# 0xPolygonZero/proof-protocol-decoder

Hardware: AMD Instinct MI355X
Metric: txn-proofs/sec (whole node), 256-txn synthetic block (higher is better)
Workload: dtype u64 (Goldilocks field)

## Files before the change

### include/bpg.h

```cpp
#ifndef BPG_H
#define BPG_H
#include <stddef.h>
#include <stdint.h>

#ifdef __cplusplus
extern "C" {
#endif

typedef enum {
  BP_OK = 0,
  BP_ERR_ABORTED = -1,
  BP_ERR_INVALID_INPUT = -2,
  BP_ERR_RANGE = -3,
  BP_ERR_DEVICE = -4,
  BP_ERR_VERIFY = -5,
  BP_ERR_UNSUPPORTED = -6
} bp_status;

const char* bp_last_error(void);
const char* bp_version(void);
int bp_device_count(void);
int bp_use_blocking_sync(int device);
int bp_host_wait_mode(int device);

// ... 61 lines not shown
  uint32_t first_index, count;
  uint32_t kind;
  uint32_t degree;
} bp_air_family;
typedef struct bp_air_desc {
  uint32_t air_id;
  char name[24];
  uint32_t fixed_n_cols;
  uint32_t n_const_max;
  uint32_t degree;
  uint32_t n_cols, n_aux;
  uint32_t n_air_constraints, n_ctl_constraints;
  uint32_t n_units;
  uint32_t n_families;
  bp_air_family families[24];
} bp_air_desc;
uint32_t bp_air_count(void);
int bp_air_describe(uint32_t air_id, uint32_t n_cols, uint32_t n_const, uint32_t deg_pow, bp_air_desc* out);

int bp_air_register(const uint64_t* program, size_t n_words, uint32_t* air_id_out);
int bp_air_unregister(uint32_t air_id);
int bp_air_program_digest(uint32_t air_id, uint8_t out[32]);

uint64_t bp_quotient_scratch_words(uint32_t air_id, const struct bp_stark_cfg* shape);
int bp_quotient_eval(uint32_t air_id, const struct bp_stark_cfg* shape, const uint64_t* d_trace_lde,
                     const uint64_t* d_aux_lde, const uint64_t* d_const_lde, const uint64_t ctl[4],
                     const uint64_t alphas[2], uint64_t* d_scratch, uint64_t* d_qvals_out, void* stream);

int bp_air_port_products(uint32_t air_id, const struct bp_stark_cfg* shape, const uint64_t* d_trace, uint64_t stride,
                         const uint64_t* d_consts, const uint64_t pub[4], const uint64_t ctl[4], uint64_t* d_aux_out, void* stream);

int bp_range_multiplicities(const uint64_t* d_values, uint64_t stride, uint32_t n_cols, uint64_t n_rows, const uint64_t* d_filter,
                            uint32_t log_range, uint64_t* d_mult, uint64_t* first_bad, void* stream);
void bp_tune_range_lds_log(int log_range);

int bp_debug_air_aux(uint32_t air_id, const struct bp_stark_cfg* shape, const uint64_t* d_trace, const uint64_t ctl[4],
                     uint64_t* d_aux_out, void* stream);

typedef struct bp_air_violation {
  uint32_t row, constraint, family, kind;
  uint64_t value;
} bp_air_violation;
int bp_air_check_trace(uint32_t air_id, const struct bp_stark_cfg* shape, const uint64_t* d_trace, uint64_t stride,
                       const uint64_t* d_consts, const uint64_t pub[4], uint32_t max_rows, uint64_t* n_violated_rows,
                       uint32_t* rows_out, bp_air_violation* viol_out, uint32_t max_viol, uint32_t* n_viol, void* stream);
int bp_air_check_trace_host(uint32_t air_id, const struct bp_stark_cfg* shape, const uint64_t* trace, uint64_t stride,
                            const uint64_t* consts, const uint64_t pub[4], uint32_t max_rows, uint64_t* n_violated_rows,
                            uint32_t* rows_out, bp_air_violation* viol_out, uint32_t max_viol, uint32_t* n_viol);

int bp_keccak_trace(const uint64_t* d_inputs, uint64_t seed, uint32_t log_n, uint64_t* d_trace_out, void* stream);
int bp_logic_trace(const uint64_t* d_inputs, uint64_t seed, uint32_t log_n, uint64_t* d_trace_out, void* stream);
int bp_memory_trace(const uint64_t* d_inputs, uint64_t seed, uint32_t log_n, uint64_t* d_trace_out, void* stream);
int bp_arithmetic_trace(const uint64_t* d_inputs, uint64_t seed, uint32_t log_n, uint64_t* d_trace_out, void* stream);
int bp_byte_packing_trace(const uint64_t* d_inputs, uint64_t seed, uint32_t log_n, uint64_t* d_trace_out, void* stream);
int bp_keccak_sponge_trace(const uint64_t* d_inputs, uint64_t seed, uint32_t log_n, uint64_t* d_trace_out, void* stream);
int bp_arithmetic_mul_trace(const uint64_t* d_inputs, uint64_t seed, uint32_t log_n, uint64_t* d_trace_out, void* stream);
int bp_arithmetic_div_trace(const uint64_t* d_inputs, uint32_t log_n, uint64_t* d_trace_out, void* stream);
int bp_arithmetic_div_layout(uint32_t* out, size_t n_words);
int bp_arithmetic_mod_trace(const uint64_t* d_inputs, uint32_t log_n, uint64_t* d_trace_out, void* stream);
int bp_arithmetic_mod_layout(uint32_t* out, size_t n_words);
int bp_arithmetic_shift_trace(const uint64_t* d_inputs, uint32_t log_n, uint64_t* d_trace_out, void* stream);
int bp_arithmetic_shift_layout(uint32_t* out, size_t n_words);
int bp_arithmetic_sdiv_trace(const uint64_t* d_inputs, uint32_t log_n, uint64_t* d_trace_out, void* stream);
int bp_arithmetic_sdiv_layout(uint32_t* out, size_t n_words);
int bp_arithmetic_exp_trace(const uint64_t* d_ops, uint32_t n_ops, const uint32_t* d_starts, uint32_t log_n, uint64_t* d_trace_out,
                            void* stream);
int bp_arithmetic_exp_layout(uint32_t* out, size_t n_words);

typedef struct bp_plonk_layout {
  uint32_t pi_len, n_paths, path_depth, path_pi0;
  uint32_t leaf_len;
} bp_plonk_layout;
int bp_plonk_constants(uint64_t seed, uint32_t log_n, const bp_plonk_layout* layout, uint64_t* d_consts_out, void* stream);
int bp_plonk_trace(const uint64_t* d_consts, uint64_t seed, const uint64_t* pi, const bp_plonk_layout* layout, const uint64_t* paths,
                   uint32_t log_n, uint64_t* d_trace_out, void* stream);

int bp_fri_fold(const uint64_t* d_values, uint32_t log_nl, uint32_t rate_bits, uint32_t arity_bits, uint64_t shift,
                const uint64_t beta[2], uint64_t* d_out, void* stream);

int bp_openings(const uint64_t* d_coeffs, uint64_t stride, uint32_t log_n, uint32_t n_cols, const uint64_t z0[2],
                const uint64_t z1[2], uint64_t* d_pw_scratch, uint64_t* d_out, void* stream);

int bp_pow_grind(const uint64_t state[12], uint32_t pos, uint32_t bits, uint64_t* nonce_out, void* stream);

typedef struct bp_stark_cfg {
  uint32_t log_n, n_cols, n_const, deg_pow, rate_bits, cap_height, num_queries, pow_bits, arity_bits,
      final_poly_bits;
} bp_stark_cfg;
int bp_stark_prove_synthetic(const bp_stark_cfg* cfg, uint64_t seed, uint64_t const_seed, int device,
                             uint8_t** out, size_t* out_len);
int bp_stark_prove_air(uint32_t air_id, const bp_stark_cfg* cfg, uint64_t seed, uint64_t const_seed, int device,
                       uint8_t** out, size_t* out_len);
int bp_stark_prove_trace(uint32_t air_id, const bp_stark_cfg* cfg, const uint64_t* d_trace, uint64_t stride,
                         const uint64_t* d_consts, const uint64_t* pub, int device, uint8_t** out, size_t* out_len);
int bp_stark_verify_air(uint32_t air_id, const bp_stark_cfg* cfg, const uint64_t* const_cap, const uint8_t* proof,
                        size_t len);
void bp_stark_public_inputs(uint64_t seed, uint64_t out[4]);
void bp_stark_public_input_list(uint64_t seed, uint64_t out[4]);
int bp_stark_verify_air_pub(uint32_t air_id, const bp_stark_cfg* cfg, const uint64_t* const_cap, const uint64_t* pub,
                            const uint8_t* proof, size_t len);
typedef struct bp_set_table {
  uint32_t air_id;
  bp_stark_cfg cfg;
  const uint64_t* d_trace;
  uint64_t stride;
  const uint64_t* d_consts;
  const uint64_t* pub;
} bp_set_table;
typedef struct bp_set_port {
  uint32_t table, port;
} bp_set_port;
typedef struct bp_set_link {
  uint32_t n_looking;
  bp_set_port looking[8];
  bp_set_port looked;
} bp_set_link;
#define BP_SET_SKIP_LINK_CHECK 1u
int bp_stark_prove_table_set(const bp_set_table* tables, uint32_t n_tables, const bp_set_link* links, uint32_t n_links,
                             uint32_t flags, int device, uint8_t** out, size_t* out_len);
int bp_stark_verify_table_set(const bp_set_table* statement, uint32_t n_tables, const uint64_t* const* const_caps,
                              const bp_set_link* links, uint32_t n_links, const uint8_t* proof, size_t len);
typedef struct bp_set_table_report {
  uint64_t n_violated_rows;
  uint32_t n_viol, reserved;
  bp_air_violation viol[8];
} bp_set_table_report;
typedef struct bp_set_link_report {
  uint32_t holds;
  uint32_t is_log;
  uint64_t n_looking, n_looked;
  uint64_t n_unbalanced;
  int32_t  first_looking_end;
  int32_t  bad_filter_end;
  int64_t  first_looking_row, first_looked_row, bad_filter_row;
  uint64_t bad_filter_value;
} bp_set_link_report;
typedef struct bp_set_report { bp_set_table_report table[8]; bp_set_link_report link[16]; } bp_set_report;
int bp_check_table_set(const bp_set_table* tables, uint32_t n_tables, const bp_set_link* links, uint32_t n_links,
                       int device, bp_set_report* out);
void bp_release_cached_memory(void);
void bp_free_buffer(uint8_t* buf);

#define BP_NUM_TABLES 7

typedef struct bp_config {
  uint32_t table_log_lo[BP_NUM_TABLES], table_log_hi[BP_NUM_TABLES];
  uint32_t stark_rate_bits, stark_cap_height, stark_num_queries, stark_pow_bits, arity_bits, final_poly_bits;
  uint32_t rec_log_n, rec_n_cols, rec_n_const, rec_rate_bits, rec_num_queries, rec_pow_bits;
  uint32_t shrink_depth;
  uint32_t rec_air_id;
  int32_t device;
  uint32_t n_workers;
  uint64_t arena_bytes;
} bp_config;

typedef struct bp_state bp_state;
typedef struct bp_verifier_state bp_verifier_state;

void bp_config_default(bp_config* cfg);
int bp_state_build(const bp_config* cfg, bp_state** out);
void bp_state_free(bp_state* s);
uint64_t bp_state_device_bytes(const bp_state* s);
const char* bp_state_warnings(const bp_state* s);
int bp_state_config(const bp_state* s, bp_config* out);

int bp_generate_txn_proof(const bp_state* s, const uint8_t* ir, size_t ir_len, const volatile int32_t* abort_flag,
// ... 152 lines not shown
```

### proof_protocol_decoder_amd/_abi.py

```python
import ctypes as C
from ctypes import POINTER as P

vp, cp, i, sz, dbl = C.c_void_p, C.c_char_p, C.c_int, C.c_size_t, C.c_double
u8, u32, u64, i32, i64 = C.c_uint8, C.c_uint32, C.c_uint64, C.c_int32, C.c_int64
u8p, u32p, u64p, i32p, szp = P(u8), P(u32), P(u64), P(i32), P(sz)
u8pp = P(u8p)

BP_OK, BP_ERR_ABORTED, BP_ERR_INVALID_INPUT, BP_ERR_RANGE, BP_ERR_DEVICE, BP_ERR_VERIFY, BP_ERR_UNSUPPORTED = 0, -1, -2, -3, -4, -5, -6
STATUS_NAMES = {v: k for k, v in list(globals().items()) if k == "BP_OK" or k.startswith("BP_ERR_")}
BP_SET_SKIP_LINK_CHECK = 1
BP_NUM_TABLES, BP_IR_WORDS, BP_PV_WORDS = 7, 25, 13

KNOBS = ("quad_threshold", "assume_loaded", "merkle_fused", "merkle_wide", "poseidon_mx", "poseidon_mx_sets",
         "poseidon_grouped", "ntt_mx", "ntt_split", "k5_spread", "host_wait", "host_poseidon", "rec_batch",
         "witness_threads", "side_lanes")


def _u32s(*names):
    return [(n, u32) for n in names]


class AirFamily(C.Structure):
    _fields_ = _u32s("first_index", "count", "kind", "degree")

# ... 104 lines not shown
_cfg, _conf, _wit, _opt, _gi = P(StarkCfg), P(BpConfig), P(TxnWitness), P(ShardOptions), P(GiOptions)
_trace = (i, [vp, u64, u32, vp, vp])
_check = [u32, _cfg, vp, u64, vp, u64p, u32, u64p, u32p, P(AirViolation), u32, u32p]
_knob, _ir_flag, _buf = (None, [i]), (i, [u64p, i]), [u8pp, szp]
PROTOTYPES = {
    "bp_last_error": (cp, []),
    "bp_version": (cp, []),
    "bp_device_count": (i, []),
    "bp_use_blocking_sync": (i, [i]),
    "bp_host_wait_mode": (i, [i]),
    "bp_ntt_batch": (i, [vp, u32, u32, u64, i, vp]),
    "bp_intt_batch": (i, [vp, u64, vp, u64, u32, u32, vp]),
    "bp_lde_batch": (i, [vp, u64, vp, u64, vp, u64, u32, u32, u32, i, vp]),
    "bp_debug_copy_u64": (i, [vp, vp, u64, vp]),
    "bp_debug_field_ops": (i, [vp, vp, vp, u64, vp]),
    "bp_debug_lazy_forms": (i, [vp, vp, vp, u64, vp]),
    "bp_debug_plonk_hash_fold": (i, [u64p, vp, vp]),
    "bp_debug_plonk_hash_fold_host": (i, [u64p, u64p]),
    "bp_debug_mul_pow2": (i, [vp, vp, u64, vp]),
    "bp_tune_quad_threshold": (None, [u64]),
    "bp_tune_merkle_fused": _knob,
    "bp_tune_merkle_wide": _knob,
    "bp_tune_poseidon_mx": _knob,
    "bp_tune_poseidon_mx_sets": _knob,
    "bp_tune_poseidon_grouped": _knob,
    "bp_tune_assume_loaded": _knob,
    "bp_tune_rec_batch": _knob,
    "bp_tune_side_lanes": _knob,
    "bp_tune_rec_riders": _knob,
    "bp_tune_txn_group": _knob,
    "bp_tune_rec_group": _knob,
    "bp_debug_rec_batch_histogram": (i, [u64p, u32, i]),
    "bp_tune_witness_threads": _knob,
    "bp_tune_host_wait": _knob,
    "bp_tune_host_poseidon": _knob,
    "bp_debug_poseidon_host": (i, [vp, sz]),
    "bp_tune_k5_spread": _knob,
    "bp_debug_poseidon_group_ops": (u32, [u32]),
    "bp_debug_poseidon_group_tables": (i, [u32, u32, u8p, i32p, i32p, i32p]),
    "bp_tune_ntt_split": _knob,
    "bp_tune_ntt_mx": _knob,
    "bp_tune_reset": (None, []),
    "bp_debug_tune_state": (i, [cp, sz]),
    "bp_debug_ntt_mx_tables": (i, [i, i, u8p, i32p, u64p, u64p]),
    "bp_debug_poseidon_mx_cin": (i, [u32p]),
    "bp_poseidon_perm_batch": (i, [vp, u64, vp]),
    "bp_merkle_digest_words": (u64, [u32, u32]),
    "bp_merkle_commit": (i, [vp, u64, u32, u32, u32, u32, vp, vp]),
    "bp_air_count": (u32, []),
    "bp_air_describe": (i, [u32, u32, u32, u32, P(AirDesc)]),
    "bp_air_register": (i, [vp, sz, u32p]),
    "bp_air_unregister": (i, [u32]),
    "bp_air_program_digest": (i, [u32, cp]),
    "bp_quotient_scratch_words": (u64, [u32, _cfg]),
    "bp_quotient_eval": (i, [u32, _cfg, vp, vp, vp, u64p, u64p, vp, vp, vp]),
    "bp_air_port_products": (i, [u32, _cfg, vp, u64, vp, u64p, u64p, vp, vp]),
    "bp_range_multiplicities": (i, [vp, u64, u32, u64, vp, u32, vp, u64p, vp]),
    "bp_tune_range_lds_log": _knob,
    "bp_debug_air_aux": (i, [u32, _cfg, vp, u64p, vp, vp]),
    "bp_air_check_trace": (i, _check + [vp]),
    "bp_air_check_trace_host": (i, _check),
    "bp_keccak_trace": _trace,
    "bp_logic_trace": _trace,
    "bp_memory_trace": _trace,
    "bp_arithmetic_trace": _trace,
    "bp_byte_packing_trace": _trace,
    "bp_keccak_sponge_trace": _trace,
    "bp_arithmetic_mul_trace": _trace,
    "bp_arithmetic_div_trace": (i, [vp, u32, vp, vp]),
    "bp_arithmetic_div_layout": (i, [u32p, sz]),
    "bp_arithmetic_mod_trace": (i, [vp, u32, vp, vp]),
    "bp_arithmetic_mod_layout": (i, [u32p, sz]),
    "bp_arithmetic_shift_trace": (i, [vp, u32, vp, vp]),
    "bp_arithmetic_shift_layout": (i, [u32p, sz]),
    "bp_arithmetic_sdiv_trace": (i, [vp, u32, vp, vp]),
    "bp_arithmetic_sdiv_layout": (i, [u32p, sz]),
    "bp_arithmetic_exp_trace": (i, [vp, u32, vp, u32, vp, vp]),
    "bp_arithmetic_exp_layout": (i, [u32p, sz]),
    "bp_plonk_constants": (i, [u64, u32, P(PlonkLayout), vp, vp]),
    "bp_plonk_trace": (i, [vp, u64, u64p, P(PlonkLayout), u64p, u32, vp, vp]),
    "bp_fri_fold": (i, [vp, u32, u32, u32, u64, u64p, vp, vp]),
    "bp_openings": (i, [vp, u64, u32, u32, u64p, u64p, vp, vp, vp]),
    "bp_pow_grind": (i, [u64p, u32, u32, u64p, vp]),
    "bp_stark_prove_synthetic": (i, [_cfg, u64, u64, i] + _buf),
    "bp_stark_prove_air": (i, [u32, _cfg, u64, u64, i] + _buf),
    "bp_stark_prove_trace": (i, [u32, _cfg, vp, u64, vp, u64p, i] + _buf),
    "bp_stark_verify_air": (i, [u32, _cfg, u64p, cp, sz]),
    "bp_stark_public_inputs": (None, [u64, u64p]),
    "bp_stark_public_input_list": (None, [u64, u64p]),
    "bp_stark_verify_air_pub": (i, [u32, _cfg, u64p, u64p, cp, sz]),
    "bp_stark_prove_table_set": (i, [P(SetTable), u32, P(SetLink), u32, u32, i] + _buf),
    "bp_stark_verify_table_set": (i, [P(SetTable), u32, P(u64p), P(SetLink), u32, cp, sz]),
    "bp_check_table_set": (i, [P(SetTable), u32, P(SetLink), u32, i, P(SetReport)]),
    "bp_release_cached_memory": (None, []),
    "bp_free_buffer": (None, [u8p]),
    "bp_config_default": (None, [_conf]),
    "bp_state_build": (i, [_conf, P(vp)]),
    "bp_state_free": (None, [vp]),
    "bp_state_device_bytes": (u64, [vp]),
    "bp_state_warnings": (cp, [vp]),
    "bp_state_config": (i, [vp, _conf]),
    "bp_generate_txn_proof": (i, [vp, cp, sz, i32p] + _buf),
    "bp_generate_txn_proof_keccak": (i, [vp, cp, sz, u64p, sz, vp] + _buf),
    "bp_generate_txn_proof_witness": (i, [vp, cp, sz, _wit, vp] + _buf),
    "bp_generate_txn_table_proofs": (i, [vp, cp, sz, _wit, vp] + _buf),
    "bp_generate_txn_table_proofs_group": (i, [vp, cp, sz, u32, vp, vp] + _buf),
    "bp_verify_txn_table_proofs": (i, [_conf, cp, sz]),
    "bp_verify_txn_table_proofs_for": (i, [_conf, cp, sz, cp, sz]),
    "bp_check_txn_witness": (i, [vp, cp, sz, _wit, P(WitnessReport)]),
    "bp_check_txn_witness_keccak": (i, [vp, cp, sz, u64p, sz, P(WitnessReport)]),
    "bp_debug_txn_plan": (i, [_conf, vp, sz, _wit, P(TxnPlan)]),
    "bp_generate_txn_proof_u8": (i, [vp, cp, sz, vp] + _buf),
    "bp_generate_agg_proof": (i, [vp, cp, sz, i, cp, sz, i] + _buf),
    "bp_generate_block_proof": (i, [vp, cp, sz, cp, sz] + _buf + [u64p]),
    "bp_verifier_state_from_prover": (i, [vp, P(vp)]),
    "bp_verifier_state_build": (i, [_conf, P(vp)]),
    "bp_verifier_state_from_caps": (i, [_conf, u64p, P(vp)]),
    "bp_verifier_state_free": (None, [vp]),
    "bp_verify_block_proof": (i, [vp, cp, sz]),
    "bp_verify_proof": (i, [vp, cp, sz]),
    "bp_ir_encode": (i, [u64, u64, u64, u64, u64p, u64, u32p, u32p, u64p]),
    "bp_ir_encode_dummy": (i, [u64, u64, u64, u64p, u64, u32p, u32p, u64p]),
    "bp_ir_set_keccak_air": _ir_flag,
    "bp_ir_set_logic_air": _ir_flag,
    "bp_ir_set_memory_air": _ir_flag,
    "bp_ir_set_arithmetic_air": _ir_flag,
    "bp_ir_set_arithmetic_mul_air": _ir_flag,
    "bp_ir_set_byte_packing_air": _ir_flag,
    "bp_ir_set_keccak_sponge_air": _ir_flag,
    "bp_proof_public_values": (i, [cp, sz, u64p, P(i)]),
    "bp_compact_decode": (i, [cp, sz, u8p, cp, u32p, u32p, u32p, u32p]),
    "bp_compact_decode_full": (i, [cp, sz] + _buf),
    "bp_compact_instructions": (i, [cp, sz] + _buf),
    "bp_keccak256": (None, [cp, sz, cp]),
    "bp_keccak256_permutation_inputs": (i, [cp, sz, cp, u64p, sz, szp]),
    "bp_keccak256_sponge_rows": (i, [cp, sz, cp, u64p, sz, szp]),
    "bp_decode_block_trace": (i, [cp, sz] + _buf),
    "bp_gi_count": (i, [cp, sz, u32p]),
    "bp_gi_chain_start": (i, [cp, sz, P(GiChain)]),
    "bp_gi_entry_ir": (i, [cp, sz, u32, _gi, P(GiChain), u64p]),
    "bp_generate_txn_proof_gi": (i, [vp, cp, sz, u32, _gi, P(GiChain), vp] + _buf),
    "bp_aggregation_plan": (u32, [u32, u32, u32p]),
    "bp_run_shard": (i, [u32, _opt, ShardLeafFn, ShardAggFn, vp, vp] + _buf + _buf),
    "bp_prove_shard": (i, [vp, cp, sz, u32, _opt, vp] + _buf + _buf),
    "bp_aggregate_proofs": (i, [vp, P(cp), szp, u32, _opt] + _buf),
    "bp_prove_shard_gi": (i, [vp, cp, sz, u32, u32, _gi, _opt, vp] + _buf + _buf),
    "bp_state_root_after": (i, [u64p, u64, u64, u64p]),
    "bp_profile_enable": (None, [i]),
    "bp_profile_reset": (None, []),
    "bp_profile_read": (i, [i, u64p, P(dbl), P(dbl)]),
}
```

### proof_protocol_decoder_amd/csrc/proofgen.cpp

```cpp
#include <algorithm>
#include <array>
#include <atomic>
#include <condition_variable>
#include <cstdlib>
#include <memory>
#include <mutex>
#include <string>
#include <system_error>
#include <thread>
#include <deque>
#include <functional>
#include <set>
#include "caller_table.hpp"
#include "mpt.hpp"
#include "prover.hpp"
#include "rec_pool.hpp"
#include "tune.hpp"
#include "txn_tables.hpp"
#include "worker_table.hpp"

using namespace bpg;
using namespace bpg::txn;
extern "C" int bp_use_blocking_sync(int device);
extern "C" int bp_host_wait_mode(int device);
// ... 553 lines not shown
  return BP_OK;
}
BPG_ABI_CATCH("bp_state_build")

const char* bp_state_warnings(const bp_state* s) { return s ? s->warnings.c_str() : ""; }
int bp_state_config(const bp_state* s, bp_config* out) {
  if (!s || !out) return fail(BP_ERR_INVALID_INPUT, "bp_state_config: null argument");
  *out = s->cfg;
  return BP_OK;
}

void bp_state_free(bp_state* s) {
  if (!s) return;
  (void)hipSetDevice(s->cfg.device);
  for (auto& w : s->workers) w->destroy();
  for (void* p : s->slabs) (void)hipFree(p);
  s->builder.destroy();
  delete s;
}

uint64_t bp_state_device_bytes(const bp_state* s) {
  if (!s) return 0;
  return s->builder.arena.capacity() + (uint64_t)s->workers.size() * s->cfg.arena_bytes;
}

int bp_state_root_after(const uint64_t root_before[4], uint64_t seed, uint64_t txn_number, uint64_t out[4]) {
  if (!root_before || !out) return fail(BP_ERR_INVALID_INPUT, "bp_state_root_after: null argument");
  for (int i = 0; i < 4; i++) if (root_before[i] >= gl::P) return fail(BP_ERR_INVALID_INPUT, "non-canonical state root");
  root_after(root_before, seed, txn_number, out);
  return BP_OK;
}

int bp_proof_public_values(const uint8_t* proof, size_t len, uint64_t pv_out[BP_PV_WORDS], int* kind_out) try {
  if (!proof || len % 8 || len < (BOX_HDR + BP_PV_WORDS) * 8) return fail(BP_ERR_INVALID_INPUT, "proof: truncated");
  const uint64_t* w = reinterpret_cast<const uint64_t*>(proof);
  if (w[0] != PROOF_BOX_MAGIC || w[1] > 2 || w[2] < BP_PV_WORDS || w[2] > air::plonk::MAX_PI || len / 8 < BOX_HDR + w[2])
    return fail(BP_ERR_INVALID_INPUT, "proof: bad header");
  if (pv_out) std::memcpy(pv_out, w + BOX_HDR + w[2] - BP_PV_WORDS, BP_PV_WORDS * 8);
  if (kind_out) *kind_out = (int)w[1];
  return BP_OK;
}
BPG_ABI_CATCH("bp_proof_public_values")

struct TableProofs {
  StarkCfg tcfg[BP_NUM_TABLES];
  std::vector<uint64_t> pv;
  Ctl ctl;
  std::vector<uint64_t> proof[BP_NUM_TABLES];
  uint64_t first_leaf[BP_NUM_TABLES][4];
};
static int build_traces(Worker& w, const Worker& stage, const uint64_t* I, const TxnWitness* wit, const StarkCfg tcfg[BP_NUM_TABLES],
                        uint64_t* const d_trace[BP_NUM_TABLES]) {
  int r;
  uint64_t* const pinned = stage.pinned;
  const size_t pinned_words = stage.pinned_words;
  bool given[BP_NUM_TABLES];
  size_t n_given[BP_NUM_TABLES];
  for (int t = 0; t < BP_NUM_TABLES; t++) {
    given[t] = given_table(wit, tcfg, t);
    n_given[t] = given[t] ? wit->n[t] : 0;
  }
  TracePlan plan;
  if ((r = plan_traces(tcfg, given, n_given, &plan))) return r;
  const bool lookup_kf = plan.lookup[L_SPONGE_KECCAK], lookup_bm = plan.lookup[L_PACKING_MEMORY], lookup_sl = plan.lookup[L_SPONGE_LOGIC];
  static const int GEN_ORDER[BP_NUM_TABLES] = {T_KECCAK_SPONGE, T_ARITHMETIC, T_BYTE_PACKING, T_CPU, T_KECCAK, T_LOGIC, T_MEMORY};
  const uint64_t* d_sponge = d_trace[T_KECCAK_SPONGE];
  const uint32_t sponge_log_n = tcfg[T_KECCAK_SPONGE].log_n;
  const uint64_t sponge_N = (uint64_t)1 << sponge_log_n;
  for (int gi = 0; gi < BP_NUM_TABLES; gi++) {
    const int t = GEN_ORDER[gi];
    const uint64_t N = (uint64_t)1 << tcfg[t].log_n, seed = I[10] ^ splitmix64(t + 1);
    const size_t wds = TABLES[t].item_words, cap = witness_capacity(t, N);
    const size_t mark = w.arena.mark();
    uint64_t* d_in = nullptr;
    if (t == T_LOGIC && lookup_sl) {
      const size_t n_ops = n_given[t], covered = (size_t)air::ctl::SPONGE_LOGIC_OPS * plan.logic_covered;
      d_in = w.arena.alloc_words((size_t)N * wds + n_ops * wds);
      if (!d_in) return fail(BP_ERR_DEVICE, "device arena exhausted for the logic table's operations");
      uint64_t* d_given = nullptr;
      if (n_ops) {
        if (n_ops * wds > pinned_words) return fail(BP_ERR_UNSUPPORTED, "too many logic operations for the input staging buffer");
        std::memcpy(pinned, wit->in[t], n_ops * wds * 8);
        d_given = d_in + (size_t)N * wds;
        BPG_HIP(hipMemcpyAsync(d_given, pinned, n_ops * wds * 8, hipMemcpyHostToDevice, w.stream));
      }
      if ((r = launch_logic_inputs_from_sponge(d_sponge, sponge_log_n, plan.logic_covered, given[t] ? d_given : nullptr, (uint32_t)n_ops,
                                               d_in, (uint32_t)N, seed, w.stream))) return r;
      if (given[t] && !d_given) {
        BPG_HIP(hipMemsetAsync(d_in + covered * wds, 0, ((size_t)N - covered) * wds * 8, w.stream));
      }
    } else if (given[t]) {
      const size_t words = cap * wds;
      d_in = w.arena.alloc_words(words);
      if (!d_in) return fail(BP_ERR_DEVICE, "device arena exhausted for the witness data of table %s", TABLES[t].name);
      if (words > pinned_words) return fail(BP_ERR_UNSUPPORTED, "table %s too tall for the input staging buffer", TABLES[t].name);
      fill_table_inputs(t, N, wit->in[t], wit->n[t], pinned);
      BPG_HIP(hipMemcpyAsync(d_in, pinned, words * 8, hipMemcpyHostToDevice, w.stream));
    } else if (t == T_KECCAK && lookup_kf) {
      d_in = w.arena.alloc_words(cap * wds);
      if (!d_in) return fail(BP_ERR_DEVICE, "device arena exhausted for the Keccak-f table's inputs");
      if ((r = launch_keccak_inputs_from_sponge(d_sponge, sponge_log_n, d_in, (uint32_t)cap, seed, w.stream))) return r;
    } else if (t == T_MEMORY && lookup_bm) {
      d_in = w.arena.alloc_words((size_t)N * wds);
      if (!d_in) return fail(BP_ERR_DEVICE, "device arena exhausted for the memory table's log");
      if ((r = launch_memory_inputs_from_byte_packing(d_trace[T_BYTE_PACKING], tcfg[T_BYTE_PACKING].log_n, d_in, (uint32_t)N, w.stream))) return r;
    }
    r = tcfg[t].air_id == air::SYNTHETIC
            ? launch_synth_trace(d_trace[t], nullptr, tcfg[t].log_n, tcfg[t].n_cols, 0, 1, seed, w.stream)
            : launch_air_trace(tcfg[t].air_id, d_trace[t], d_in, tcfg[t].log_n, d_in ? 0 : seed, w.stream, plan.sponge_row_limit);
    if (r) return r;
    if (t == T_KECCAK && lookup_kf) {
      r = launch_lookup_filter(air::KECCAK_F, d_trace[t], tcfg[t].log_n, d_sponge + (size_t)air::keccak_sponge::COL_FULL * sponge_N,
                               d_sponge + (size_t)air::keccak_sponge::COL_FINAL * sponge_N, (uint32_t)sponge_N, w.stream);
    } else if (t == T_MEMORY && lookup_bm) {
      r = launch_lookup_filter(air::MEMORY, d_trace[t], tcfg[t].log_n, d_trace[T_BYTE_PACKING], nullptr, (uint32_t)1 << tcfg[T_BYTE_PACKING].log_n, w.stream);
    } else if (t == T_LOGIC && lookup_sl) {
      r = launch_lookup_filter(air::LOGIC, d_trace[t], tcfg[t].log_n, d_sponge + (size_t)air::keccak_sponge::COL_FULL * sponge_N,
                               d_sponge + (size_t)air::keccak_sponge::COL_FINAL * sponge_N, plan.logic_covered, w.stream);
    }
    if (r) return r;
    if (d_in) {
      if ((r = w.wait())) return r;
      w.arena.release(mark);
    }
  }
  return BP_OK;
}

static int emit_tables(const TableProofs& tp, uint8_t** out, size_t* out_len) {
  const StarkCfg* tcfg = tp.tcfg;
  const std::vector<uint64_t>& pv = tp.pv;
  std::vector<uint64_t> o = {TABLES_MAGIC, BP_NUM_TABLES};
  o.insert(o.end(), pv.begin(), pv.end());
  o.insert(o.end(), tp.ctl.v, tp.ctl.v + 4);
  for (int t = 0; t < BP_NUM_TABLES; t++) {
    const uint64_t hdr[4] = {tcfg[t].air_id, tcfg[t].log_n, tcfg[t].n_cols, tp.proof[t].size()};
    o.insert(o.end(), hdr, hdr + 4);
    o.insert(o.end(), tp.proof[t].begin(), tp.proof[t].end());
  }
  uint64_t* buf = static_cast<uint64_t*>(std::malloc(o.size() * 8));
  if (!buf) return fail(BP_ERR_DEVICE, "host allocation failed");
  std::memcpy(buf, o.data(), o.size() * 8);
  *out = reinterpret_cast<uint8_t*>(buf);
  *out_len = o.size() * 8;
  return BP_OK;
}

static int group_recursion(const bp_state* s, Worker& w, size_t arena_mark, TableProofs* const* tps, uint32_t g, uint8_t** outs,
                           size_t* out_lens, RecPool* pool, const uint32_t* nodes) {
  const bp_config& cfg = s->cfg;
  constexpr uint32_t T = BP_NUM_TABLES;
  const uint32_t n_chains = T * g;
  int r;
  struct Child {
    uint64_t digest[4], leaf_cap[8];
  };
  std::vector<Child> child(n_chains);
  std::vector<std::vector<PathWitness>> slot_path(n_chains);
  for (uint32_t i = 0; i < g; i++) {
    TableProofs& tp = *tps[i];
    for (uint32_t t = 0; t < T; t++) {
      Child& c = child[T * i + t];
      proof_digest(tp.tcfg[t], tp.proof[t].data(), c.digest);
      slot_path[T * i + t].resize(1);
      first_query_trace_path(tp.tcfg[t], tp.proof[t].data(), c.leaf_cap, c.leaf_cap + 4, &slot_path[T * i + t][0], tp.first_leaf[t]);
      std::vector<uint64_t>().swap(tp.proof[t]);
    }
  }
  if ((r = w.wait())) return r;
  w.arena.release(arena_mark);
  {
    const uint32_t cap = lockstep_cap(s->rec_cfg, w.pinned_words, g);
    std::vector<const Circuit*> circ(n_chains);
    std::vector<std::vector<uint64_t>> pis(n_chains), chain_proof;
    for (uint32_t depth = 0; depth < cfg.shrink_depth; depth++) {
      if (w.aborted()) return fail(BP_ERR_ABORTED, "aborted in the recursion chains (level %u)", depth);
      for (uint32_t i = 0; i < g; i++)
        for (uint32_t t = 0; t < T; t++) {
          const Child& c = child[T * i + t];
          circ[T * i + t] = depth == 0 ? &s->table_circuits[s->table_offset[t] + (tps[i]->tcfg[t].log_n - cfg.table_log_lo[t])] : &s->shrink_circuits[t];
// ... 650 lines not shown
```

### proof_protocol_decoder_amd/csrc/prover.cpp

```cpp
#include <cstdio>
#include <cstdlib>
#include "prover.hpp"
#include "tune.hpp"
#include <algorithm>
#include <chrono>
#if defined(__x86_64__)
#include <immintrin.h>
#endif
#include <memory>
#include <mutex>
#include <unordered_map>
#include <thread>

namespace bpg {

static const uint64_t RC_HOST[360] = {
#include "poseidon_rc.inc"
};
static inline uint64_t sbox_host(uint64_t x) {
  uint64_t x2 = gl::mulc(x, x), x4 = gl::mulc(x2, x2), x3 = gl::mulc(x2, x);
  return gl::mulc(x3, x4);
}
static const uint32_t MDS_C[12] = {17, 15, 41, 16, 2, 28, 13, 13, 39, 18, 34, 20};
static inline void mds_finish_host(const uint64_t al[12], const uint64_t ah[12], uint64_t s[12]) {
// ... 205 lines not shown
  L.n_zeta = c.n_const + c.n_cols + L.n_aux + L.n_quot;
  L.n_next = c.n_cols + L.n_aux;
  L.depth0 = c.log_n + c.rate_bits - c.cap_height;
  size_t o = PROOF_HDR_WORDS;
  L.trace_cap = o; o += L.cap_words;
  L.aux_cap = o; o += L.cap_words;
  L.quot_cap = o; o += L.cap_words;
  L.open_zeta = o; o += 2 * (size_t)L.n_zeta;
  L.open_next = o; o += 2 * (size_t)L.n_next;
  L.open_first = o; o += 2 * (size_t)L.n_aux;
  L.fri_caps = o; o += L.cap_words * L.n_layers;
  L.final_poly = o; o += 2 * (size_t)L.final_len;
  L.pow = o; o += 1;
  L.queries = o;
  size_t q = 1 + (size_t)L.n_zeta + (size_t)(c.n_const ? 4 : 3) * L.depth0 * 4;
  uint32_t lm = c.log_n + c.rate_bits;
  for (uint32_t l = 0; l < L.n_layers; l++) {
    q += (2u << c.arity_bits) + (size_t)(lm - c.arity_bits - c.cap_height) * 4;
    lm -= c.arity_bits;
  }
  L.query_words = q;
  L.total = o + q * c.num_queries;
  return L;
}
void proof_digest(const StarkCfg& c, const uint64_t* proof, uint64_t out[4]) {
  ProofLayout L = proof_layout(c);
  std::vector<uint64_t> buf;
  buf.insert(buf.end(), proof + L.trace_cap, proof + L.trace_cap + 3 * L.cap_words);
  buf.insert(buf.end(), proof + L.final_poly, proof + L.final_poly + 2 * (size_t)L.final_len);
  buf.push_back(proof[L.pow]);
  hash_no_pad_host(buf.data(), buf.size(), out);
}

#define TRY(expr)        \
  do {                   \
    int _rc = (expr);    \
    if (_rc) return _rc; \
  } while (0)

int DeviceArena::init(size_t bytes) {
  destroy();
  BPG_HIP(hipMalloc(reinterpret_cast<void**>(&base_), bytes));
  cap_ = bytes;
  off_ = high_ = 0;
  owned_ = true;
  return BP_OK;
}
void DeviceArena::adopt(void* base, size_t bytes) {
  destroy();
  base_ = static_cast<char*>(base);
  cap_ = bytes;
  off_ = high_ = 0;
  owned_ = false;
}
void DeviceArena::destroy() {
  if (base_ && owned_) (void)hipFree(base_);
  base_ = nullptr;
  cap_ = off_ = 0;
  owned_ = true;
}
uint64_t* DeviceArena::alloc_words(size_t words) {
  size_t bytes = (words * 8 + 255) & ~(size_t)255;
  if (off_ + bytes > cap_) return nullptr;
  char* p = base_ + off_;
  off_ += bytes;
  high_ = std::max(high_, off_);
  return reinterpret_cast<uint64_t*>(p);
}
int Worker::init(int dev, size_t arena_bytes, void* slice) {
  device = dev;
  (void)bp_use_blocking_sync(dev);
  BPG_HIP(hipSetDevice(dev));
  BPG_HIP(hipStreamCreateWithFlags(&stream, hipStreamNonBlocking));
  if (slice) {
    arena.adopt(slice, arena_bytes);
  } else if (int rc = arena.init(arena_bytes)) {
    return rc;
  }
  pinned_words = (size_t)1 << 22;
  BPG_HIP(hipHostMalloc(reinterpret_cast<void**>(&pinned), pinned_words * 8, hipHostMallocDefault));
  BPG_HIP(hipHostGetDevicePointer(reinterpret_cast<void**>(&pinned_dev), pinned, 0));
  BPG_HIP(hipHostMalloc(reinterpret_cast<void**>(&hash_rows), MAX_LOCKSTEP * HASH_ROWS_WORDS * 8, hipHostMallocDefault));
  BPG_HIP(hipHostGetDevicePointer(reinterpret_cast<void**>(&hash_rows_dev), hash_rows, 0));
  BPG_HIP(hipMalloc(reinterpret_cast<void**>(&d_pow_result), 8 * MAX_LOCKSTEP));
  {
    void* dev = nullptr;
    BPG_HIP(hipHostMalloc(&args_mem, ARG_RING_BYTES, hipHostMallocDefault));
    BPG_HIP(hipHostGetDevicePointer(&dev, args_mem, 0));
    args.adopt(args_mem, dev, ARG_RING_BYTES);
    arg_ring_register(stream, &args);
  }
  BPG_HIP(hipEventCreateWithFlags(&sync_event, hipEventBlockingSync | hipEventDisableTiming));
  return init_ntt_kernels();
}
void Worker::destroy() {
  if (stream) (void)hipStreamSynchronize(stream);
  if (stream) arg_ring_unregister(stream);
  args.forget();
  if (args_mem) (void)hipHostFree(args_mem);
  args_mem = nullptr;
  arena.destroy();
  if (pinned) (void)hipHostFree(pinned);
  if (hash_rows) (void)hipHostFree(hash_rows);
  hash_rows = hash_rows_dev = nullptr;
  if (d_pow_result) (void)hipFree(d_pow_result);
  if (sync_event) (void)hipEventDestroy(sync_event);
  if (stream) (void)hipStreamDestroy(stream);
  sync_event = nullptr;
  pinned = nullptr;
  d_pow_result = nullptr;
  stream = nullptr;
}
extern "C" int bp_host_wait_mode(int device);
int Worker::wait_recorded() {
  using clock = std::chrono::steady_clock;
  const int knob = tune().host_wait.load(std::memory_order_relaxed);
  if (knob != 1 && !device_loaded()) {
    const clock::time_point t0 = clock::now();
    for (;;) {
      const hipError_t e = hipEventQuery(sync_event);
      if (e == hipSuccess) return BP_OK;
      if (e != hipErrorNotReady) return fail(BP_ERR_DEVICE, "hipEventQuery failed: %s", hipGetErrorString(e));
      if (clock::now() - t0 > std::chrono::microseconds(1500)) break;
    }
  }
  if (knob == 1 || (knob == 0 && bp_host_wait_mode(device) == 1)) {
    BPG_HIP(hipEventSynchronize(sync_event));
    return BP_OK;
  }
  const clock::time_point t0 = clock::now();
  for (;;) {
    const hipError_t e = hipEventQuery(sync_event);
    if (e == hipSuccess) return BP_OK;
    if (e != hipErrorNotReady) return fail(BP_ERR_DEVICE, "hipEventQuery failed: %s", hipGetErrorString(e));
    const int64_t waited_us = std::chrono::duration_cast<std::chrono::microseconds>(clock::now() - t0).count();
    if (waited_us < 8) continue;
    std::this_thread::sleep_for(std::chrono::microseconds(std::min<int64_t>(200, std::max<int64_t>(5, waited_us / 8))));
  }
}
int Worker::wait() {
  BPG_HIP(hipEventRecord(sync_event, stream));
  TRY(wait_recorded());
  args.rewind();
  return BP_OK;
}

namespace {
constexpr int MAX_DEVICES = 16;
struct SharedRing {
  std::mutex mu;
  ArgRing ring;
  void* mem = nullptr;
};
struct ArgRings {
  std::mutex mu;
  std::unordered_map<hipStream_t, ArgRing*> of;
  std::atomic<uint64_t> generation{1};
  SharedRing shared[MAX_DEVICES];
};
ArgRings& arg_rings() {
  static ArgRings* r = new ArgRings();
  return *r;
}
struct FoundRings {
  uint64_t generation = 0;
  int n = 0;
  hipStream_t st[4];
  ArgRing* ring[4];
};
ArgRing* ring_of(hipStream_t st) {
  thread_local FoundRings found;
  ArgRings& r = arg_rings();
  const uint64_t gen = r.generation.load(std::memory_order_acquire);
  if (found.generation != gen) { found.generation = gen; found.n = 0; }
  for (int k = 0; k < found.n; k++)
    if (found.st[k] == st) return found.ring[k];
  ArgRing* ring = nullptr;
  bool current = true;
  {
    std::lock_guard<std::mutex> lk(r.mu);
    current = r.generation.load(std::memory_order_relaxed) == gen;
    auto it = r.of.find(st);
    if (it != r.of.end()) ring = it->second;
  }
  if (ring && current) {
    const int k = found.n < 4 ? found.n++ : 0;
    found.st[k] = st;
    found.ring[k] = ring;
  }
  return ring;
}
int arg_ring_status(ArgRing::Status s, size_t bytes, size_t cap) {
  switch (s) {
    case ArgRing::OK: return BP_OK;
    case ArgRing::TOO_LARGE: return fail(BP_ERR_UNSUPPORTED, "argument blocks of %zu bytes do not fit the argument ring (%zu bytes)", bytes, cap);
    case ArgRing::WAIT_FAILED: return fail(BP_ERR_DEVICE, "waiting for the stream of a full argument ring failed");
    default: return fail(BP_ERR_DEVICE, "the stream's argument ring has no memory");
  }
}
}
void arg_ring_register(hipStream_t st, ArgRing* ring) {
  ArgRings& r = arg_rings();
  std::lock_guard<std::mutex> lk(r.mu);
  r.of[st] = ring;
  r.generation.fetch_add(1, std::memory_order_release);
}
void arg_ring_unregister(hipStream_t st) {
  ArgRings& r = arg_rings();
  std::lock_guard<std::mutex> lk(r.mu);
  r.of.erase(st);
  r.generation.fetch_add(1, std::memory_order_release);
}
int arg_ring_put(hipStream_t st, const void* blocks, size_t bytes, const void** dev) {
  if (ArgRing* own = ring_of(st))
    return arg_ring_status(own->put(blocks, bytes, dev, [&] { return hipStreamSynchronize(st) == hipSuccess ? 0 : 1; }), bytes, own->capacity());
  int device = 0;
  BPG_HIP(hipGetDevice(&device));
  if (device < 0 || device >= MAX_DEVICES) return fail(BP_ERR_UNSUPPORTED, "device %d: argument rings are kept for devices 0..%d", device, MAX_DEVICES - 1);
  SharedRing& sh = arg_rings().shared[device];
  std::lock_guard<std::mutex> lk(sh.mu);
  if (!sh.mem) {
    void *m = nullptr, *d = nullptr;
    BPG_HIP(hipHostMalloc(&m, ARG_RING_BYTES, hipHostMallocDefault));
    const hipError_t e = hipHostGetDevicePointer(&d, m, 0);
    if (e != hipSuccess) {
      (void)hipHostFree(m);
      return fail(BP_ERR_DEVICE, "hipHostGetDevicePointer failed for the argument ring: %s", hipGetErrorString(e));
    }
    sh.mem = m;
    sh.ring.adopt(m, d, ARG_RING_BYTES);
  }
  return arg_ring_status(sh.ring.put(blocks, bytes, dev, [] { return hipDeviceSynchronize() == hipSuccess ? 0 : 1; }), bytes, sh.ring.capacity());
}
int Worker::d2h(uint64_t* host_dst, const uint64_t* dev_src, size_t words) {
  for (size_t off = 0; off < words; off += pinned_words) {
    size_t k = std::min(pinned_words, words - off);
    BPG_HIP(hipMemcpyAsync(pinned, dev_src + off, k * 8, hipMemcpyDeviceToHost, stream));
    TRY(wait());
    std::memcpy(host_dst + off, pinned, k * 8);
  }
  return BP_OK;
}

#define ARENA_ALLOC(var, words)                                                                         \
  uint64_t* var = w.arena.alloc_words(words);                                                           \
  if (!var)                                                                                             \
    return fail(BP_ERR_DEVICE, "device arena exhausted (%zu MiB) allocating %zu words for " #var,     \
                w.arena.capacity() >> 20, (size_t)(words))

extern "C" int bp_lde_batch(const uint64_t*, uint64_t, uint64_t*, uint64_t, uint64_t*, uint64_t, uint32_t, uint32_t,
                            uint32_t, int, void*);
extern "C" uint64_t bp_merkle_digest_words(uint32_t, uint32_t);

int commit_batch(Worker& w, const uint64_t* d_in, uint32_t n_cols, uint32_t batch, uint32_t log_n, uint32_t rate_bits,
                 uint32_t cap_height, bool from_coeffs, Committed* out) {
  PendingCommit pc;
  TRY(commit_launch(w, w, 0, d_in, n_cols, batch, log_n, rate_bits, cap_height, from_coeffs, &pc));
  return commit_finish(pc, out);
}
int commit_launch(Worker& mem, Worker& lane, size_t mailbox_word, const uint64_t* d_in, uint32_t n_cols, uint32_t batch,
                  uint32_t log_n, uint32_t rate_bits, uint32_t cap_height, bool from_coeffs, PendingCommit* pc) {
  Worker& w = mem;
  if (batch == 0 || batch > MAX_LOCKSTEP) return fail(BP_ERR_INVALID_INPUT, "commit: batch of %u", batch);
  const uint64_t n = (uint64_t)1 << log_n, m = n << rate_bits;
  const size_t all_cols = (size_t)n_cols * batch;
  ARENA_ALLOC(lde, all_cols * m);
  const size_t dw = bp_merkle_digest_words(log_n + rate_bits, cap_height);
  ARENA_ALLOC(digests, dw * batch);
  uint64_t* coeffs = const_cast<uint64_t*>(d_in);
  if (!from_coeffs) {
    ARENA_ALLOC(c, all_cols * n);
    coeffs = c;
  }
  TRY(bp_lde_batch(d_in, n, from_coeffs ? nullptr : coeffs, n, lde, m, log_n, rate_bits, (uint32_t)all_cols, from_coeffs,
                   lane.stream));
  const size_t cw = (size_t)4 << cap_height;
  if (mailbox_word + cw * batch > lane.pinned_words) return fail(BP_ERR_UNSUPPORTED, "caps do not fit the mailbox");
  bool mirrored = false;
  TRY(merkle_commit_cols(lde, m, n_cols, log_n, rate_bits, cap_height, digests, lane.stream, lane.pinned_dev + mailbox_word,
                         &mirrored, batch, (uint64_t)n_cols * m, dw));
  if (!mirrored) {
    for (uint32_t b = 0; b < batch; b++)
      BPG_HIP(hipMemcpyAsync(lane.pinned + mailbox_word + b * cw, digests + (b + 1) * dw - cw, cw * 8, hipMemcpyDeviceToHost,
                             lane.stream));
  }
  *pc = PendingCommit{&lane, mailbox_word, d_in, coeffs, lde, digests, dw, cw, n_cols, batch, log_n, rate_bits, cap_height, from_coeffs};
  return BP_OK;
}
int commit_finish(const PendingCommit& pc, Committed* out) {
  TRY(pc.lane->wait());
  const uint64_t n = (uint64_t)1 << pc.log_n, m = n << pc.rate_bits;
  for (uint32_t b = 0; b < pc.batch; b++) {
    Committed& o = out[b];
    o.log_n = pc.log_n; o.n_cols = pc.n_cols; o.rate_bits = pc.rate_bits; o.cap_height = pc.cap_height;
    o.coeffs = pc.coeffs + (size_t)b * pc.n_cols * n;
    o.lde = pc.lde + (size_t)b * pc.n_cols * m;
    o.digests = pc.digests + (size_t)b * pc.dw;
    o.values = pc.from_coeffs ? nullptr : pc.d_in + (size_t)b * pc.n_cols * n;
    const uint64_t* cap = pc.lane->pinned + pc.mailbox_word + b * pc.cw;
    o.cap.assign(cap, cap + pc.cw);
  }
  return BP_OK;
}
int commit(Worker& w, const uint64_t* d_in, uint32_t n_cols, uint32_t log_n, uint32_t rate_bits,
           uint32_t cap_height, bool from_coeffs, Committed* out) {
  return commit_batch(w, d_in, n_cols, 1, log_n, rate_bits, cap_height, from_coeffs, out);
}

int quotient_args(const StarkCfg& cfg, const Ctl& ctl, uint64_t alpha0, uint64_t alpha1, QuotArgs* out, QuotCoset* coset,
                  int loaded, uint32_t batch) {
  QuotArgs& qa = *out;
  const uint32_t log_n = cfg.log_n, r = cfg.rate_bits, R = 1u << r, C = cfg.n_cols, K = cfg.n_const;
  const air::Shape shape{cfg.air_id, C, K, cfg.deg_pow};
  const uint32_t A = air::any_n_aux(shape);
  const uint64_t N = (uint64_t)1 << log_n, M = N << r;
  const uint64_t wM = gl::root(log_n + r), wN = gl::root(log_n);
  qa.trace_stride = qa.aux_stride = qa.const_stride = M;
  TRY(get_table(0, log_n, 0, &qa.tw_n));
  qa.air_id = cfg.air_id;
  qa.log_n = log_n; qa.rate_bits = r; qa.n_cols = C; qa.n_const = K; qa.n_aux = A; qa.deg_pow = cfg.deg_pow;
  qa.n_air_constraints = air::any_n_constraints(shape);
  qa.n_constraints = qa.n_air_constraints + air::any_n_ctl_constraints(shape);
  qa.side_rows = cfg.air_id == air::PLONK ? 1 : 0;
  qa.n_air_units = air::any_n_units(shape) - qa.side_rows;
  if (qa.side_rows) {
    const uint64_t* fold = nullptr;
    TRY(get_hash_fold_table(&fold));
  }
  qa.aux_per_unit = cfg.air_id == air::SYNTHETIC ? std::max<uint32_t>(16, (A + 15) / 16) : A;
  qa.n_ctl_units = cfg.air_id == air::PLONK ? 0 : (A + qa.aux_per_unit - 1) / qa.aux_per_unit;
  qa.n_ports = air::prog::is_registered(cfg.air_id) && A > 1 ? A / 2 : 0;
  if (qa.n_ports) qa.n_ctl_units = qa.n_ports;
  const uint32_t n_units = qa.n_air_units + qa.n_ctl_units, wg_x = (uint32_t)((M + 255) / 256) * std::max<uint32_t>(1, batch);
  const uint32_t loaded_rows = (cfg.air_id == air::SYNTHETIC && !tune().k5_spread.load(std::memory_order_relaxed))
                                   ? 1 : std::min<uint32_t>(n_units, std::max<uint32_t>(1, (256 + wg_x - 1) / wg_x));
  const bool is_loaded = loaded < 0 ? device_loaded() : loaded != 0;
  const uint32_t want_rows = is_loaded ? loaded_rows : std::min<uint32_t>(n_units, std::max<uint32_t>(1, (2048 + wg_x - 1) / wg_x));
  qa.units_per_wg = (n_units + want_rows - 1) / want_rows;
  qa.alpha0 = alpha0; qa.alpha1 = alpha1;
  qa.g = wN; qa.g_inv = gl::inv(wN); qa.n_inv = gl::inv(N);
  if (coset)
    for (uint32_t t = 0; t < R; t++) {
      coset->g_t[t] = gl::mulc(gl::GENERATOR, gl::pow(wM, t));
      coset->zh_t[t] = gl::subc(gl::pow(coset->g_t[t], N), 1);
      coset->zh_inv_t[t] = gl::inv(coset->zh_t[t]);
    }
  qa.ctl = ctl;
  return BP_OK;
}
size_t quotient_partial_words(const QuotArgs& qa) {
  const uint32_t n_units = qa.n_air_units + qa.n_ctl_units, wg_rows = (n_units + qa.units_per_wg - 1) / qa.units_per_wg + qa.side_rows;
  return wg_rows > 1 ? (size_t)wg_rows * 2 * (((size_t)1 << qa.log_n) << qa.rate_bits) : 0;
}

int fri_layer_args(uint32_t log_nl, uint32_t rate_bits, uint32_t arity_bits, uint64_t shift, FriLayerArgs* out) {
  FriLayerArgs& fa = *out;
  const uint32_t R = 1u << rate_bits, arity = 1u << arity_bits;
  if (arity_bits != 4) return fail(BP_ERR_UNSUPPORTED, "only arity_bits = 4 is built");
  if (log_nl < arity_bits || rate_bits > 4) return fail(BP_ERR_INVALID_INPUT, "FRI layer too small or rate too high");
  fa.log_nl = log_nl; fa.rate_bits = rate_bits; fa.arity_bits = arity_bits;
  TRY(get_table(1, log_nl, 0, &fa.tw_nl_inv));
  const uint64_t wMl = gl::root(log_nl + rate_bits), wa_inv = gl::inv(gl::root(arity_bits));
  for (uint32_t t = 0; t < R; t++) fa.g_t_inv[t] = gl::inv(gl::mulc(shift, gl::pow(wMl, t)));
  for (uint32_t k = 0; k < arity; k++) fa.wa_inv_pow[k] = gl::pow(wa_inv, k);
  fa.arity_inv = gl::inv(arity);
  return BP_OK;
}

int stark_prove(Worker& w, const StarkCfg& cfg, const Committed* consts, const Committed& trace,
                const uint64_t* d_tv, const Ctl& ctl, Challenger& ch, std::vector<uint64_t>& proof, uint64_t* first_trace_leaf) {
  return stark_prove_batch(w, cfg, 1, &consts, &trace, &d_tv, &ctl, &ch, &proof, first_trace_leaf);
}

int stark_prove_batch(Worker& w, const StarkCfg& cfg, uint32_t B, const Committed* const* consts,
                      const Committed* trace, const uint64_t* const* d_tv, const Ctl* ctl, Challenger* ch,
                      std::vector<uint64_t>* proofs, uint64_t* first_trace_leaf) {
  TRY(check_cfg(cfg));
  if (B == 0 || B > MAX_LOCKSTEP || (size_t)B * cfg.num_queries > MAX_BATCH_QUERIES)
    return fail(BP_ERR_INVALID_INPUT, "stark_prove_batch: %u proofs x %u queries (at most %u proofs, %u queries in all)", B,
                cfg.num_queries, MAX_LOCKSTEP, MAX_BATCH_QUERIES);
  const ProofLayout L = proof_layout(cfg);
  const uint32_t log_n = cfg.log_n, r = cfg.rate_bits, h = cfg.cap_height, R = 1u << r;
  const uint64_t N = (uint64_t)1 << log_n, M = N << r;
  const uint32_t C = cfg.n_cols, K = cfg.n_const, A = L.n_aux, Q = L.n_quot;
  hipStream_t st = w.stream;
  uint64_t* P[MAX_LOCKSTEP];
  for (uint32_t b = 0; b < B; b++) {
    if (K && !(consts && consts[b])) return fail(BP_ERR_INVALID_INPUT, "constants commitment missing");
    proofs[b].assign(L.total, 0);
    uint64_t* p = P[b] = proofs[b].data();
    p[0] = PROOF_MAGIC; p[1] = log_n; p[2] = C; p[3] = K; p[4] = A; p[5] = Q; p[6] = r; p[7] = h;
    p[8] = cfg.num_queries; p[9] = L.n_layers; p[10] = L.final_len; p[11] = cfg.deg_pow; p[12] = cfg.pow_bits;
    p[13] = cfg.arity_bits; p[14] = cfg.air_id;
    std::memcpy(p + L.trace_cap, trace[b].cap.data(), L.cap_words * 8);
  }
  if (w.aborted()) return fail(BP_ERR_ABORTED, "aborted before auxiliary commitment");

  const uint64_t wN = gl::root(log_n);
  const uint64_t *tw_n = nullptr, *coset_scale = nullptr, *coset_scale_inv = nullptr;
  TRY(get_table(0, log_n, 0, &tw_n));
  TRY(get_table(2, log_n, r, &coset_scale));
  TRY(get_table(3, log_n, r, &coset_scale_inv));

  ARENA_ALLOC(d_auxv, (size_t)B * A * N);
  {
    AuxArgs aa[MAX_LOCKSTEP];
    for (uint32_t b = 0; b < B; b++) {
      aa[b] = AuxArgs{d_tv[b], d_auxv + (size_t)b * A * N, ctl[b]};
      if (K) aa[b].consts = consts[b]->values;
    }
    TRY(launch_aux(aa, B, cfg.air_id, C, log_n, st));
  }
  Committed aux[MAX_LOCKSTEP];
  TRY(commit_batch(w, d_auxv, A, B, log_n, r, h, false, aux));
  for (uint32_t b = 0; b < B; b++) {
    std::memcpy(P[b] + L.aux_cap, aux[b].cap.data(), L.cap_words * 8);
    ch[b].observe(aux[b].cap.data(), L.cap_words);
  }

  QuotArgs qa[MAX_LOCKSTEP] = {};
  QuotCoset coset{};
  const int loaded = device_loaded();
  for (uint32_t b = 0; b < B; b++) {
    const uint64_t alpha0 = ch[b].challenge(), alpha1 = ch[b].challenge();
    qa[b].trace_lde = trace[b].lde; qa[b].aux_lde = aux[b].lde; qa[b].const_lde = K ? consts[b]->lde : nullptr;
    TRY(quotient_args(cfg, ctl[b], alpha0, alpha1, &qa[b], &coset, loaded, B));
  }
  ARENA_ALLOC(d_qc, (size_t)B * Q * N);
  const size_t mark_tmp = w.arena.mark();
  {
    const size_t cpow_words = quotient_table_words(qa[0]), part_words = quotient_partial_words(qa[0]) + 1;
    ARENA_ALLOC(d_cpow, B * cpow_words);
    ARENA_ALLOC(d_partial, B * part_words);
    ARENA_ALLOC(d_qvals, (size_t)B * 2 * M);
    for (uint32_t b = 0; b < B; b++) {
      qa[b].apow = d_cpow + b * cpow_words; qa[b].partial = d_partial + b * part_words; qa[b].qvals = d_qvals + (size_t)b * 2 * M;
    }
    TRY(launch_quotient(qa, B, coset, st));
    TRY(intt_nat2br(d_qvals, N, d_qvals, N, log_n, B * 2 * R, true, st));
    ChunkArgs ca[MAX_LOCKSTEP] = {};
    const uint64_t wr_inv = gl::inv(gl::root(r)), sn_inv = gl::inv(gl::pow(gl::GENERATOR, N)), r_inv = gl::inv(R);
    for (uint32_t b = 0; b < B; b++) {
      ChunkArgs& c = ca[b];
      c.e = d_qvals + (size_t)b * 2 * M; c.inv_scale = coset_scale_inv; c.out = d_qc + (size_t)b * Q * N; c.out_stride = N;
      c.log_n = log_n; c.rate_bits = r;
      for (uint32_t k = 0; k < R; k++) {
        c.wr_inv_pow[k] = gl::pow(wr_inv, k);
        c.chunk_scale[k] = gl::mulc(gl::pow(sn_inv, k), r_inv);
      }
// ... 39 lines not shown
        }
        d_o += (size_t)n_cols * 4;
      };
      seg(K ? consts[b]->coeffs : nullptr, K, pw, 1);
      seg(trace[b].coeffs, C, pw, 2);
      seg(aux[b].coeffs, A, pw, 2);
      seg(quot[b].coeffs, Q, pw, 1);
      seg(aux[b].coeffs, A, pw1, 1);
    }
    TRY(launch_openings_multi(om, B, st));
  }
  TRY(w.wait());
  for (uint32_t b = 0; b < B; b++) {
    const uint64_t* ho = w.pinned + (size_t)b * open_cols * 4;
    uint64_t* oz = P[b] + L.open_zeta;
    for (size_t c = 0; c < (size_t)K + C + A + Q; c++) { oz[2 * c] = ho[4 * c]; oz[2 * c + 1] = ho[4 * c + 1]; }
    uint64_t* on = P[b] + L.open_next;
    for (size_t c = 0; c < (size_t)C + A; c++) { on[2 * c] = ho[4 * (K + c) + 2]; on[2 * c + 1] = ho[4 * (K + c) + 3]; }
    uint64_t* of = P[b] + L.open_first;
    const size_t base = (size_t)K + C + A + Q;
    for (size_t c = 0; c < A; c++) { of[2 * c] = ho[4 * (base + c)]; of[2 * c + 1] = ho[4 * (base + c) + 1]; }
    ch[b].observe(P[b] + L.open_zeta, 2 * (size_t)L.n_zeta);
    ch[b].observe(P[b] + L.open_next, 2 * (size_t)L.n_next);
    ch[b].observe(P[b] + L.open_first, 2 * (size_t)A);
  }

  gl::Ext alpha[MAX_LOCKSTEP];
  for (uint32_t b = 0; b < B; b++) alpha[b] = ch[b].challenge_ext();
  const uint32_t k0 = L.n_zeta, k1 = L.n_next, k2 = A;
  ARENA_ALLOC(d_apow, (size_t)B * 2 * k0);
  {
    AlphaPowArgs ap[MAX_LOCKSTEP];
    for (uint32_t b = 0; b < B; b++) ap[b] = AlphaPowArgs{d_apow + (size_t)b * 2 * k0, alpha[b]};
    TRY(launch_alpha_pows(ap, B, k0, st));
  }
  struct OracleRef { const Committed* c; int32_t e[3]; };
  OracleRef refs[MAX_LOCKSTEP][4];
  int n_or = 0;
  for (uint32_t b = 0; b < B; b++) {
    n_or = 0;
    if (K) refs[b][n_or++] = {consts[b], {0, -1, -1}};
    refs[b][n_or++] = {&trace[b], {(int32_t)K, 0, -1}};
    refs[b][n_or++] = {&aux[b], {(int32_t)(K + C), (int32_t)C, 0}};
    refs[b][n_or++] = {&quot[b], {(int32_t)(K + C + A), -1, -1}};
  }
  const uint32_t cols_per_chunk = 64;
  uint32_t total_chunks = 0;
  for (int o = 0; o < n_or; o++) total_chunks += (refs[0][o].c->n_cols + cols_per_chunk - 1) / cols_per_chunk;
  ARENA_ALLOC(d_g, (size_t)B * 6 * N);
  {
    const bool one_pass = loaded != 0;
    uint64_t* d_cpart = nullptr;
    if (!one_pass) {
      ARENA_ALLOC(cp, (size_t)B * total_chunks * 6 * N);
      d_cpart = cp;
    }
    CombineMulti cm[MAX_LOCKSTEP] = {};
    uint64_t* gp[MAX_LOCKSTEP];
    CombineReduceArgs cr[MAX_LOCKSTEP];
    for (uint32_t b = 0; b < B; b++) {
      uint32_t chunk_base = 0;
      uint64_t* part = d_cpart ? d_cpart + (size_t)b * total_chunks * 6 * N : nullptr;
      for (int o = 0; o < n_or; o++) {
        CombineArgs& cb = cm[b].a[cm[b].n_oracles++];
        cb.coeffs = refs[b][o].c->coeffs; cb.stride = N; cb.log_n = log_n; cb.n_cols = refs[b][o].c->n_cols;
        cb.cols_per_chunk = cols_per_chunk; cb.chunk_base = chunk_base;
        for (int k = 0; k < 3; k++) cb.exp_base[k] = refs[b][o].e[k];
        cb.alpha_pows = d_apow + (size_t)b * 2 * k0; cb.partial = part;
        chunk_base += (cb.n_cols + cols_per_chunk - 1) / cols_per_chunk;
      }
      gp[b] = d_g + (size_t)b * 6 * N;
      cr[b] = CombineReduceArgs{part, gp[b]};
    }
    if (one_pass) {
      TRY(launch_combine_all(cm, B, gp, st));
    } else {
      TRY(launch_combine_partial_multi(cm, B, total_chunks, st));
      TRY(launch_combine_reduce(cr, B, total_chunks, log_n, st));
    }
  }
  ARENA_ALLOC(d_glde, (size_t)B * 6 * M);
  TRY(ntt_br2nat(d_g, N, d_glde, M, N, log_n, 6 * B, R, coset_scale, false, st));
  ARENA_ALLOC(d_v0, (size_t)B * 2 * M);
  {
    FriInitArgs fi[MAX_LOCKSTEP] = {};
    for (uint32_t b = 0; b < B; b++) {
      FriInitArgs& f = fi[b];
      f.glde = d_glde + (size_t)b * 6 * M; f.tw_n = tw_n; f.log_n = log_n; f.rate_bits = r;
      std::memcpy(f.g_t, coset.g_t, sizeof(f.g_t));
      const uint64_t* opens[3] = {P[b] + L.open_zeta, P[b] + L.open_next, P[b] + L.open_first};
      const uint32_t kk[3] = {k0, k1, k2};
      for (int k = 0; k < 3; k++) {
        gl::Ext acc = gl::ext(0);
        for (size_t j = kk[k]; j-- > 0;) acc = gl::add(gl::mul(acc, alpha[b]), gl::Ext{opens[k][2 * j], opens[k][2 * j + 1]});
        f.y[k] = acc;
      }
      f.z[0] = zeta[b]; f.z[1] = zeta_next[b]; f.z[2] = gl::ext(1);
      f.alpha_shift[0] = gl::pow(alpha[b], (uint64_t)k1 + k2);
      f.alpha_shift[1] = gl::pow(alpha[b], k2);
      f.alpha_shift[2] = gl::ext(1);
      f.out = d_v0 + (size_t)b * 2 * M;
    }
    TRY(launch_fri_init(fi, B, st));
  }

  const uint32_t ab = cfg.arity_bits, arity = 1u << ab;
  const uint64_t *layer_values[9], *layer_digests[9];
  size_t layer_vstride[9], layer_dstride[9];
  uint32_t layer_log_nl[9];
  uint64_t* cur = d_v0;
  size_t cur_stride = 2 * M;
  uint32_t log_nl = log_n;
  uint64_t shift = gl::GENERATOR;
  for (uint32_t l = 0; l < L.n_layers; l++) {
    const uint32_t log_leaves = log_nl - ab + r;
    const size_t dw = bp_merkle_digest_words(log_leaves, h), next_words = (size_t)2 << log_leaves;
    ARENA_ALLOC(d_dig, dw * B);
    ARENA_ALLOC(d_next, next_words * B);
    FriLayerArgs fa[MAX_LOCKSTEP] = {};
    TRY(fri_layer_args(log_nl, r, ab, shift, &fa[0]));
    for (uint32_t b = 0; b < B; b++) {
      if (b) fa[b] = fa[0];
      fa[b].values = cur + b * cur_stride; fa[b].out = d_next + b * next_words; fa[b].digests = d_dig + b * dw;
    }
    TRY(launch_fri_layer_leaves(fa, B, st));
    bool mirrored = false;
    TRY(merkle_upper_levels(d_dig, log_leaves, h, st, w.pinned_dev, &mirrored, B, dw));
    if (!mirrored)
      for (uint32_t b = 0; b < B; b++)
        BPG_HIP(hipMemcpyAsync(w.pinned + b * L.cap_words, d_dig + (b + 1) * dw - L.cap_words, L.cap_words * 8,
                               hipMemcpyDeviceToHost, st));
    TRY(w.wait());
    for (uint32_t b = 0; b < B; b++) {
      uint64_t* cap = P[b] + L.fri_caps + l * L.cap_words;
      std::memcpy(cap, w.pinned + b * L.cap_words, L.cap_words * 8);
      ch[b].observe(cap, L.cap_words);
      fa[b].beta = ch[b].challenge_ext();
    }
    TRY(launch_fri_fold(fa, B, st));
    layer_values[l] = cur; layer_vstride[l] = cur_stride; layer_digests[l] = d_dig; layer_dstride[l] = dw;
    layer_log_nl[l] = log_nl;
    cur = d_next;
    cur_stride = next_words;
    log_nl -= ab;
    shift = gl::pow(shift, arity);
  }
  {
    const uint32_t log_ml = log_nl + r;
    const uint64_t ml = (uint64_t)1 << log_ml, nl = (uint64_t)1 << log_nl;
    if (2 * ml * B > w.pinned_words) return fail(BP_ERR_UNSUPPORTED, "final FRI layer does not fit the mailbox");
    for (uint32_t b = 0; b < B; b++)
      BPG_HIP(hipMemcpyAsync(w.pinned + b * 2 * ml, cur + b * cur_stride, 2 * ml * 8, hipMemcpyDeviceToHost, st));
    TRY(w.wait());
    const uint64_t w_inv = gl::inv(gl::root(log_ml)), s_inv = gl::inv(shift), ml_inv = gl::inv(ml);
    std::vector<uint64_t> wp(ml);
    wp[0] = 1;
    for (uint64_t k = 1; k < ml; k++) wp[k] = gl::mulc(wp[k - 1], w_inv);
    for (uint32_t b = 0; b < B; b++) {
      const uint64_t* hv = w.pinned + b * 2 * ml;
      uint64_t sk = ml_inv;
      for (uint64_t k = 0; k < ml; k++) {
        uint64_t c0 = 0, c1 = 0;
        for (uint64_t i = 0; i < ml; i++) {
          const uint64_t pos = (i & (R - 1)) * nl + (i >> r);
          const uint64_t tw = wp[(i * k) & (ml - 1)];
          c0 = gl::addc(c0, gl::mulc(hv[2 * pos], tw));
          c1 = gl::addc(c1, gl::mulc(hv[2 * pos + 1], tw));
        }
        c0 = gl::mulc(c0, sk);
        c1 = gl::mulc(c1, sk);
        sk = gl::mulc(sk, s_inv);
        if (k < L.final_len) {
          P[b][L.final_poly + 2 * k] = c0;
          P[b][L.final_poly + 2 * k + 1] = c1;
        } else if (c0 || c1) {
          return fail(BP_ERR_INVALID_INPUT, "FRI final polynomial has a non-zero tail: the witness violates the AIR");
        }
      }
      ch[b].observe(P[b] + L.final_poly, 2 * (size_t)L.final_len);
    }
  }
  if (w.aborted()) return fail(BP_ERR_ABORTED, "aborted before proof of work");

  {
    PowArgs pa[MAX_LOCKSTEP] = {};
    for (uint32_t b = 0; b < B; b++) {
      ch[b].pow_state(pa[b].state, &pa[b].pos);
      pa[b].bits = cfg.pow_bits;
    }
    unsigned long long res[MAX_LOCKSTEP];
    for (uint32_t b = 0; b < B; b++) res[b] = 0;
    if (cfg.pow_bits) {
      const uint32_t batch0 = (uint32_t)std::min<uint64_t>(1u << 20, std::max<uint64_t>(1u << 12, (uint64_t)1 << (cfg.pow_bits ? cfg.pow_bits - 1 : 0)));
      uint32_t batch = batch0, n_batches = 0;
      BPG_HIP(hipMemsetAsync(w.d_pow_result, 0xFF, 8 * MAX_LOCKSTEP, st));
      for (uint64_t base = 0;;) {
        for (int k = 0; k < 4; k++) {
          if (++n_batches > 8) batch = std::min<uint32_t>(1u << 20, batch * 2);
          for (uint32_t b = 0; b < B; b++) pa[b].base = base;
          TRY(launch_pow(pa, B, batch, w.d_pow_result, st));
          base += batch;
        }
        BPG_HIP(hipMemcpyAsync(w.pinned, w.d_pow_result, 8 * B, hipMemcpyDeviceToHost, st));
        TRY(w.wait());
        bool all = true;
        for (uint32_t b = 0; b < B; b++) {
          res[b] = reinterpret_cast<const unsigned long long*>(w.pinned)[b];
          all = all && res[b] != ~0ULL;
        }
        if (all) break;
        if (w.aborted()) return fail(BP_ERR_ABORTED, "aborted during proof of work");
        if (base > ((uint64_t)1 << 44)) return fail(BP_ERR_DEVICE, "proof of work search exhausted");
      }
    }
    for (uint32_t b = 0; b < B; b++) {
      const uint64_t nonce = res[b];
      P[b][L.pow] = nonce;
      ch[b].observe(nonce);
      const uint64_t resp = ch[b].challenge();
      if (cfg.pow_bits && (resp >> (64 - cfg.pow_bits)) != 0)
        return fail(BP_ERR_DEVICE, "proof-of-work witness failed the host re-check");
    }
  }

  {
    std::unique_ptr<QueryArgs> qa2(new QueryArgs());
    std::unique_ptr<QueryLayerArgs> ql(new QueryLayerArgs());
    const size_t q_words = (size_t)cfg.num_queries * L.query_words;
    const bool q_direct = q_words * B + 4 * B <= w.pinned_words;
    uint64_t* d_q = q_direct ? w.pinned_dev : w.arena.alloc_words(q_words * B + 4 * B);
    if (!d_q) return fail(BP_ERR_DEVICE, "device arena exhausted (%zu MiB) allocating the query buffer", w.arena.capacity() >> 20);
    qa2->query_words = ql->query_words = L.query_words;
    qa2->n_queries = ql->n_queries = cfg.num_queries;
    qa2->log_n = log_n; qa2->rate_bits = r; qa2->cap_height = h;
    ql->rate_bits = r; ql->cap_height = h; ql->arity_bits = ab;
    for (uint32_t b = 0; b < B; b++) {
      for (uint32_t q = 0; q < cfg.num_queries; q++)
        qa2->x_index[b * cfg.num_queries + q] = ql->x_index[b * cfg.num_queries + q] = ch[b].challenge() & (M - 1);
      qa2->proof[b].out = ql->proof[b].out = d_q + b * q_words;
      qa2->proof[b].first_leaf = first_trace_leaf ? d_q + B * q_words + 4 * b : nullptr;
      uint32_t off = 1;
      for (int o = 0; o < n_or; o++) {
        const Committed* c = refs[b][o].c;
        qa2->proof[b].oracle[o] = QueryOracle{c->lde, c->digests, M, c->n_cols, off};
        off += c->n_cols + L.depth0 * 4;
      }
      for (uint32_t l = 0; l < L.n_layers; l++) {
        ql->proof[b].layer[l] = QueryLayer{layer_values[l] + b * layer_vstride[l], layer_digests[l] + b * layer_dstride[l],
                                          layer_log_nl[l], off};
        off += 2 * arity + (layer_log_nl[l] - ab + r - h) * 4;
      }
    }
    qa2->leaf_oracle = K ? 1 : 0;
    TRY(launch_query_initial(*qa2, B, n_or, st));
    TRY(launch_query_layers(*ql, B, L.n_layers, st));
    if (q_direct) {
      TRY(w.wait());
      for (uint32_t b = 0; b < B; b++) std::memcpy(P[b] + L.queries, w.pinned + b * q_words, q_words * 8);
      if (first_trace_leaf) std::memcpy(first_trace_leaf, w.pinned + B * q_words, 4 * B * 8);
    } else {
      for (uint32_t b = 0; b < B; b++) TRY(w.d2h(P[b] + L.queries, d_q + b * q_words, q_words));
      if (first_trace_leaf) TRY(w.d2h(first_trace_leaf, d_q + B * q_words, 4 * B));
    }
  }
  return BP_OK;
}

}
```

### proof_protocol_decoder_amd/csrc/prover.hpp

```cpp
#pragma once
#include <atomic>
#include <cstdint>
#include <cstring>
#include <random>
#include <vector>
#include "common.hpp"
#include "gl.hpp"
#include "stark_kernels.hpp"
#include "arg_ring.hpp"
#include "air_program.hpp"

namespace bpg {

void poseidon_host(uint64_t s[12]);
void hash_no_pad_host(const uint64_t* in, size_t len, uint64_t out[4]);
void poseidon_hash_rows(const uint64_t* in, size_t n, std::vector<uint64_t>* rows, uint64_t digest[4]);
void poseidon_merkle_rows(const uint64_t leaf[4], uint64_t index, const uint64_t* siblings, uint32_t depth, uint64_t* rows,
                          uint64_t root[4]);

class Challenger {
 public:
  Challenger() { std::memset(this, 0, sizeof(*this)); }
  void observe(uint64_t e) {
    n_out_ = 0;
// ... 13 lines not shown
  }
  gl::Ext challenge_ext() {
    uint64_t a = challenge(), b = challenge();
    return gl::Ext{a, b};
  }
  void pow_state(uint64_t st[12], uint32_t* pos) const {
    std::memcpy(st, state_, sizeof(state_));
    for (unsigned i = 0; i < n_in_; i++) st[i] = in_[i];
    *pos = n_in_;
  }

 private:
  void duplex() {
    for (unsigned i = 0; i < n_in_; i++) state_[i] = in_[i];
    n_in_ = 0;
    poseidon_host(state_);
    std::memcpy(out_, state_, 8 * sizeof(uint64_t));
    n_out_ = 8;
  }
  uint64_t state_[12], in_[8], out_[8];
  unsigned n_in_, n_out_;
};

struct FreshChallenges {
  std::mt19937_64 g{((uint64_t)std::random_device{}() << 32) ^ std::random_device{}()};
  uint64_t operator()() {
    uint64_t a;
    do a = g() % gl::P; while (a < 2);
    return a;
  }
};

struct StarkCfg {
  uint32_t log_n, n_cols, n_const, deg_pow, rate_bits, cap_height, num_queries, pow_bits, arity_bits,
      final_poly_bits;
  uint32_t air_id = air::SYNTHETIC;
};
struct ProofLayout {
  size_t cap_words, trace_cap, aux_cap, quot_cap, open_zeta, open_next, open_first, fri_caps, final_poly, pow,
      queries, query_words, total;
  uint32_t n_aux, n_quot, n_layers, final_len, n_zeta, n_next, depth0;
};
constexpr uint64_t PROOF_MAGIC = 0x4B52415453475042ULL;
constexpr size_t PROOF_HDR_WORDS = 16;
int check_cfg(const StarkCfg& c);
ProofLayout proof_layout(const StarkCfg& c);
void proof_digest(const StarkCfg& c, const uint64_t* proof, uint64_t out[4]);

class DeviceArena {
 public:
  int init(size_t bytes);
  void adopt(void* base, size_t bytes);
  void span(size_t bytes) { cap_ = bytes; }
  void destroy();
  uint64_t* alloc_words(size_t words);
  size_t mark() const { return off_; }
  void release(size_t m) { off_ = m; }
  size_t capacity() const { return cap_; }
  size_t high_water() const { return high_; }

 private:
  char* base_ = nullptr;
  size_t cap_ = 0, off_ = 0, high_ = 0;
  bool owned_ = true;
};

constexpr size_t HASH_ROWS_WORDS = (size_t)(air::plonk::HASH_ROWS_MAX + air::plonk::MERKLE_ROWS_MAX + air::plonk::LEAF_ROWS_MAX) * air::plonk::H_WIRES;

struct Committed {
  uint64_t *coeffs = nullptr, *lde = nullptr, *digests = nullptr;
  const uint64_t* values = nullptr;
  uint32_t log_n = 0, n_cols = 0, rate_bits = 0, cap_height = 0;
  std::vector<uint64_t> cap;
};

struct Worker {
  hipStream_t stream = nullptr;
  DeviceArena arena;
  uint64_t* pinned = nullptr;
  uint64_t* pinned_dev = nullptr;
  size_t pinned_words = 0;
  uint64_t *hash_rows = nullptr, *hash_rows_dev = nullptr;
  unsigned long long* d_pow_result = nullptr;
  ArgRing args;
  void* args_mem = nullptr;
  hipEvent_t sync_event = nullptr;
  const volatile int32_t* abort_flag = nullptr;
  const volatile uint8_t* abort_flag_u8 = nullptr;
  int device = 0;

  int init(int device, size_t arena_bytes, void* slice = nullptr);
  void destroy();
  int d2h(uint64_t* host_dst, const uint64_t* dev_src, size_t words);
  int wait();
  int wait_recorded();
  bool aborted() const { return (abort_flag && *abort_flag) || (abort_flag_u8 && *abort_flag_u8); }
};

int commit(Worker& w, const uint64_t* d_in, uint32_t n_cols, uint32_t log_n, uint32_t rate_bits,
           uint32_t cap_height, bool from_coeffs, Committed* out);
int commit_batch(Worker& w, const uint64_t* d_in, uint32_t n_cols, uint32_t batch, uint32_t log_n, uint32_t rate_bits,
                 uint32_t cap_height, bool from_coeffs, Committed* out);

struct PendingCommit {
  Worker* lane = nullptr;
  size_t mailbox_word = 0;
  const uint64_t* d_in = nullptr;
  uint64_t *coeffs = nullptr, *lde = nullptr, *digests = nullptr;
  size_t dw = 0, cw = 0;
  uint32_t n_cols = 0, batch = 0, log_n = 0, rate_bits = 0, cap_height = 0;
  bool from_coeffs = false;
};
int commit_launch(Worker& mem, Worker& lane, size_t mailbox_word, const uint64_t* d_in, uint32_t n_cols, uint32_t batch,
                  uint32_t log_n, uint32_t rate_bits, uint32_t cap_height, bool from_coeffs, PendingCommit* pc);
int commit_finish(const PendingCommit& pc, Committed* out);

int stark_prove(Worker& w, const StarkCfg& cfg, const Committed* consts, const Committed& trace,
                const uint64_t* d_trace_values, const Ctl& ctl, Challenger& ch, std::vector<uint64_t>& proof,
                uint64_t* first_trace_leaf = nullptr);
int stark_prove_batch(Worker& w, const StarkCfg& cfg, uint32_t batch, const Committed* const* consts,
                      const Committed* trace, const uint64_t* const* d_trace_values, const Ctl* ctl, Challenger* ch,
                      std::vector<uint64_t>* proofs, uint64_t* first_trace_leaf = nullptr);

constexpr size_t ARG_RING_BYTES = (size_t)1 << 20;
void arg_ring_register(hipStream_t st, ArgRing* ring);
void arg_ring_unregister(hipStream_t st);

void prover_active(int delta);
int provers_active();
bool device_loaded();

int quotient_args(const StarkCfg& cfg, const Ctl& ctl, uint64_t alpha0, uint64_t alpha1, QuotArgs* out, QuotCoset* coset,
                  int loaded = -1, uint32_t batch = 1);
size_t quotient_partial_words(const QuotArgs& qa);
int fri_layer_args(uint32_t log_nl, uint32_t rate_bits, uint32_t arity_bits, uint64_t shift, FriLayerArgs* out);

int stark_verify(const StarkCfg& cfg, const uint64_t* const_cap, const Ctl& ctl, Challenger& ch,
                 const uint64_t* proof, size_t n_words);

}
```

### proof_protocol_decoder_amd/csrc/stark_api.cpp

```cpp
#include <algorithm>
#include <cstdlib>
#include <cstring>
#include <vector>
#include "caller_table.hpp"
#include "plonk_hash_fold.hpp"

using namespace bpg;

namespace {
constexpr uint32_t LONE_PI_LEN = 4;
void lone_public_input_list(uint64_t seed, uint64_t out[LONE_PI_LEN]) {
  for (uint64_t j = 0; j < LONE_PI_LEN; j++) {
    uint64_t z = (seed ^ ((0x50 + j) << 32)) + 0x9E3779B97F4A7C15ULL;
    z = (z ^ (z >> 30)) * 0xBF58476D1CE4E5B9ULL;
    z = (z ^ (z >> 27)) * 0x94D049BB133111EBULL;
    out[j] = gl::canon(z ^ (z >> 31));
  }
}
int prove_lone(Worker& w, const CallerTable& t, uint8_t** out, size_t* out_len) {
  Challenger ch;
  Committed consts, trace;
  const uint64_t* d_values = nullptr;
  int rc = commit_caller_table(w, ch, t, &consts, &trace, &d_values);
  if (rc) return rc;
// ... 343 lines not shown
}

int bp_quotient_eval(uint32_t air_id, const bp_stark_cfg* shape, const uint64_t* d_trace_lde, const uint64_t* d_aux_lde,
                     const uint64_t* d_const_lde, const uint64_t ctl_in[4], const uint64_t alphas[2],
                     uint64_t* d_scratch, uint64_t* d_qvals_out, void* stream) try {
  StarkCfg c;
  int rc = quot_cfg(air_id, shape, &c);
  if (rc) return rc;
  if (!d_trace_lde || !d_aux_lde || (c.n_const && !d_const_lde) || !ctl_in || !alphas || !d_scratch || !d_qvals_out)
    return fail(BP_ERR_INVALID_INPUT, "bp_quotient_eval: null argument");
  for (int i = 0; i < 4; i++)
    if (ctl_in[i] >= gl::P) return fail(BP_ERR_INVALID_INPUT, "bp_quotient_eval: non-canonical challenge");
  if (alphas[0] >= gl::P || alphas[1] >= gl::P) return fail(BP_ERR_INVALID_INPUT, "bp_quotient_eval: non-canonical alpha");
  if ((rc = init_ntt_kernels())) return rc;
  Ctl ctl;
  for (int i = 0; i < 4; i++) ctl.v[i] = ctl_in[i];
  QuotArgs qa{};
  QuotCoset coset{};
  qa.trace_lde = d_trace_lde; qa.aux_lde = d_aux_lde; qa.const_lde = c.n_const ? d_const_lde : nullptr;
  if ((rc = quotient_args(c, ctl, alphas[0], alphas[1], &qa, &coset))) return rc;
  qa.apow = d_scratch; qa.partial = d_scratch + quotient_table_words(qa); qa.qvals = d_qvals_out;
  return launch_quotient(qa, coset, as_stream(stream));
}
BPG_ABI_CATCH("bp_quotient_eval")

int bp_air_port_products(uint32_t air_id, const bp_stark_cfg* shape, const uint64_t* d_trace, uint64_t stride, const uint64_t* d_consts,
                         const uint64_t pub[4], const uint64_t ctl_in[4], uint64_t* d_aux_out, void* stream) try {
  const auto program = air::prog::find(air_id);
  if (!program || !program->n_ports)
    return fail(BP_ERR_INVALID_INPUT, "bp_air_port_products: air_id 0x%08x is no registered program with lookup ports", air_id);
  StarkCfg c;
  int rc = quot_cfg(air_id, shape, &c);
  if (rc) return rc;
  if (!ctl_in || !d_aux_out) return fail(BP_ERR_INVALID_INPUT, "bp_air_port_products: null argument");
  const CallerTable t = caller_table(c, d_trace, stride, d_consts, pub);
  if ((rc = check_caller_table("bp_air_port_products", "", t))) return rc;
  AuxArgs a{d_trace, d_aux_out, Ctl{}};
  a.consts = t.consts;
  for (int i = 0; i < 4; i++) {
    if (ctl_in[i] >= gl::P) return fail(BP_ERR_INVALID_INPUT, "bp_air_port_products: non-canonical challenge");
    a.ctl.v[i] = ctl_in[i];
    a.ctl.pub[i] = pub ? pub[i] : 0;
  }
  return launch_port_products(&a, 1, air_id, c.log_n, stride, as_stream(stream));
}
BPG_ABI_CATCH("bp_air_port_products")

int bp_debug_air_aux(uint32_t air_id, const bp_stark_cfg* shape, const uint64_t* d_trace, const uint64_t ctl_in[4], uint64_t* d_aux_out,
                     void* stream) try {
  const air::Desc* ai = air::info(air_id);
  if (!ai || !ai->in_pair) return fail(BP_ERR_INVALID_INPUT, "bp_debug_air_aux: air_id %u is no built-in AIR with a lookup side", air_id);
  StarkCfg c;
  int rc = quot_cfg(air_id, shape, &c);
  if (rc) return rc;
  if (!d_trace || !ctl_in || !d_aux_out) return fail(BP_ERR_INVALID_INPUT, "bp_debug_air_aux: null argument");
  AuxArgs a{d_trace, d_aux_out, Ctl{}};
  for (int i = 0; i < 4; i++) {
    if (ctl_in[i] >= gl::P) return fail(BP_ERR_INVALID_INPUT, "bp_debug_air_aux: non-canonical challenge");
    a.ctl.v[i] = ctl_in[i];
  }
  return launch_aux(&a, 1, air_id, c.n_cols, c.log_n, as_stream(stream));
}
BPG_ABI_CATCH("bp_debug_air_aux")

int bp_fri_fold(const uint64_t* d_values, uint32_t log_nl, uint32_t rate_bits, uint32_t arity_bits, uint64_t shift,
                const uint64_t beta[2], uint64_t* d_out, void* stream) try {
  if (!d_values || !d_out || !beta) return fail(BP_ERR_INVALID_INPUT, "bp_fri_fold: null argument");
  if (shift == 0 || shift >= gl::P || beta[0] >= gl::P || beta[1] >= gl::P)
    return fail(BP_ERR_INVALID_INPUT, "bp_fri_fold: non-canonical field element");
  int rc = init_ntt_kernels();
  if (rc) return rc;
  FriLayerArgs fa{};
  if ((rc = fri_layer_args(log_nl, rate_bits, arity_bits, shift, &fa))) return rc;
  fa.values = d_values; fa.out = d_out; fa.digests = nullptr;
  fa.beta = gl::Ext{beta[0], beta[1]};
  return launch_fri_fold(fa, as_stream(stream));
}
BPG_ABI_CATCH("bp_fri_fold")

int bp_pow_grind(const uint64_t state[12], uint32_t pos, uint32_t bits, uint64_t* nonce_out, void* stream) try {
  if (!state || !nonce_out) return fail(BP_ERR_INVALID_INPUT, "bp_pow_grind: null argument");
  if (pos >= 8 || bits == 0 || bits > 40) return fail(BP_ERR_INVALID_INPUT, "bp_pow_grind: pos must be a rate word, bits in 1..40");
  hipStream_t st = as_stream(stream);
  DeviceBuf res_buf;
  BPG_HIP(hipMalloc(&res_buf.p, 8));
  unsigned long long* d_res = res_buf.as<unsigned long long>();
  PowArgs pa{};
  for (int i = 0; i < 12; i++) pa.state[i] = state[i];
  pa.pos = pos; pa.bits = bits;
  int rc = BP_OK;
  unsigned long long res = ~0ULL;
  if (hipMemsetAsync(d_res, 0xFF, 8, st) != hipSuccess) rc = fail(BP_ERR_DEVICE, "hipMemsetAsync failed");
  uint32_t batch = (uint32_t)std::min<uint64_t>(1u << 20, std::max<uint64_t>(1u << 12, (uint64_t)2 << bits));
  for (uint64_t base = 0; rc == BP_OK; base += batch, batch = std::min<uint32_t>(1u << 20, batch * 2)) {
    pa.base = base;
    if ((rc = launch_pow(pa, batch, d_res, st))) break;
    if (hipMemcpyAsync(&res, d_res, 8, hipMemcpyDeviceToHost, st) != hipSuccess || hipStreamSynchronize(st) != hipSuccess) {
      rc = fail(BP_ERR_DEVICE, "bp_pow_grind: copy back failed");
      break;
    }
    if (res != ~0ULL) break;
    if (base > ((uint64_t)1 << 44)) rc = fail(BP_ERR_DEVICE, "proof of work search exhausted");
  }
  if (rc == BP_OK) *nonce_out = res;
  return rc;
}
BPG_ABI_CATCH("bp_pow_grind")

int bp_openings(const uint64_t* d_coeffs, uint64_t stride, uint32_t log_n, uint32_t n_cols, const uint64_t z0[2],
                const uint64_t z1[2], uint64_t* d_pw_scratch, uint64_t* d_out, void* stream) try {
  if (!n_cols) return BP_OK;
  if (!d_coeffs || !z0 || !d_pw_scratch || !d_out) return fail(BP_ERR_INVALID_INPUT, "bp_openings: null argument");
  if (log_n > 30 || stride < ((uint64_t)1 << log_n)) return fail(BP_ERR_INVALID_INPUT, "bp_openings: bad shape");
  const uint64_t* zz[2] = {z0, z1 ? z1 : z0};
  for (int k = 0; k < 2; k++)
    if (zz[k][0] >= gl::P || zz[k][1] >= gl::P) return fail(BP_ERR_INVALID_INPUT, "bp_openings: non-canonical point");
  hipStream_t st = as_stream(stream);
  const uint32_t n_points = z1 ? 2 : 1;
  int rc = launch_power_vectors(d_pw_scratch, log_n, gl::Ext{z0[0], z0[1]}, gl::Ext{zz[1][0], zz[1][1]}, n_points, st);
  if (rc) return rc;
  return launch_openings(d_coeffs, stride, log_n, n_cols, d_pw_scratch, n_points, d_out, st);
}
BPG_ABI_CATCH("bp_openings")

}
```

### proof_protocol_decoder_amd/csrc/stark_kernels.hip

```cpp
#include <map>
#include <mutex>
#include <vector>
#include "common.hpp"
#include "gl.hpp"
#include "poseidon.cuh"
#include "poseidon_mx.cuh"
#include "stark_kernels.hpp"
#include "arg_ring.hpp"
#include "quotient_dev.cuh"
#include "air_program.hpp"
#include "plonk_hash_fold.hpp"

namespace {

using gl::Ext;
using namespace bpg::k5;

__device__ __forceinline__ uint64_t splitmix64(uint64_t x) {
  uint64_t z = x + 0x9E3779B97F4A7C15ULL;
  z = (z ^ (z >> 30)) * 0xBF58476D1CE4E5B9ULL;
  z = (z ^ (z >> 27)) * 0x94D049BB133111EBULL;
  return z ^ (z >> 31);
}
__device__ __forceinline__ uint64_t rnd(uint64_t seed, uint64_t col, uint64_t row) {
// ... 1030 lines not shown
}
__device__ __forceinline__ void fri_combine_store(gl::DotAcc (&d01)[4], gl::DotAcc (&d2)[4], uint64_t* out, uint32_t n, uint32_t pos) {
  const Ext acc[3] = {Ext{gl::dot_reduce(d01[0]), gl::dot_reduce(d01[1])}, Ext{gl::dot_reduce(d01[2]), gl::dot_reduce(d01[3])},
                      Ext{gl::dot_reduce(d2[0]), gl::dot_reduce(d2[1])}};
#pragma unroll
  for (int b = 0; b < 3; b++) {
    out[(2 * b) * (uint64_t)n + pos] = acc[b].c0;
    out[(2 * b + 1) * (uint64_t)n + pos] = acc[b].c1;
  }
}
__device__ __forceinline__ void fri_combine_partial_body(const bpg::CombineArgs& a, uint32_t chunk) {
  const uint32_t pos = blockIdx.x * blockDim.x + threadIdx.x, n = 1u << a.log_n;
  if (pos >= n) return;
  const uint32_t c0 = chunk * a.cols_per_chunk, c1 = min(c0 + a.cols_per_chunk, a.n_cols);
  gl::DotAcc d01[4] = {gl::dot_zero(), gl::dot_zero(), gl::dot_zero(), gl::dot_zero()};
  gl::DotAcc d2[4] = {gl::dot_zero(), gl::dot_zero(), gl::dot_zero(), gl::dot_zero()};
  fri_combine_accumulate(a, c0, c1, pos, d01, d2);
  fri_combine_store(d01, d2, a.partial + (uint64_t)(a.chunk_base + chunk) * 6 * n, n, pos);
}
struct GPtrs {
  uint64_t* g[bpg::MAX_LOCKSTEP];
};
__global__ void __launch_bounds__(256) fri_combine_all_kernel(bpg::ArgPtr<bpg::CombineMulti> args, GPtrs gp) {
  BPG_ARG_BATCH(bpg::CombineMulti, args);
  if (gridDim.x * gridDim.z <= 64) __builtin_amdgcn_s_setprio(3);
  const bpg::CombineMulti& m = batch[blockIdx.z];
  uint64_t* __restrict__ g = gp.g[blockIdx.z];
  const uint32_t pos = blockIdx.x * blockDim.x + threadIdx.x, n = 1u << m.a[0].log_n;
  if (pos >= n) return;
  gl::DotAcc d01[4] = {gl::dot_zero(), gl::dot_zero(), gl::dot_zero(), gl::dot_zero()};
  gl::DotAcc d2[4] = {gl::dot_zero(), gl::dot_zero(), gl::dot_zero(), gl::dot_zero()};
  for (uint32_t o = 0; o < m.n_oracles; o++) fri_combine_accumulate(m.a[o], 0, m.a[o].n_cols, pos, d01, d2);
  fri_combine_store(d01, d2, g, n, pos);
}
__global__ void __launch_bounds__(256) fri_combine_partial_kernel(bpg::CombineArgs a) {
  if (gridDim.x * gridDim.y * gridDim.z <= 64) __builtin_amdgcn_s_setprio(3);
  fri_combine_partial_body(a, blockIdx.y);
}
__global__ void __launch_bounds__(256) fri_combine_partial_multi_kernel(bpg::ArgPtr<bpg::CombineMulti> args) {
  BPG_ARG_BATCH(bpg::CombineMulti, args);
  if (gridDim.x * gridDim.y * gridDim.z <= 64) __builtin_amdgcn_s_setprio(3);
  const bpg::CombineMulti& m = batch[blockIdx.z];
  uint32_t o = 0;
#pragma unroll
  for (int k = 1; k < 4; k++)
    if (k < (int)m.n_oracles && blockIdx.y >= m.a[k].chunk_base) o = k;
  fri_combine_partial_body(m.a[o], blockIdx.y - m.a[o].chunk_base);
}
__global__ void __launch_bounds__(256)
fri_combine_reduce_kernel(bpg::ArgPtr<bpg::CombineReduceArgs> args, uint32_t n_chunks, uint32_t log_n) {
  BPG_ARG_BATCH(bpg::CombineReduceArgs, args);
  if (gridDim.x * gridDim.y * gridDim.z <= 64) __builtin_amdgcn_s_setprio(3);
  const uint64_t* __restrict__ partial = batch[blockIdx.z].partial;
  uint64_t* __restrict__ g = batch[blockIdx.z].g;
  const uint32_t pos = blockIdx.x * blockDim.x + threadIdx.x, n = 1u << log_n;
  if (pos >= n) return;
  uint64_t acc = 0;
  for (uint32_t c = 0; c < n_chunks; c++) acc = gl::addc(acc, partial[((uint64_t)c * 6 + blockIdx.y) * n + pos]);
  g[(uint64_t)blockIdx.y * n + pos] = acc;
}
__global__ void __launch_bounds__(256) fri_quotient_values_kernel(bpg::ArgPtr<bpg::FriInitArgs> args) {
  BPG_ARG_BATCH(bpg::FriInitArgs, args);
  if (gridDim.x * gridDim.y * gridDim.z <= 64) __builtin_amdgcn_s_setprio(3);
  const bpg::FriInitArgs& a = batch[blockIdx.z];
  const uint64_t rows = (uint64_t)1 << (a.log_n + a.rate_bits);
  const uint64_t pos = blockIdx.x * (uint64_t)blockDim.x + threadIdx.x;
  if (pos >= rows) return;
  const uint32_t t = (uint32_t)(pos >> a.log_n), m = (uint32_t)(pos & ((1u << a.log_n) - 1));
  const uint64_t x = gl::mulc(a.g_t[t], root_pow(a.tw_n, a.log_n, m));
  const Ext d0 = gl::sub(gl::ext(x), a.z[0]), d1 = gl::sub(gl::ext(x), a.z[1]), d2 = gl::sub(gl::ext(x), a.z[2]);
  const Ext d01 = gl::mul(d0, d1);
  const Ext all_inv = gl::inv(gl::mul(d01, d2));
  const Ext i2 = gl::mul(all_inv, d01), i01 = gl::mul(all_inv, d2);
  const Ext den_inv[3] = {gl::mul(i01, d1), gl::mul(i01, d0), i2};
  Ext sum = gl::ext(0);
#pragma unroll
  for (int b = 0; b < 3; b++) {
    const Ext gv{a.glde[(2 * b) * rows + pos], a.glde[(2 * b + 1) * rows + pos]};
    const Ext num = gl::sub(gv, a.y[b]);
    sum = gl::add(sum, gl::mul(a.alpha_shift[b], gl::mul(num, den_inv[b])));
  }
  a.out[2 * pos] = sum.c0;
  a.out[2 * pos + 1] = sum.c1;
}

__global__ void __launch_bounds__(256) fri_layer_leaf_kernel(bpg::ArgPtr<bpg::FriLayerArgs> args) {
  BPG_ARG_BATCH(bpg::FriLayerArgs, args);
  if (gridDim.x * gridDim.y * gridDim.z <= 64) __builtin_amdgcn_s_setprio(3);
  const bpg::FriLayerArgs& a = batch[blockIdx.z];
  const uint32_t log_q = a.log_nl - a.arity_bits;
  const uint64_t n_leaves = (uint64_t)1 << (log_q + a.rate_bits);
  const uint64_t id = blockIdx.x * (uint64_t)blockDim.x + threadIdx.x;
  if (id >= n_leaves) return;
  const uint32_t t = (uint32_t)(id >> log_q), m0 = (uint32_t)(id & ((1u << log_q) - 1));
  const uint64_t base = ((uint64_t)t << a.log_nl) + m0;
  const uint32_t arity = 1u << a.arity_bits;
  uint64_t s[12];
#pragma unroll
  for (int k = 0; k < 12; k++) s[k] = 0;
  for (uint32_t j = 0; j < arity; j += 4) {
#pragma unroll
    for (int u = 0; u < 4; u++) {
      const uint32_t jj = gl::bitrev(j + u, a.arity_bits);
      const uint64_t p = base + ((uint64_t)jj << log_q);
      s[2 * u] = a.values[2 * p];
      s[2 * u + 1] = a.values[2 * p + 1];
    }
    poseidon::permute(s);
  }
  const uint64_t leaf = gl::bitrev((uint32_t)(t + ((uint64_t)m0 << a.rate_bits)), log_q + a.rate_bits);
#pragma unroll
  for (int k = 0; k < 4; k++) a.digests[leaf * 4 + k] = gl::canon(s[k]);
}
__global__ void __launch_bounds__(256) fri_layer_leaf_quad_kernel(bpg::ArgPtr<bpg::FriLayerArgs> args) {
  BPG_ARG_BATCH(bpg::FriLayerArgs, args);
  if (gridDim.x * gridDim.y * gridDim.z <= 64) __builtin_amdgcn_s_setprio(3);
  const bpg::FriLayerArgs& a = batch[blockIdx.z];
  __shared__ uint64_t rc[360];
  for (uint32_t i = threadIdx.x; i < 360; i += blockDim.x) rc[i] = poseidon::RC[i];
  __syncthreads();
  const uint32_t log_q = a.log_nl - a.arity_bits;
  const uint64_t n_leaves = (uint64_t)1 << (log_q + a.rate_bits);
  const uint64_t id = (blockIdx.x * (uint64_t)blockDim.x + threadIdx.x) >> 2;
  if (id >= n_leaves) return;
  const poseidon::QuadCtx qc = poseidon::quad_ctx();
  const uint32_t t = (uint32_t)(id >> log_q), m0 = (uint32_t)(id & ((1u << log_q) - 1));
  const uint64_t base = ((uint64_t)t << a.log_nl) + m0;
  const uint32_t arity = 1u << a.arity_bits, u = qc.q >> 1, comp = qc.q & 1;
  uint64_t e[3] = {0, 0, 0};
  for (uint32_t j = 0; j < arity; j += 4) {
    const uint64_t p0 = base + ((uint64_t)gl::bitrev(j + u, a.arity_bits) << log_q);
    const uint64_t p1 = base + ((uint64_t)gl::bitrev(j + 2 + u, a.arity_bits) << log_q);
    e[0] = a.values[2 * p0 + comp];
    e[1] = a.values[2 * p1 + comp];
    poseidon::permute_quad(e, qc, rc);
  }
  const uint64_t leaf = gl::bitrev((uint32_t)(t + ((uint64_t)m0 << a.rate_bits)), log_q + a.rate_bits);
  a.digests[leaf * 4 + qc.q] = gl::canon(e[0]);
}
template <int NS>
__global__ void __launch_bounds__(256) fri_layer_leaf_mx_kernel(bpg::ArgPtr<bpg::FriLayerArgs> args) {
  BPG_ARG_BATCH(bpg::FriLayerArgs, args);
  if (gridDim.x * gridDim.z <= 64) __builtin_amdgcn_s_setprio(3);
  const bpg::FriLayerArgs& a = batch[blockIdx.z];
  __shared__ __attribute__((aligned(16))) uint32_t cin[poseidon::mx::CIN_WORDS];
  poseidon::mx::build_cin(cin);
  __syncthreads();
  const poseidon::mx::Ctx c = poseidon::mx::make_ctx(cin);
  const uint32_t log_q = a.log_nl - a.arity_bits;
  const uint64_t n_leaves = (uint64_t)1 << (log_q + a.rate_bits);
  const uint64_t id0 = ((uint64_t)blockIdx.x * 4 + (threadIdx.x >> 6)) * (16 * NS) + (threadIdx.x & 15);
  const uint32_t arity = 1u << a.arity_bits, u = c.kb >> 1, comp = c.kb & 1;
  uint64_t base[NS], e[NS][3];
#pragma unroll
  for (int m = 0; m < NS; m++) {
    const uint64_t id = id0 + 16 * m < n_leaves ? id0 + 16 * m : n_leaves - 1;
    const uint32_t t = (uint32_t)(id >> log_q), m0 = (uint32_t)(id & ((1u << log_q) - 1));
    base[m] = ((uint64_t)t << a.log_nl) + m0;
    e[m][0] = e[m][1] = e[m][2] = 0;
  }
  for (uint32_t j = 0; j < arity; j += 4) {
    const uint64_t o0 = (uint64_t)gl::bitrev(j + u, a.arity_bits) << log_q;
    const uint64_t o1 = (uint64_t)gl::bitrev(j + 2 + u, a.arity_bits) << log_q;
#pragma unroll
    for (int m = 0; m < NS; m++) {
      e[m][0] = a.values[2 * (base[m] + o0) + comp];
      e[m][1] = a.values[2 * (base[m] + o1) + comp];
    }
    poseidon::mx::permute<NS>(e, c);
  }
#pragma unroll
  for (int m = 0; m < NS; m++) {
    const uint64_t id = id0 + 16 * m;
    if (id < n_leaves) {
      const uint32_t t = (uint32_t)(id >> log_q), m0 = (uint32_t)(id & ((1u << log_q) - 1));
      const uint64_t leaf = gl::bitrev((uint32_t)(t + ((uint64_t)m0 << a.rate_bits)), log_q + a.rate_bits);
      a.digests[leaf * 4 + c.kb] = gl::canon(e[m][0]);
    }
  }
}
__global__ void __launch_bounds__(256) fri_fold_kernel(bpg::ArgPtr<bpg::FriLayerArgs> args) {
  BPG_ARG_BATCH(bpg::FriLayerArgs, args);
  if (gridDim.x * gridDim.y * gridDim.z <= 64) __builtin_amdgcn_s_setprio(3);
  const bpg::FriLayerArgs& a = batch[blockIdx.z];
  const uint32_t log_q = a.log_nl - a.arity_bits;
  const uint64_t n_out = (uint64_t)1 << (log_q + a.rate_bits);
  const uint64_t id = blockIdx.x * (uint64_t)blockDim.x + threadIdx.x;
  if (id >= n_out) return;
  const uint32_t t = (uint32_t)(id >> log_q), m0 = (uint32_t)(id & ((1u << log_q) - 1));
  const uint64_t base = ((uint64_t)t << a.log_nl) + m0;
  const uint64_t x_inv = gl::mulc(a.g_t_inv[t], root_pow(a.tw_nl_inv, a.log_nl, m0));
  uint64_t c0[16], c1[16];
#pragma unroll
  for (int j = 0; j < 16; j++) {
    const uint64_t p = base + ((uint64_t)j << log_q);
    c0[j] = a.values[2 * p];
    c1[j] = a.values[2 * p + 1];
  }
#pragma unroll
  for (int s = 0; s < 4; s++) {
    const int half = 8 >> s;
#pragma unroll
    for (int k0 = 0; k0 < 8; k0 += 2) {
      uint64_t d[4], w[4], r[4];
      int mm[2];
#pragma unroll
      for (int i = 0; i < 2; i++) {
        const int k = k0 + i, m = (k / half) * 2 * half + (k % half);
        mm[i] = m;
        const uint64_t wv = a.wa_inv_pow[(m & (half - 1)) << s];
        const uint64_t x0 = c0[m], x1 = c1[m], y0 = c0[m + half], y1 = c1[m + half];
        c0[m] = gl::addc(x0, y0);
        c1[m] = gl::addc(x1, y1);
        d[2 * i] = gl::subc(x0, y0);
        d[2 * i + 1] = gl::subc(x1, y1);
        w[2 * i] = wv;
        w[2 * i + 1] = wv;
      }
      if (half == 1) {
#pragma unroll
        for (int i = 0; i < 4; i++) r[i] = d[i];
      } else {
        gl::mul_n<4>(d, w, r);
#pragma unroll
        for (int i = 0; i < 4; i++) r[i] = gl::canon(r[i]);
        __builtin_amdgcn_sched_barrier(0);
      }
#pragma unroll
      for (int i = 0; i < 2; i++) {
        c0[mm[i] + half] = r[2 * i];
        c1[mm[i] + half] = r[2 * i + 1];
      }
    }
  }
  const Ext bx = gl::scale(a.beta, x_inv);
  Ext acc = gl::ext(0);
#pragma unroll
  for (int i = 15; i >= 0; i--) {
    const int slot = ((i & 1) << 3) | ((i & 2) << 1) | ((i & 4) >> 1) | ((i & 8) >> 3);
    acc = gl::add(gl::mul(acc, bx), Ext{c0[slot], c1[slot]});
  }
  acc = gl::scale(acc, a.arity_inv);
  a.out[2 * id] = acc.c0;
  a.out[2 * id + 1] = acc.c1;
}

__global__ void __launch_bounds__(256) pow_grind_kernel(bpg::ArgPtr<bpg::PowArgs> args, unsigned long long* result) {
  BPG_ARG_BATCH(bpg::PowArgs, args);
  const bpg::PowArgs& a = batch[blockIdx.z];
  result += blockIdx.z;
  if (__hip_atomic_load(result, __ATOMIC_RELAXED, __HIP_MEMORY_SCOPE_AGENT) < a.base + blockIdx.x * (uint64_t)blockDim.x) return;
  const uint64_t cand = a.base + blockIdx.x * (uint64_t)blockDim.x + threadIdx.x;
  uint64_t s[12];
#pragma unroll
  for (int k = 0; k < 12; k++) s[k] = a.state[k];
  s[a.pos] = cand;
  poseidon::permute(s);
  if ((gl::canon(s[7]) >> (64 - a.bits)) == 0) atomicMin(result, (unsigned long long)cand);
}
template <bool GR>
__global__ void __launch_bounds__(256) __attribute__((amdgpu_waves_per_eu(3)))
pow_grind_mx_kernel(bpg::ArgPtr<bpg::PowArgs> args, unsigned long long* result, const uint32_t* __restrict__ gtab) {
  BPG_ARG_BATCH(bpg::PowArgs, args);
  const bpg::PowArgs& a = batch[blockIdx.z];
  result += blockIdx.z;
  __shared__ uint32_t beaten;
  if (threadIdx.x == 0)
    beaten = __hip_atomic_load(result, __ATOMIC_RELAXED, __HIP_MEMORY_SCOPE_AGENT) < a.base + (uint64_t)blockIdx.x * 256;
  __syncthreads();
  if (beaten) return;
  __shared__ __attribute__((aligned(16))) uint32_t cin[GR ? poseidon::mx::CIN_GROUPED_WORDS : poseidon::mx::CIN_WORDS];
  __shared__ __attribute__((aligned(16))) uint32_t gt[GR ? poseidon::mx::grp::TABLE_WORDS : 4];
  if constexpr (GR) {
    poseidon::mx::build_cin_grouped(cin);
    poseidon::mx::grp::load_tables(gt, gtab);
  } else {
    poseidon::mx::build_cin(cin);
  }
  __syncthreads();
  const poseidon::mx::Ctx c = poseidon::mx::make_ctx(cin);
  const uint64_t cand0 = a.base + ((uint64_t)blockIdx.x * 4 + (threadIdx.x >> 6)) * 64 + (threadIdx.x & 15);
  uint64_t e[4][3];
#pragma unroll
  for (int s = 0; s < 3; s++) {
    uint64_t w = a.state[4 * s];
#pragma unroll
    for (int q = 1; q < 4; q++) w = c.kb == (uint32_t)q ? a.state[4 * s + q] : w;
    const bool mine = c.kb + 4 * s == a.pos;
#pragma unroll
    for (int m = 0; m < 4; m++) e[m][s] = mine ? cand0 + 16 * m : w;
  }
  if constexpr (GR) poseidon::mx::permute_grouped(e, c, gt, gtab);
  else poseidon::mx::permute<4>(e, c);
  if (c.kb == 3) {
#pragma unroll
    for (int m = 0; m < 4; m++)
      if ((gl::canon(e[m][1]) >> (64 - a.bits)) == 0) atomicMin(result, (unsigned long long)(cand0 + 16 * m));
  }
}

__global__ void __launch_bounds__(256) query_initial_kernel(bpg::ArgPtr<bpg::QueryArgs> args) {
  if (gridDim.x * gridDim.y * gridDim.z <= 64) __builtin_amdgcn_s_setprio(3);
  const bpg::QueryArgs& a = *(const bpg::QueryArgs*)args;
  const uint32_t b = blockIdx.x / a.n_queries, q = blockIdx.x % a.n_queries, o = blockIdx.y;
  const uint64_t x = a.x_index[blockIdx.x];
  const bpg::QueryOracle& orc = a.proof[b].oracle[o];
  const uint32_t log_rows = a.log_n + a.rate_bits;
  const uint32_t i = gl::bitrev((uint32_t)x, log_rows);
  const uint64_t pos = ((uint64_t)(i & ((1u << a.rate_bits) - 1)) << a.log_n) + (i >> a.rate_bits);
  uint64_t* out = a.proof[b].out;
  if (o == 0 && threadIdx.x == 0) out[(uint64_t)q * a.query_words] = x;
  uint64_t* w = out + (uint64_t)q * a.query_words + orc.out_offset;
  for (uint32_t c = threadIdx.x; c < orc.n_cols; c += blockDim.x) w[c] = orc.lde[(uint64_t)c * orc.stride + pos];
  w += orc.n_cols;
  const uint32_t depth = log_rows - a.cap_height;
  for (uint32_t k = threadIdx.x; k < depth * 4; k += blockDim.x) {
    const uint32_t lvl = k >> 2;
    const uint64_t off = ((uint64_t)2 << log_rows) - ((uint64_t)2 << (log_rows - lvl));
    w[k] = orc.digests[(off + ((x >> lvl) ^ 1)) * 4 + (k & 3)];
  }
  if (q == 0 && o == a.leaf_oracle && a.proof[b].first_leaf && threadIdx.x < 4) a.proof[b].first_leaf[threadIdx.x] = orc.digests[x * 4 + threadIdx.x];
}
__global__ void __launch_bounds__(64) query_layers_kernel(bpg::ArgPtr<bpg::QueryLayerArgs> args) {
  if (gridDim.x * gridDim.y * gridDim.z <= 64) __builtin_amdgcn_s_setprio(3);
  const bpg::QueryLayerArgs& a = *(const bpg::QueryLayerArgs*)args;
  const uint32_t b = blockIdx.x / a.n_queries, q = blockIdx.x % a.n_queries, l = blockIdx.y;
  const bpg::QueryLayer& L = a.proof[b].layer[l];
  const uint32_t arity = 1u << a.arity_bits;
  const uint64_t leaf = a.x_index[blockIdx.x] >> (a.arity_bits * (l + 1));
  const uint32_t log_q = L.log_nl - a.arity_bits, log_leaves = log_q + a.rate_bits;
  const uint32_t c = gl::bitrev((uint32_t)leaf, log_leaves);
  const uint32_t t = c & ((1u << a.rate_bits) - 1), m0 = c >> a.rate_bits;
  const uint64_t base = ((uint64_t)t << L.log_nl) + m0;
  uint64_t* w = a.proof[b].out + (uint64_t)q * a.query_words + L.out_offset;
  for (uint32_t k = threadIdx.x; k < 2 * arity; k += blockDim.x) {
    const uint32_t jj = gl::bitrev(k >> 1, a.arity_bits);
    w[k] = L.values[2 * (base + ((uint64_t)jj << log_q)) + (k & 1)];
  }
  w += 2 * arity;
  const uint32_t depth = log_leaves - a.cap_height;
  for (uint32_t k = threadIdx.x; k < depth * 4; k += blockDim.x) {
    const uint32_t lvl = k >> 2;
    const uint64_t off = ((uint64_t)2 << log_leaves) - ((uint64_t)2 << (log_leaves - lvl));
    w[k] = L.digests[(off + ((leaf >> lvl) ^ 1)) * 4 + (k & 3)];
  }
}

}

namespace bpg {

int launch_synth_constants(uint64_t* d_out, uint32_t log_n, uint32_t n_const, uint64_t seed, hipStream_t st) {
  uint64_t total = (uint64_t)n_const << log_n;
  if (!total) return BP_OK;
  synth_const_kernel<<<ceil_div(total, 256), 256, 0, st>>>(d_out, log_n, n_const, seed);
  BPG_LAUNCH_CHECK();
  return BP_OK;
}
#define BPG_ARG_BLOCKS(var, a, n, st)                                               \
  const std::remove_cv_t<std::remove_reference_t<decltype((a)[0])>>* var##_dev = nullptr; \
  if (int rc_ = arg_put(st, &(a)[0], n, &var##_dev)) return rc_;                    \
  const auto var = arg_ptr(var##_dev)
template <class... A>
constexpr bool blocks_fit() { return ((sizeof(A) <= ARG_BLOCK_MAX) && ...); }
static_assert(blocks_fit<SynthTraceArgs, PlonkTraceArgs, AuxArgs, QuotArgs, AlphaTabArgs, ChunkArgs, PowerVecArgs, AlphaPowArgs, OpenMulti,
                         CombineMulti, CombineReduceArgs, FriInitArgs, FriLayerArgs, PowArgs>(),
              "arg_ring.hpp: ARG_BLOCK_MAX bounds every per-proof argument block");
static_assert(sizeof(QueryArgs) <= ARG_WHOLE_MAX && sizeof(QueryLayerArgs) <= ARG_WHOLE_MAX, "arg_ring.hpp: ARG_WHOLE_MAX");
static int check_batch(uint32_t batch) {
  return batch >= 1 && batch <= MAX_LOCKSTEP ? BP_OK : fail(BP_ERR_INVALID_INPUT, "batch of %u proofs: 1..%u can be proved in lock-step", batch, MAX_LOCKSTEP);
}
int launch_synth_trace(const SynthTraceArgs* a, uint32_t batch, uint32_t log_n, uint32_t n_cols, uint32_t n_const,
                       uint32_t deg_pow, hipStream_t st) {
  if (int rc = check_batch(batch)) return rc;
  dim3 grid(ceil_div((uint64_t)1 << log_n, 256), n_cols / 4 + 1, batch);
  BPG_ARG_BLOCKS(ab, a, batch, st);
  synth_trace_kernel<<<grid, 256, 0, st>>>(ab, log_n, n_cols, n_const, deg_pow);
  BPG_LAUNCH_CHECK();
  return BP_OK;
}
int launch_air_trace(uint32_t air_id, uint64_t* d_trace, const uint64_t* d_inputs, uint32_t log_n, uint64_t seed, hipStream_t st,
                     uint32_t sponge_row_limit) {
  const unsigned gx = ceil_div((uint64_t)1 << log_n, 256);
  switch (air_id) {
    case air::KECCAK_F: keccak_trace_kernel<<<dim3(gx, 6), 256, 0, st>>>(d_trace, d_inputs, log_n, seed); break;
    case air::LOGIC: logic_trace_kernel<<<dim3(gx, 2), 256, 0, st>>>(d_trace, d_inputs, log_n, seed); break;
    case air::MEMORY: memory_trace_kernel<<<gx, 256, 0, st>>>(d_trace, d_inputs, log_n, seed); break;
    case air::ARITHMETIC: arithmetic_trace_kernel<<<gx, 256, 0, st>>>(d_trace, d_inputs, log_n, seed); break;
    case air::BYTE_PACKING: byte_packing_trace_kernel<<<gx, 256, 0, st>>>(d_trace, d_inputs, log_n, seed); break;
    case air::KECCAK_SPONGE: keccak_sponge_trace_kernel<<<dim3(gx, 3), 256, 0, st>>>(d_trace, d_inputs, log_n, seed, sponge_row_limit); break;
    case air::ARITHMETIC_MUL: arithmetic_mul_trace_kernel<<<gx, 256, 0, st>>>(d_trace, d_inputs, log_n, seed); break;
    default: return fail(BP_ERR_INVALID_INPUT, "launch_air_trace: AIR %u has a witness entry of its own (launch_synth_trace, launch_plonk_trace) or none", air_id);
  }
  BPG_LAUNCH_CHECK();
  return BP_OK;
}
int launch_keccak_inputs_from_sponge(const uint64_t* d_sponge_trace, uint32_t sponge_log_n, uint64_t* d_inputs, uint32_t n_perms,
                                     uint64_t seed, hipStream_t st) {
  if (!n_perms) return BP_OK;
  keccak_inputs_from_sponge_kernel<<<ceil_div(n_perms, 256), 256, 0, st>>>(d_sponge_trace, sponge_log_n, d_inputs, n_perms, seed);
  BPG_LAUNCH_CHECK();
  return BP_OK;
}
int launch_logic_inputs_from_sponge(const uint64_t* d_sponge_trace, uint32_t sponge_log_n, uint32_t covered, const uint64_t* d_given,
                                    uint32_t n_given, uint64_t* d_inputs, uint32_t n_logic, uint64_t seed, hipStream_t st) {
  if (5ull * covered > n_logic || covered > (1u << sponge_log_n))
    return fail(BP_ERR_INVALID_INPUT, "the logic table (%u rows) cannot hold five operations for each of %u sponge rows", n_logic, covered);
  logic_inputs_from_sponge_kernel<<<ceil_div(n_logic, 256), 256, 0, st>>>(d_sponge_trace, sponge_log_n, covered, d_given, n_given, d_inputs,
                                                                           n_logic, seed);
  BPG_LAUNCH_CHECK();
  return BP_OK;
}
int launch_memory_inputs_from_byte_packing(const uint64_t* d_pack_trace, uint32_t pack_log_n, uint64_t* d_log, uint32_t n_mem,
                                           hipStream_t st) {
  memory_inputs_from_byte_packing_kernel<<<ceil_div(n_mem, 256), 256, 0, st>>>(d_pack_trace, pack_log_n, d_log, n_mem);
  BPG_LAUNCH_CHECK();
  return BP_OK;
}
int launch_lookup_filter(uint32_t air_id, uint64_t* d_trace, uint32_t log_n, const uint64_t* flag_a, const uint64_t* flag_b,
                         uint32_t n_flags, hipStream_t st) {
  if (!flag_a || !n_flags) return BP_OK;
  if (air_id == air::KECCAK_F) {
    if (!flag_b) return fail(BP_ERR_INVALID_INPUT, "launch_lookup_filter: the Keccak-f table's filter needs both flag columns of the sponge table");
    keccak_lookup_filter_kernel<<<ceil_div((uint64_t)1 << log_n, 256), 256, 0, st>>>(d_trace, log_n, flag_a, flag_b, n_flags);
  } else if (air_id == air::MEMORY) {
    memory_lookup_filter_kernel<<<ceil_div(n_flags, 256), 256, 0, st>>>(d_trace, log_n, flag_a, n_flags);
  } else if (air_id == air::LOGIC) {
    if (!flag_b) return fail(BP_ERR_INVALID_INPUT, "launch_lookup_filter: the logic table's filter needs both flag columns of the sponge table");
    logic_lookup_filter_kernel<<<ceil_div(5ull * n_flags, 256), 256, 0, st>>>(d_trace, log_n, flag_a, flag_b, n_flags);
  } else {
    return fail(BP_ERR_INVALID_INPUT, "launch_lookup_filter: AIR %u is not a looked table", air_id);
  }
  BPG_LAUNCH_CHECK();
  return BP_OK;
}
int launch_plonk_constants(uint64_t* d_out, uint32_t log_n, uint64_t seed, const air::plonk::Layout& lay, hipStream_t st) {
  if (lay.pi_len < 1 || lay.pi_len > air::plonk::MAX_PI)
    return fail(BP_ERR_INVALID_INPUT, "a recursion circuit hashes a public-input list of 1..%u words: got %u", air::plonk::MAX_PI, lay.pi_len);
  if (log_n >= 4 && log_n < 31 && !air::plonk::layout_ok(lay, 1u << log_n))
    return fail(BP_ERR_INVALID_INPUT, "plonk circuit layout: %u paths of %u levels (at most %u Merkle rows), their words at %u.. of a "
                "list of %u, leaves of %u words (0 or more than 8; at most %u leaf rows), and one arithmetic group must fit 2^%u rows",
                lay.n_paths, lay.depth, air::plonk::MERKLE_ROWS_MAX, lay.path_pi0, lay.pi_len, lay.leaf_len, air::plonk::LEAF_ROWS_MAX, log_n);
  if (log_n < 5) return fail(BP_ERR_INVALID_INPUT, "the plonk circuit needs 32 rows: the Poseidon rows (4..19) and one arithmetic group");
  const uint64_t* tw_n = nullptr;
  if (int rc = get_table(0, log_n, 0, &tw_n)) return rc;
  plonk_constants_kernel<<<dim3(ceil_div((uint64_t)1 << log_n, 256), air::plonk::N_CONST), 256, 0, st>>>(d_out, log_n, seed, tw_n, lay);
  BPG_LAUNCH_CHECK();
  return BP_OK;
}
int launch_plonk_trace(const PlonkTraceArgs* a, uint32_t batch, uint32_t log_n, hipStream_t st) {
  if (int rc = check_batch(batch)) return rc;
  for (uint32_t b = 0; b < batch; b++)
    if (!a[b].hash_rows || a[b].n_hash_rows < 1 || a[b].n_hash_rows > air::plonk::HASH_ROWS_MAX)
      return fail(BP_ERR_INVALID_INPUT, "launch_plonk_trace: the witness of the hash rows is missing (poseidon_hash_rows)");
  uint32_t region = 0;
  for (uint32_t b = 0; b < batch; b++) {
    if (a[b].arith_row0 < air::plonk::MERKLE_ROW0 || (a[b].arith_row0 & 3) || a[b].arith_row0 + 4 > (1ull << log_n) ||
        air::plonk::MERKLE_ROW0 + a[b].n_merkle_rows > a[b].arith_row0 || a[b].n_merkle_rows > air::plonk::MERKLE_ROWS_MAX + air::plonk::LEAF_ROWS_MAX)
      return fail(BP_ERR_INVALID_INPUT, "launch_plonk_trace: %u Merkle rows and first arithmetic row %u do not fit 2^%u rows", a[b].n_merkle_rows, a[b].arith_row0, log_n);
    region = std::max(region, a[b].arith_row0 - air::plonk::HASH_ROW0);
  }
  BPG_ARG_BLOCKS(ab, a, batch, st);
  plonk_trace_kernel<<<dim3(ceil_div((((uint64_t)1 << log_n) / 4) * air::plonk::N_SLOTS, 256), 1, batch), 256, 0, st>>>(ab, log_n);
  BPG_LAUNCH_CHECK();
  plonk_hash_rows_kernel<<<dim3(1, region, batch), 256, 0, st>>>(ab, log_n);
  BPG_LAUNCH_CHECK();
  return BP_OK;
}
int launch_port_products(const AuxArgs* a, uint32_t batch, uint32_t air_id, uint32_t log_n, uint64_t trace_stride, hipStream_t st) {
  if (int rc = check_batch(batch)) return rc;
  const uint32_t n_aux = air::any_n_aux(air::Shape{air_id, 0, 0, 1});
  const auto program = air::prog::find(air_id);
  const uint32_t log_ports = program ? program->log_ports() : 0;
  const uint32_t threads = std::max(64u, std::min(1024u, 1u << log_n));
  if (!log_ports) {
    for (uint32_t b = 0; b < batch; b++)
      if (int rc = launch_port_terms(a[b], air_id, log_n, trace_stride, nullptr, st)) return rc;
    BPG_ARG_BLOCKS(ab, a, batch, st);
    KernelTimer kt(PROF_AUX, st, 16.0 * (double)((uint64_t)1 << log_n) * n_aux * batch, true);
    BPG_LAUNCH_TIMED(kt, aux_suffix_product_kernel<air::ctl::TERMS_IN_COLUMN>, dim3(n_aux, 1, batch), threads, 0, st, ab, log_n, 0u);
    BPG_LAUNCH_CHECK();
    return BP_OK;
  }
  struct PoleWords {
    uint64_t* d = nullptr;
    ~PoleWords() { (void)hipFree(d); }
  } pole;
  const size_t words = 2 * (size_t)air::prog::MAX_PORTS;
  BPG_HIP(hipMalloc(reinterpret_cast<void**>(&pole.d), batch * words * 8));
  BPG_HIP(hipMemsetAsync(pole.d, 0xFF, batch * words * 8, st));
  for (uint32_t b = 0; b < batch; b++)
    if (int rc = launch_port_terms(a[b], air_id, log_n, trace_stride, pole.d + b * words, st)) return rc;
  {
    BPG_ARG_BLOCKS(ab, a, batch, st);
    KernelTimer kt(PROF_AUX, st, 16.0 * (double)((uint64_t)1 << log_n) * n_aux * batch, true);
    BPG_LAUNCH_TIMED(kt, port_running_columns_kernel, dim3(n_aux, 1, batch), threads, 0, st, ab, log_n, log_ports);
    BPG_LAUNCH_CHECK();
  }
  uint64_t found[MAX_LOCKSTEP * 2 * air::prog::MAX_PORTS];
  BPG_HIP(hipMemcpyAsync(found, pole.d, batch * words * 8, hipMemcpyDeviceToHost, st));
  BPG_HIP(hipStreamSynchronize(st));
  for (uint32_t b = 0; b < batch; b++)
    for (uint32_t k = 0; k < n_aux; k++)
      if (found[b * words + k] != ~0ULL)
        return fail(BP_ERR_VERIFY, "AIR program 0x%08x: log port %u, challenge set %u, row %llu: gamma + v = 0 where the filter is not 0, "
                    "so the port's running sum has no value (a pole)", air_id, k / 2, k % 2, (unsigned long long)found[b * words + k]);
  return BP_OK;
}
int launch_aux(const AuxArgs* a, uint32_t batch, uint32_t air_id, uint32_t n_cols, uint32_t log_n, hipStream_t st) {
  const air::Shape shape{air_id, n_cols, 0, 1};
  const uint32_t n_aux = air::any_n_aux(shape), p0 = air::ctl::first_product(air_id);
  if (!n_aux) return BP_OK;
  if (int rc = check_batch(batch)) return rc;
  if (air::prog::is_registered(air_id) && n_aux > 1) return launch_port_products(a, batch, air_id, log_n, (uint64_t)1 << log_n, st);
  BPG_ARG_BLOCKS(ab, a, batch, st);
  if (air_id == air::KECCAK_F) {
    keccak_ctl_helpers_kernel<<<dim3(ceil_div((uint64_t)1 << log_n, 256), 1, batch), 256, 0, st>>>(ab, log_n);
    BPG_LAUNCH_CHECK();
  }
  uint32_t threads = (1u << log_n) < 1024 ? (1u << log_n) : 1024;
  if (threads < 64) threads = 64;
  if (air_id == air::PLONK) {
    for (uint32_t b = 0; b < batch; b++)
      if (!a[b].consts) return fail(BP_ERR_INVALID_INPUT, "the plonk AIR needs the circuit's constant columns (the sigmas) for its copy products");
    const uint64_t* tw_n = nullptr;
    if (int rc = get_table(0, log_n, 0, &tw_n)) return rc;
    const uint32_t gx = ceil_div((uint64_t)1 << log_n, 256);
    plonk_chunk_ratios_kernel<<<dim3(gx, 2, batch), 256, 0, st>>>(ab, log_n, tw_n);
    BPG_LAUNCH_CHECK();
    aux_suffix_product_kernel<air::PLONK><<<dim3(2, 1, batch), threads, 0, st>>>(ab, log_n, n_cols);
    BPG_LAUNCH_CHECK();
    plonk_partial_products_kernel<<<dim3(gx, 18, batch), 256, 0, st>>>(ab, log_n);
    BPG_LAUNCH_CHECK();
    return BP_OK;
  }
  const dim3 grid(n_aux - p0, 1, batch);
  const uint32_t reads = air_id < air::COUNT ? air::DESC[air_id].aux_reads : 0;
  KernelTimer kt(PROF_AUX, st, 8.0 * (double)((uint64_t)1 << log_n) * (reads + 1) * (n_aux - p0) * batch, true);
  air::dispatch(reads ? air_id : air::ARITHMETIC, [&](auto A) {
    if constexpr (air::DESC[A.value].aux_reads || A.value == air::ARITHMETIC)
      BPG_LAUNCH_TIMED(kt, aux_suffix_product_kernel<A.value>, grid, threads, 0, st, ab, log_n, n_cols);
  });
  BPG_LAUNCH_CHECK();
  return BP_OK;
}
int get_hash_fold_table(const uint64_t** out) {
  static std::mutex mu;
  static std::map<int, const uint64_t*> tabs;
  int dev = 0;
  BPG_HIP(hipGetDevice(&dev));
  std::lock_guard<std::mutex> lk(mu);
  auto it = tabs.find(dev);
  if (it == tabs.end()) {
    static const std::vector<uint64_t> host = air::plonk::hash_fold_table();
    if (host.empty()) return fail(BP_ERR_DEVICE, "the Poseidon gate's fold table does not fit its workgroups");
    uint64_t* d = nullptr;
    BPG_HIP(hipMalloc(reinterpret_cast<void**>(&d), host.size() * 8));
    BPG_HIP(hipMemcpy(d, host.data(), host.size() * 8, hipMemcpyHostToDevice));
    it = tabs.emplace(dev, d).first;
  }
  *out = it->second;
  return BP_OK;
}
static int launch_alpha_tables(const QuotArgs* qs, uint32_t batch, const QuotCoset& coset, hipStream_t st) {
  const QuotArgs& q = qs[0];
  CosetTab ct;
  for (int t = 0; t < 16; t++) { ct.v[t] = coset.g_t[t]; ct.v[16 + t] = coset.zh_t[t]; ct.v[32 + t] = coset.zh_inv_t[t]; }
  const uint64_t* fold = nullptr;
  if (q.side_rows) {
    if (q.n_constraints < air::plonk::HASH_FOLD_T_MIN || q.n_constraints > air::plonk::HASH_FOLD_T_MAX)
      return fail(BP_ERR_INVALID_INPUT, "the Poseidon gate's fold weights are made for a constraint list of %u..%u entries, not %u",
                  air::plonk::HASH_FOLD_T_MIN, air::plonk::HASH_FOLD_T_MAX, q.n_constraints);
    if (int rc = get_hash_fold_table(&fold)) return rc;
  }
  AlphaTabArgs tabs[MAX_LOCKSTEP];
  for (uint32_t b = 0; b < batch; b++) tabs[b] = AlphaTabArgs{const_cast<uint64_t*>(qs[b].apow), qs[b].alpha0, qs[b].alpha1};
  BPG_ARG_BLOCKS(at, tabs, batch, st);
  alpha_table_kernel<<<dim3(fold ? air::plonk::HASH_FOLD_BLOCKS : ceil_div(q.n_constraints, 256), 2, batch), 256, 0, st>>>(at, q.n_constraints, ct, fold);
  BPG_LAUNCH_CHECK();
  return BP_OK;
}
int debug_plonk_hash_fold(uint64_t alpha0, uint64_t alpha1, uint64_t* d_out, hipStream_t st) {
  QuotArgs q{};
  q.n_constraints = air::plonk::N_CONSTRAINTS + air::ctl::PLONK_N_CONSTRAINTS;
  q.side_rows = 1;
  q.alpha0 = alpha0; q.alpha1 = alpha1;
  struct Table {
    uint64_t* d = nullptr;
    ~Table() { (void)hipFree(d); }
  } tab;
  BPG_HIP(hipMalloc(reinterpret_cast<void**>(&tab.d), quotient_table_words(q) * 8));
  q.apow = tab.d;
  if (int rc = launch_alpha_tables(&q, 1, QuotCoset{}, st)) return rc;
  BPG_HIP(hipMemcpyAsync(d_out, tab.d + 2 * (size_t)q.n_constraints + 48, air::plonk::HASH_FOLD_WORDS * 8, hipMemcpyDeviceToDevice, st));
  BPG_HIP(hipStreamSynchronize(st));
  return BP_OK;
}
int launch_quotient(const QuotArgs* qs, uint32_t batch, const QuotCoset& coset, hipStream_t st) {
  if (int rc = check_batch(batch)) return rc;
  const QuotArgs& q = qs[0];
  const uint64_t rows = (uint64_t)1 << (q.log_n + q.rate_bits);
  if (q.n_ports && q.side_rows) return fail(BP_ERR_INVALID_INPUT, "launch_quotient: lookup ports and a side row in one table");
  if (int rc = launch_alpha_tables(qs, batch, coset, st)) return rc;
  const uint32_t n_units = q.n_air_units + q.n_ctl_units, wg_rows = ceil_div(n_units, q.units_per_wg);
  BPG_ARG_BLOCKS(qb, qs, batch, st);
  if (q.n_ports)
    if (int rc = launch_beta_tables(qb_dev, batch, st)) return rc;
  dim3 g1(ceil_div(rows, 256), wg_rows, batch);
  KernelTimer kt(PROF_K5 + (q.air_id < air::COUNT ? q.air_id : 0), st, 8.0 * (double)rows * ((double)q.n_cols + q.n_aux + q.n_const + 2) * batch, true);
  if (bpg::air::prog::is_registered(q.air_id)) {
    if (int rc = launch_quotient_program(qb_dev, q, g1, kt, st)) return rc;
  } else air::dispatch(q.air_id, [&](auto A) { BPG_LAUNCH_TIMED(kt, quotient_air_kernel<A.value>, g1, 256, 0, st, qb); });
  kt.stop();
  if (q.side_rows) {
    BPG_LAUNCH_CHECK();
    KernelTimer kh(PROF_K5 + q.air_id, st, 0.0, true);
    BPG_LAUNCH_TIMED(kh, quotient_plonk_hash_kernel, dim3(ceil_div(rows, 256), 1, batch), 256, 0, st, qb, wg_rows);
  }
  BPG_LAUNCH_CHECK();
  if (wg_rows + q.side_rows > 1) {
    quotient_sum_kernel<<<dim3(ceil_div(rows, 256), 2, batch), 256, 0, st>>>(qb, wg_rows + q.side_rows);
    BPG_LAUNCH_CHECK();
  }
  return BP_OK;
}
int launch_quotient_chunks(const ChunkArgs* c, uint32_t batch, hipStream_t st) {
  if (int rc = check_batch(batch)) return rc;
  dim3 grid(ceil_div((uint64_t)1 << c[0].log_n, 256), 2, batch);
  BPG_ARG_BLOCKS(cb, c, batch, st);
  quotient_chunks_kernel<<<grid, 256, 0, st>>>(cb);
  BPG_LAUNCH_CHECK();
  return BP_OK;
}
int launch_power_vectors(const PowerVecArgs* a, uint32_t batch, uint32_t log_n, uint32_t n_points, hipStream_t st) {
  if (int rc = check_batch(batch)) return rc;
  if (n_points < 1 || n_points > 3) return fail(BP_ERR_INVALID_INPUT, "launch_power_vectors: 1..3 points");
  dim3 grid(ceil_div((uint64_t)1 << log_n, 256), n_points, batch);
  BPG_ARG_BLOCKS(ab, a, batch, st);
  power_vector_kernel<<<grid, 256, 0, st>>>(ab, log_n);
  BPG_LAUNCH_CHECK();
  return BP_OK;
}
int launch_alpha_pows(const AlphaPowArgs* a, uint32_t batch, uint32_t count, hipStream_t st) {
  if (int rc = check_batch(batch)) return rc;
  BPG_ARG_BLOCKS(ab, a, batch, st);
  alpha_pows_kernel<<<dim3(ceil_div(count, 256), 1, batch), 256, 0, st>>>(ab, count);
  BPG_LAUNCH_CHECK();
  return BP_OK;
}
int launch_openings(const uint64_t* d_coeffs, uint64_t stride, uint32_t log_n, uint32_t n_cols,
                    const uint64_t* d_pw, uint32_t n_points, uint64_t* d_out, hipStream_t st) {
  if (!n_cols) return BP_OK;
  openings_kernel<<<n_cols, 256, 0, st>>>(d_coeffs, stride, log_n, d_pw, n_points, d_out);
  BPG_LAUNCH_CHECK();
  return BP_OK;
}
int launch_openings_multi(const OpenMulti* m, uint32_t batch, hipStream_t st) {
  if (int rc = check_batch(batch)) return rc;
  const uint32_t total = m[0].first_col[m[0].n_segs];
  if (!total) return BP_OK;
  BPG_ARG_BLOCKS(mb, m, batch, st);
  KernelTimer kt(PROF_OPENINGS, st, 8.0 * (double)((uint64_t)1 << m[0].log_n) * total * batch, true);
  BPG_LAUNCH_TIMED(kt, openings_multi_kernel, dim3(total, 1, batch), 256, 0, st, mb);
  BPG_LAUNCH_CHECK();
  return BP_OK;
}
static double combine_bytes(const CombineMulti& m) {
  double cols = 6;
  for (uint32_t o = 0; o < m.n_oracles; o++) cols += m.a[o].n_cols;
  return 8.0 * (double)((uint64_t)1 << m.a[0].log_n) * cols;
}
int launch_combine_partial_multi(const CombineMulti* m, uint32_t batch, uint32_t total_chunks, hipStream_t st) {
  if (!total_chunks) return BP_OK;
  if (int rc = check_batch(batch)) return rc;
  dim3 grid(ceil_div((uint64_t)1 << m[0].a[0].log_n, 256), total_chunks, batch);
  BPG_ARG_BLOCKS(mb, m, batch, st);
  KernelTimer kt(PROF_FRI_COMBINE, st, combine_bytes(m[0]) * batch, true);
  BPG_LAUNCH_TIMED(kt, fri_combine_partial_multi_kernel, grid, 256, 0, st, mb);
  BPG_LAUNCH_CHECK();
  return BP_OK;
}
int launch_combine_all(const CombineMulti* m, uint32_t batch, uint64_t* const* d_g, hipStream_t st) {
  if (int rc = check_batch(batch)) return rc;
  GPtrs gp{};
  for (uint32_t b = 0; b < batch; b++) gp.g[b] = d_g[b];
  BPG_ARG_BLOCKS(mb, m, batch, st);
  KernelTimer kt(PROF_FRI_COMBINE, st, combine_bytes(m[0]) * batch, true);
  BPG_LAUNCH_TIMED(kt, fri_combine_all_kernel, dim3(ceil_div((uint64_t)1 << m[0].a[0].log_n, 256), 1, batch), 256, 0, st, mb, gp);
  BPG_LAUNCH_CHECK();
  return BP_OK;
}
int launch_combine_reduce(const CombineReduceArgs* a, uint32_t batch, uint32_t n_chunks, uint32_t log_n, hipStream_t st) {
  if (int rc = check_batch(batch)) return rc;
  dim3 grid(ceil_div((uint64_t)1 << log_n, 256), 6, batch);
  BPG_ARG_BLOCKS(ab, a, batch, st);
  fri_combine_reduce_kernel<<<grid, 256, 0, st>>>(ab, n_chunks, log_n);
  BPG_LAUNCH_CHECK();
  return BP_OK;
}
int launch_fri_init(const FriInitArgs* a, uint32_t batch, hipStream_t st) {
  if (int rc = check_batch(batch)) return rc;
  uint64_t rows = (uint64_t)1 << (a[0].log_n + a[0].rate_bits);
  BPG_ARG_BLOCKS(ab, a, batch, st);
  fri_quotient_values_kernel<<<dim3(ceil_div(rows, 256), 1, batch), 256, 0, st>>>(ab);
  BPG_LAUNCH_CHECK();
  return BP_OK;
}
uint64_t quad_threshold();
bool poseidon_mx();
int mx_sets(uint64_t n);
int launch_fri_layer_leaves(const FriLayerArgs* as, uint32_t batch, hipStream_t st) {
  if (int rc = check_batch(batch)) return rc;
  const FriLayerArgs& a = as[0];
  uint64_t n = (uint64_t)1 << (a.log_nl - a.arity_bits + a.rate_bits);
  BPG_ARG_BLOCKS(ab, as, batch, st);
  if (const int ns = mx_sets(n * batch)) {
    if (ns == 4) fri_layer_leaf_mx_kernel<4><<<dim3(ceil_div(n, 256), 1, batch), 256, 0, st>>>(ab);
    else if (ns == 2) fri_layer_leaf_mx_kernel<2><<<dim3(ceil_div(n, 128), 1, batch), 256, 0, st>>>(ab);
    else fri_layer_leaf_mx_kernel<1><<<dim3(ceil_div(n, 64), 1, batch), 256, 0, st>>>(ab);
  } else if (n * batch < quad_threshold()) fri_layer_leaf_quad_kernel<<<dim3(ceil_div(n * 4, 256), 1, batch), 256, 0, st>>>(ab);
  else fri_layer_leaf_kernel<<<dim3(ceil_div(n, 256), 1, batch), 256, 0, st>>>(ab);
  BPG_LAUNCH_CHECK();
  return BP_OK;
}
int launch_fri_fold(const FriLayerArgs* a, uint32_t batch, hipStream_t st) {
  if (int rc = check_batch(batch)) return rc;
  uint64_t n = (uint64_t)1 << (a[0].log_nl - a[0].arity_bits + a[0].rate_bits);
  BPG_ARG_BLOCKS(ab, a, batch, st);
  KernelTimer kt(PROF_FRI_FOLD, st, 16.0 * (double)n * ((1 << a[0].arity_bits) + 1) * batch, true);
  BPG_LAUNCH_TIMED(kt, fri_fold_kernel, dim3(ceil_div(n, 256), 1, batch), 256, 0, st, ab);
  BPG_LAUNCH_CHECK();
  return BP_OK;
}
int launch_pow(const PowArgs* a, uint32_t batch, uint32_t n_candidates, unsigned long long* d_result, hipStream_t st) {
  if (int rc = check_batch(batch)) return rc;
  BPG_ARG_BLOCKS(ab, a, batch, st);
  const dim3 grid(n_candidates / 256, 1, batch);
  if (poseidon_mx()) {
    const uint32_t* gtab = group_tables();
    if (gtab) pow_grind_mx_kernel<true><<<grid, 256, 0, st>>>(ab, d_result, gtab);
    else pow_grind_mx_kernel<false><<<grid, 256, 0, st>>>(ab, d_result, nullptr);
  } else
    pow_grind_kernel<<<grid, 256, 0, st>>>(ab, d_result);
  BPG_LAUNCH_CHECK();
  return BP_OK;
}
int launch_query_initial(const QueryArgs& a, uint32_t batch, uint32_t n_oracles, hipStream_t st) {
  if (int rc = check_batch(batch)) return rc;
  if (!a.n_queries || a.n_queries * batch > MAX_BATCH_QUERIES) return fail(BP_ERR_INVALID_INPUT, "query launch: %u x %u indices, at most %u", a.n_queries, batch, MAX_BATCH_QUERIES);
  dim3 grid(a.n_queries * batch, n_oracles);
  const QueryArgs* ab = nullptr;
  if (int rc = arg_put(st, &a, 1, &ab)) return rc;
  query_initial_kernel<<<grid, 256, 0, st>>>(arg_ptr(ab));
  BPG_LAUNCH_CHECK();
  return BP_OK;
}
int launch_query_layers(const QueryLayerArgs& a, uint32_t batch, uint32_t n_layers, hipStream_t st) {
  if (!n_layers) return BP_OK;
  if (int rc = check_batch(batch)) return rc;
  if (!a.n_queries || a.n_queries * batch > MAX_BATCH_QUERIES || n_layers > MAX_FRI_LAYERS)
    return fail(BP_ERR_INVALID_INPUT, "query launch: %u x %u indices, %u layers", a.n_queries, batch, n_layers);
  dim3 grid(a.n_queries * batch, n_layers);
  const QueryLayerArgs* ab = nullptr;
  if (int rc = arg_put(st, &a, 1, &ab)) return rc;
  query_layers_kernel<<<grid, 64, 0, st>>>(arg_ptr(ab));
  BPG_LAUNCH_CHECK();
  return BP_OK;
}

}
```

### proof_protocol_decoder_amd/csrc/stark_kernels.hpp

```cpp
#pragma once
#include <hip/hip_runtime.h>
#include <cstdint>
#include "air.hpp"
#include "gl.hpp"

namespace bpg {

struct Ctl {
  uint64_t v[4];
  uint64_t pub[4] = {0, 0, 0, 0};
};

constexpr uint32_t MAX_BATCH = 8;
constexpr uint32_t MAX_LOCKSTEP = 24;
int arg_ring_put(hipStream_t st, const void* blocks, size_t bytes, const void** dev);
template <class A>
using ArgPtr = const __attribute__((address_space(4))) A*;
template <class A>
inline ArgPtr<A> arg_ptr(const A* dev) { return (ArgPtr<A>)dev; }
#define BPG_ARG_BATCH(T, args) const T* __restrict__ batch = (const T*)(args)
template <class A>
inline int arg_put(hipStream_t st, const A* a, uint32_t n, const A** dev) {
  const void* d = nullptr;
  const int rc = arg_ring_put(st, a, sizeof(A) * n, &d);
  *dev = static_cast<const A*>(d);
  return rc;
}

struct QuotArgs {
  const uint64_t *trace_lde, *aux_lde, *const_lde;
  uint64_t trace_stride, aux_stride, const_stride;
  uint64_t *partial, *qvals;
  const uint64_t* tw_n;
  const uint64_t* apow;
  uint32_t air_id, log_n, rate_bits, n_cols, n_const, n_aux, deg_pow;
  uint32_t n_air_constraints, n_constraints, n_air_units, n_ctl_units, aux_per_unit, units_per_wg;
  uint32_t side_rows;
  uint32_t n_ports;
  uint64_t alpha0, alpha1, g, g_inv, n_inv;
  Ctl ctl;
};
inline size_t quotient_table_words(const QuotArgs& q) {
  return 2 * (size_t)q.n_constraints + 48 + (q.n_ports ? 256 : 0) + (q.side_rows ? air::plonk::HASH_FOLD_WORDS : 0);
}
struct QuotCoset {
  uint64_t g_t[16], zh_t[16], zh_inv_t[16];
};
struct SynthTraceArgs {
  uint64_t* trace;
  const uint64_t* consts;
  uint64_t seed;
};
struct AuxArgs {
  const uint64_t* trace;
  uint64_t* aux;
  Ctl ctl;
  const uint64_t* consts = nullptr;
};
struct PowerVecArgs {
  uint64_t* out;
  gl::Ext z[3];
};
struct AlphaPowArgs {
  uint64_t* out;
  gl::Ext alpha;
};
struct CombineReduceArgs {
  const uint64_t* partial;
  uint64_t* g;
};
struct ChunkArgs {
  const uint64_t* e;
  const uint64_t* inv_scale;
  uint64_t* out;
  uint64_t out_stride;
  uint32_t log_n, rate_bits;
  uint64_t wr_inv_pow[16];
  uint64_t chunk_scale[16];
};
struct CombineArgs {
  const uint64_t* coeffs;
  uint64_t stride;
  uint32_t log_n, n_cols, cols_per_chunk, chunk_base;
  int32_t exp_base[3];
  const uint64_t* alpha_pows;
  uint64_t* partial;
};
struct CombineMulti {
  CombineArgs a[4];
  uint32_t n_oracles;
};
struct OpenMulti {
  const uint64_t* coeffs[5];
  const uint64_t* pw[5];
  uint64_t* out[5];
  uint32_t first_col[6], n_points[5];
  uint64_t stride;
  uint32_t log_n, n_segs;
};
struct FriInitArgs {
  const uint64_t* glde;
  uint64_t* out;
  const uint64_t* tw_n;
  uint32_t log_n, rate_bits;
  uint64_t g_t[16];
  gl::Ext y[3], z[3], alpha_shift[3];
};
struct FriLayerArgs {
  const uint64_t* values;
  uint64_t* out;
  uint64_t* digests;
  const uint64_t* tw_nl_inv;
  uint32_t log_nl, rate_bits, arity_bits;
  uint64_t g_t_inv[16];
  uint64_t wa_inv_pow[16];
  uint64_t arity_inv;
  gl::Ext beta;
};
struct PowArgs {
  uint64_t state[12];
  uint64_t base;
  uint32_t pos, bits;
};
struct QueryOracle {
  const uint64_t *lde, *digests;
  uint64_t stride;
  uint32_t n_cols, out_offset;
};
constexpr uint32_t MAX_BATCH_QUERIES = 672;
struct QueryProof {
  uint64_t* out;
  QueryOracle oracle[4];
  uint64_t* first_leaf = nullptr;
};
struct QueryArgs {
  uint64_t x_index[MAX_BATCH_QUERIES];
  uint64_t query_words;
  uint32_t log_n, rate_bits, cap_height, n_queries;
  uint32_t leaf_oracle = 0;
  QueryProof proof[MAX_LOCKSTEP];
};
struct QueryLayer {
  const uint64_t *values, *digests;
  uint32_t log_nl, out_offset;
};
constexpr uint32_t MAX_FRI_LAYERS = 8;
struct QueryLayerProof {
  uint64_t* out;
  QueryLayer layer[MAX_FRI_LAYERS];
};
struct QueryLayerArgs {
  uint64_t x_index[MAX_BATCH_QUERIES];
  uint64_t query_words;
  uint32_t rate_bits, cap_height, arity_bits, n_queries;
  QueryLayerProof proof[MAX_LOCKSTEP];
};

int launch_synth_constants(uint64_t* d_out, uint32_t log_n, uint32_t n_const, uint64_t seed, hipStream_t st);
int launch_synth_trace(const SynthTraceArgs* a, uint32_t batch, uint32_t log_n, uint32_t n_cols, uint32_t n_const,
                       uint32_t deg_pow, hipStream_t st);
inline int launch_synth_trace(uint64_t* d_trace, const uint64_t* d_consts, uint32_t log_n, uint32_t n_cols,
                              uint32_t n_const, uint32_t deg_pow, uint64_t seed, hipStream_t st) {
  const SynthTraceArgs a{d_trace, d_consts, seed};
  return launch_synth_trace(&a, 1, log_n, n_cols, n_const, deg_pow, st);
}
int launch_air_trace(uint32_t air_id, uint64_t* d_trace, const uint64_t* d_inputs, uint32_t log_n, uint64_t seed, hipStream_t st,
                     uint32_t sponge_row_limit = ~0u);
int launch_keccak_inputs_from_sponge(const uint64_t* d_sponge_trace, uint32_t sponge_log_n, uint64_t* d_inputs, uint32_t n_perms,
                                     uint64_t seed, hipStream_t st);
int launch_logic_inputs_from_sponge(const uint64_t* d_sponge_trace, uint32_t sponge_log_n, uint32_t covered, const uint64_t* d_given,
                                    uint32_t n_given, uint64_t* d_inputs, uint32_t n_logic, uint64_t seed, hipStream_t st);
int launch_memory_inputs_from_byte_packing(const uint64_t* d_pack_trace, uint32_t pack_log_n, uint64_t* d_log, uint32_t n_mem,
                                           hipStream_t st);
int launch_lookup_filter(uint32_t air_id, uint64_t* d_trace, uint32_t log_n, const uint64_t* flag_a, const uint64_t* flag_b,
                         uint32_t n_flags, hipStream_t st);
int launch_aux(const AuxArgs* a, uint32_t batch, uint32_t air_id, uint32_t n_cols, uint32_t log_n, hipStream_t st);
int launch_plonk_constants(uint64_t* d_out, uint32_t log_n, uint64_t seed, const air::plonk::Layout& lay, hipStream_t st);
struct PlonkTraceArgs {
  uint64_t* trace;
  const uint64_t* consts;
  uint64_t seed, pub[4];
  const uint64_t* hash_rows;
  uint32_t n_hash_rows;
  uint32_t n_merkle_rows = 0, arith_row0 = (air::plonk::MERKLE_ROW0 + 3) & ~3u;
};
int launch_plonk_trace(const PlonkTraceArgs* a, uint32_t batch, uint32_t log_n, hipStream_t st);
int launch_quotient(const QuotArgs* q, uint32_t batch, const QuotCoset& coset, hipStream_t st);
inline int launch_quotient(const QuotArgs& q, const QuotCoset& coset, hipStream_t st) { return launch_quotient(&q, 1, coset, st); }
struct KernelTimer;
int launch_quotient_program(const QuotArgs* qb, const QuotArgs& q0, dim3 grid, KernelTimer& kt, hipStream_t st);
int get_hash_fold_table(const uint64_t** out);
int debug_plonk_hash_fold(uint64_t alpha0, uint64_t alpha1, uint64_t* d_out, hipStream_t st);
int launch_beta_tables(const QuotArgs* qb, uint32_t batch, hipStream_t st);
int launch_port_terms(const AuxArgs& a, uint32_t air_id, uint32_t log_n, uint64_t trace_stride, uint64_t* d_pole, hipStream_t st);
int launch_port_products(const AuxArgs* a, uint32_t batch, uint32_t air_id, uint32_t log_n, uint64_t trace_stride, hipStream_t st);
int launch_quotient_chunks(const ChunkArgs* c, uint32_t batch, hipStream_t st);
int launch_power_vectors(const PowerVecArgs* a, uint32_t batch, uint32_t log_n, uint32_t n_points, hipStream_t st);
inline int launch_power_vectors(uint64_t* d_out, uint32_t log_n, gl::Ext z0, gl::Ext z1, uint32_t n_points,
                                hipStream_t st, gl::Ext z2 = gl::Ext{1, 0}) {
  const PowerVecArgs a{d_out, {z0, z1, z2}};
  return launch_power_vectors(&a, 1, log_n, n_points, st);
}
int launch_alpha_pows(const AlphaPowArgs* a, uint32_t batch, uint32_t count, hipStream_t st);
int launch_openings(const uint64_t* d_coeffs, uint64_t stride, uint32_t log_n, uint32_t n_cols,
                    const uint64_t* d_pw, uint32_t n_points, uint64_t* d_out, hipStream_t st);
int launch_openings_multi(const OpenMulti* m, uint32_t batch, hipStream_t st);
int launch_combine_partial_multi(const CombineMulti* m, uint32_t batch, uint32_t total_chunks, hipStream_t st);
int launch_combine_all(const CombineMulti* m, uint32_t batch, uint64_t* const* d_g, hipStream_t st);
int launch_combine_reduce(const CombineReduceArgs* a, uint32_t batch, uint32_t n_chunks, uint32_t log_n, hipStream_t st);
int launch_fri_init(const FriInitArgs* a, uint32_t batch, hipStream_t st);
int launch_fri_layer_leaves(const FriLayerArgs* a, uint32_t batch, hipStream_t st);
int launch_fri_fold(const FriLayerArgs* a, uint32_t batch, hipStream_t st);
inline int launch_fri_fold(const FriLayerArgs& a, hipStream_t st) { return launch_fri_fold(&a, 1, st); }
int launch_pow(const PowArgs* a, uint32_t batch, uint32_t n_candidates, unsigned long long* d_result, hipStream_t st);
inline int launch_pow(const PowArgs& a, uint32_t n_candidates, unsigned long long* d_result, hipStream_t st) {
  return launch_pow(&a, 1, n_candidates, d_result, st);
}
int launch_query_initial(const QueryArgs& a, uint32_t batch, uint32_t n_oracles, hipStream_t st);
int launch_query_layers(const QueryLayerArgs& a, uint32_t batch, uint32_t n_layers, hipStream_t st);

int init_ntt_kernels();
int get_table(int kind, uint32_t log_n, uint32_t rate_bits, const uint64_t** out);
int intt_nat2br(const uint64_t* in, uint64_t in_stride, uint64_t* out, uint64_t out_stride, uint32_t log_n,
                uint32_t n_cols, bool inverse, hipStream_t st);
int ntt_br2nat(const uint64_t* in, uint64_t in_stride, uint64_t* out, uint64_t out_stride, uint64_t coset_stride,
               uint32_t log_n, uint32_t n_cols, uint32_t n_cosets, const uint64_t* scale, bool inverse,
               hipStream_t st);
const uint32_t* group_tables();
int merkle_upper_levels(uint64_t* d_digests, uint32_t log_leaves, uint32_t cap_height, hipStream_t st,
                        uint64_t* mirror, bool* mirrored, uint32_t batch = 1, uint64_t dig_bstride = 0);
int merkle_commit_cols(const uint64_t* d_lde, uint64_t lde_stride, uint32_t n_cols, uint32_t log_n, uint32_t rate_bits,
                       uint32_t cap_height, uint64_t* d_digests, hipStream_t st, uint64_t* mirror, bool* mirrored,
                       uint32_t batch = 1, uint64_t lde_bstride = 0, uint64_t dig_bstride = 0);

}
```

### proof_protocol_decoder_amd/ops.py

```python
import contextlib
import ctypes as C

import numpy as np
import torch

from ._lib import KNOBS, StarkCfg, call_for_buffer, check, lib, own

NTT_FWD_BR2NAT, NTT_INV_NAT2BR, NTT_FWD_NAT, NTT_INV_NAT = 0, 1, 2, 3


def _stream():
    return torch.cuda.current_stream().cuda_stream


_tuned_active = False


@contextlib.contextmanager
def tuned(**knobs):
    global _tuned_active
    if _tuned_active:
        raise RuntimeError("ops.tuned() inside ops.tuned(): name all the knobs in one call")
    unknown = sorted(set(knobs) - set(KNOBS))
    if unknown:
# ... 258 lines not shown
        return "AirCheck(air %d: %d violated rows, first %s)" % (self.air_id, self.n_violated_rows, self.rows[:8])


def _check_cfg(air_id, n_cols, n_const, log_n, deg_pow):
    d = air_describe(air_id, n_cols, n_const, deg_pow)
    if d.fixed_n_cols:
        deg_pow = 3 if d.degree > 3 else 1
    return stark_cfg(log_n, n_cols, n_const=n_const, deg_pow=deg_pow, rate_bits=1 if deg_pow == 1 else 3)


def _check_shapes(n, consts, pub):
    if n < 1 or n & (n - 1):
        raise ValueError("a trace has 2^log_n rows: got %d" % n)
    if consts is not None and (len(consts.shape) != 2 or consts.shape[1] != n):
        raise ValueError("constants must be [n_const, %d]: got %s" % (n, tuple(consts.shape)))
    if pub is not None and len(pub) != 4:
        raise ValueError("four public inputs: got %d" % len(pub))


def _check_call(fn, air_id, cfg, trace_ptr, stride, consts_ptr, pub, max_rows, max_viol, *stream):
    from ._lib import AirViolation
    n_rows, n_viol = C.c_uint64(), C.c_uint32()
    rows = (C.c_uint32 * max(1, max_rows))()
    viol = (AirViolation * max(1, max_viol))()
    pub_arr = (C.c_uint64 * 4)(*[int(x) for x in pub]) if pub is not None else None
    check(fn(air_id, C.byref(cfg), trace_ptr, stride, consts_ptr, pub_arr, max_rows, C.byref(n_rows), rows, viol, max_viol,
             C.byref(n_viol), *stream))
    got_rows = min(n_rows.value, max_rows)
    return AirCheck(air_id, n_rows.value, [int(rows[i]) for i in range(got_rows)],
                    [viol[i] for i in range(min(n_viol.value, max_viol))], n_viol.value)


def check_air_trace(air_id, trace, consts=None, pub=None, max_rows=16, max_viol=None, deg_pow=1):
    if not trace.is_cuda or trace.dtype != torch.int64 or trace.stride(1) != 1:
        raise ValueError("check_air_trace needs an int64 device tensor with contiguous columns")
    n_cols, n = trace.shape
    if consts is not None:
        _require_cuda(consts)
    _check_shapes(n, consts, pub)
    cfg = _check_cfg(air_id, n_cols, consts.shape[0] if consts is not None else 0, n.bit_length() - 1, deg_pow)
    return _check_call(own().bp_air_check_trace, air_id, cfg, trace.data_ptr(), trace.stride(0),
                       consts.data_ptr() if consts is not None else None, pub, max_rows,
                       4 * max_rows + 64 if max_viol is None else max_viol, _stream())


def check_air_trace_host(air_id, trace, consts=None, pub=None, max_rows=16, max_viol=None, deg_pow=1):
    trace = np.asarray(trace)
    if trace.dtype != np.uint64 or trace.strides[1] != 8:
        raise ValueError("check_air_trace_host needs a uint64 array with contiguous columns")
    n_cols, n = trace.shape
    if consts is not None:
        consts = np.ascontiguousarray(consts, dtype=np.uint64)
    _check_shapes(n, consts, pub)
    cfg = _check_cfg(air_id, n_cols, consts.shape[0] if consts is not None else 0, n.bit_length() - 1, deg_pow)
    return _check_call(own().bp_air_check_trace_host, air_id, cfg, trace.ctypes.data, trace.strides[0] // 8,
                       consts.ctypes.data if consts is not None else None, pub, max_rows,
                       4 * max_rows + 64 if max_viol is None else max_viol)


def fri_fold(values, log_nl, rate_bits, shift, beta, arity_bits=4):
    _require_cuda(values)
    out = torch.empty(((1 << (log_nl - arity_bits)) << rate_bits, 2), dtype=torch.int64, device=values.device)
    check(own().bp_fri_fold(values.data_ptr(), log_nl, rate_bits, arity_bits, int(shift),
                            (C.c_uint64 * 2)(int(beta[0]), int(beta[1])), out.data_ptr(), _stream()))
    return out


def openings(coeffs, z0, z1=None):
    _require_cuda(coeffs)
    n_cols, n = coeffs.shape
    pw = torch.empty(4 * n, dtype=torch.int64, device=coeffs.device)
    out = torch.zeros((n_cols, 4), dtype=torch.int64, device=coeffs.device)
    a0 = (C.c_uint64 * 2)(int(z0[0]), int(z0[1]))
    a1 = (C.c_uint64 * 2)(int(z1[0]), int(z1[1])) if z1 is not None else None
    check(own().bp_openings(coeffs.data_ptr(), n, n.bit_length() - 1, n_cols, a0, a1, pw.data_ptr(), out.data_ptr(),
                            _stream()))
    return out


def pow_grind(state, pos, bits):
    nonce = C.c_uint64()
    check(own().bp_pow_grind((C.c_uint64 * 12)(*[int(x) for x in state]), pos, bits, C.byref(nonce), _stream()))
    return nonce.value


def merkle_commit(lde, log_n, rate_bits, cap_height):
    _require_cuda(lde)
    n_cols, rows = lde.shape
    assert rows == 1 << (log_n + rate_bits)
    words = own().bp_merkle_digest_words(log_n + rate_bits, cap_height)
    dig = torch.empty((words // 4, 4), dtype=torch.int64, device=lde.device)
    check(own().bp_merkle_commit(lde.data_ptr(), rows, n_cols, log_n, rate_bits, cap_height, dig.data_ptr(),
                                 _stream()))
    return dig


def stark_cfg(log_n, n_cols, n_const=0, deg_pow=1, rate_bits=1, cap_height=4, num_queries=84, pow_bits=16,
              arity_bits=4, final_poly_bits=5):
    return StarkCfg(log_n, n_cols, n_const, deg_pow, rate_bits, cap_height, num_queries, pow_bits, arity_bits,
                    final_poly_bits)


def _words(proof_bytes):
    return np.frombuffer(proof_bytes, dtype=np.uint64).copy()


def stark_prove_air(air_id, cfg, seed, const_seed=0, device=0):
    return _words(call_for_buffer(own().bp_stark_prove_air, air_id, C.byref(cfg), seed, const_seed, device))


def stark_prove_trace(air_id, cfg, trace, consts=None, pub=None, device=None):
    if not trace.is_cuda or trace.dtype != torch.int64 or trace.stride(1) != 1:
        raise ValueError("stark_prove_trace needs an int64 device tensor with contiguous columns")
    if consts is not None:
        _require_cuda(consts)
    _check_shapes(trace.shape[1], consts, pub)
    if trace.shape[0] != cfg.n_cols or trace.shape[1] != 1 << cfg.log_n:
        raise ValueError("the trace is %s, the configuration says [%d, %d]" % (tuple(trace.shape), cfg.n_cols, 1 << cfg.log_n))
    torch.cuda.synchronize(trace.device)
    pub_arr = (C.c_uint64 * 4)(*[int(x) for x in pub]) if pub is not None else None
    dev = trace.device.index if device is None else device
    return _words(call_for_buffer(own().bp_stark_prove_trace, air_id, C.byref(cfg), trace.data_ptr(), trace.stride(0),
                                  consts.data_ptr() if consts is not None else None, pub_arr, dev or 0))


def air_port_products(air_id, trace, ctl, consts=None, pub=None):
    if not trace.is_cuda or trace.dtype != torch.int64 or trace.stride(1) != 1:
        raise ValueError("air_port_products needs an int64 device tensor with contiguous columns")
    n_cols, n = trace.shape
    if consts is not None:
        _require_cuda(consts)
    _check_shapes(n, consts, pub)
    d = air_describe(air_id)
    cfg = _check_cfg(air_id, n_cols, consts.shape[0] if consts is not None else 0, n.bit_length() - 1, 1)
    out = torch.empty((d.n_aux, n), dtype=torch.int64, device=trace.device)
    pub_arr = (C.c_uint64 * 4)(*[int(x) for x in pub]) if pub is not None else None
    check(own().bp_air_port_products(air_id, C.byref(cfg), trace.data_ptr(), trace.stride(0),
                                     consts.data_ptr() if consts is not None else None, pub_arr,
                                     (C.c_uint64 * 4)(*[int(x) for x in ctl]), out.data_ptr(), _stream()))
    return out


def range_multiplicities(values, log_range, filter=None, out=None):
    from ._lib import BpgError
    if not values.is_cuda or values.dtype != torch.int64 or values.dim() != 2 or values.stride(1) != 1:
        raise ValueError("range_multiplicities needs a 2-d int64 device tensor with contiguous columns")
    n_cols, n_rows = values.shape
    if filter is not None:
        _require_cuda(filter)
        if filter.shape != (n_rows,):
            raise ValueError("the filter has one word per row")
    if out is None:
        out = torch.zeros(1 << log_range, dtype=torch.int64, device=values.device)
    _require_cuda(out)
    if out.shape != (1 << log_range,):
        raise ValueError("out holds 2^log_range words")
    first_bad = C.c_uint64()
    try:
        check(own().bp_range_multiplicities(values.data_ptr(), values.stride(0), n_cols, n_rows,
                                            filter.data_ptr() if filter is not None else None, log_range, out.data_ptr(),
                                            C.byref(first_bad), _stream()))
    except BpgError as e:
        e.first_bad = first_bad.value
        raise
    return out

# ... 125 lines not shown
```

Baseline: 39.52.

## Cut stream packets: keyed PoW mailbox, FRI final-layer mirroring, fused query kernel

Proof-of-work search now uses a keyed per-search candidate space with device tickets and writes results straight into a pinned mailbox. This removes the per-search memset and the device-to-host copy on each polling round. The final FRI layer is mirrored into pinned memory by the fold/init kernel, replacing explicit async copies, and the two query kernels are merged into one launch. Debug counters for copy/fill packets are added. In exchange the code gains complexity around key wraparound, ticket state and zero-copy host writes.

```diff
diff --git a/include/bpg.h b/include/bpg.h
--- a/include/bpg.h
+++ b/include/bpg.h
@@ -167,6 +167,8 @@
                 const uint64_t z1[2], uint64_t* d_pw_scratch, uint64_t* d_out, void* stream);
 
 int bp_pow_grind(const uint64_t state[12], uint32_t pos, uint32_t bits, uint64_t* nonce_out, void* stream);
+int bp_debug_pow_search(const uint64_t* states, const uint32_t* pos, uint32_t n, uint32_t bits, uint64_t* nonces_out, int device);
+int bp_debug_stream_packets(uint64_t out[2], int reset);
 
 typedef struct bp_stark_cfg {
   uint32_t log_n, n_cols, n_const, deg_pow, rate_bits, cap_height, num_queries, pow_bits, arity_bits,
diff --git a/proof_protocol_decoder_amd/_abi.py b/proof_protocol_decoder_amd/_abi.py
--- a/proof_protocol_decoder_amd/_abi.py
+++ b/proof_protocol_decoder_amd/_abi.py
@@ -210,6 +210,8 @@
     "bp_fri_fold": (i, [vp, u32, u32, u32, u64, u64p, vp, vp]),
     "bp_openings": (i, [vp, u64, u32, u32, u64p, u64p, vp, vp, vp]),
     "bp_pow_grind": (i, [u64p, u32, u32, u64p, vp]),
+    "bp_debug_pow_search": (i, [u64p, u32p, u32, u32, u64p, i]),
+    "bp_debug_stream_packets": (i, [u64p, i]),
     "bp_stark_prove_synthetic": (i, [_cfg, u64, u64, i] + _buf),
     "bp_stark_prove_air": (i, [u32, _cfg, u64, u64, i] + _buf),
     "bp_stark_prove_trace": (i, [u32, _cfg, vp, u64, vp, u64p, i] + _buf),
diff --git a/proof_protocol_decoder_amd/csrc/proofgen.cpp b/proof_protocol_decoder_amd/csrc/proofgen.cpp
--- a/proof_protocol_decoder_amd/csrc/proofgen.cpp
+++ b/proof_protocol_decoder_amd/csrc/proofgen.cpp
@@ -659,12 +659,12 @@
         if (n_ops * wds > pinned_words) return fail(BP_ERR_UNSUPPORTED, "too many logic operations for the input staging buffer");
         std::memcpy(pinned, wit->in[t], n_ops * wds * 8);
         d_given = d_in + (size_t)N * wds;
-        BPG_HIP(hipMemcpyAsync(d_given, pinned, n_ops * wds * 8, hipMemcpyHostToDevice, w.stream));
+        BPG_HIP(stream_copy(d_given, pinned, n_ops * wds * 8, hipMemcpyHostToDevice, w.stream));
       }
       if ((r = launch_logic_inputs_from_sponge(d_sponge, sponge_log_n, plan.logic_covered, given[t] ? d_given : nullptr, (uint32_t)n_ops,
                                                d_in, (uint32_t)N, seed, w.stream))) return r;
       if (given[t] && !d_given) {
-        BPG_HIP(hipMemsetAsync(d_in + covered * wds, 0, ((size_t)N - covered) * wds * 8, w.stream));
+        BPG_HIP(stream_fill(d_in + covered * wds, 0, ((size_t)N - covered) * wds * 8, w.stream));
       }
     } else if (given[t]) {
       const size_t words = cap * wds;
@@ -672,7 +672,7 @@
       if (!d_in) return fail(BP_ERR_DEVICE, "device arena exhausted for the witness data of table %s", TABLES[t].name);
       if (words > pinned_words) return fail(BP_ERR_UNSUPPORTED, "table %s too tall for the input staging buffer", TABLES[t].name);
       fill_table_inputs(t, N, wit->in[t], wit->n[t], pinned);
-      BPG_HIP(hipMemcpyAsync(d_in, pinned, words * 8, hipMemcpyHostToDevice, w.stream));
+      BPG_HIP(stream_copy(d_in, pinned, words * 8, hipMemcpyHostToDevice, w.stream));
     } else if (t == T_KECCAK && lookup_kf) {
       d_in = w.arena.alloc_words(cap * wds);
       if (!d_in) return fail(BP_ERR_DEVICE, "device arena exhausted for the Keccak-f table's inputs");
diff --git a/proof_protocol_decoder_amd/csrc/prover.cpp b/proof_protocol_decoder_amd/csrc/prover.cpp
--- a/proof_protocol_decoder_amd/csrc/prover.cpp
+++ b/proof_protocol_decoder_amd/csrc/prover.cpp
@@ -311,7 +311,15 @@
   BPG_HIP(hipHostGetDevicePointer(reinterpret_cast<void**>(&pinned_dev), pinned, 0));
   BPG_HIP(hipHostMalloc(reinterpret_cast<void**>(&hash_rows), MAX_LOCKSTEP * HASH_ROWS_WORDS * 8, hipHostMallocDefault));
   BPG_HIP(hipHostGetDevicePointer(reinterpret_cast<void**>(&hash_rows_dev), hash_rows, 0));
-  BPG_HIP(hipMalloc(reinterpret_cast<void**>(&d_pow_result), 8 * MAX_LOCKSTEP));
+  {
+    BPG_HIP(hipMalloc(reinterpret_cast<void**>(&d_pow_result), 12 * MAX_LOCKSTEP));
+    d_pow_tickets = reinterpret_cast<uint32_t*>(d_pow_result + MAX_LOCKSTEP);
+    uint64_t init[MAX_LOCKSTEP + MAX_LOCKSTEP / 2];
+    for (uint32_t k = 0; k < MAX_LOCKSTEP; k++) init[k] = ~0ULL;
+    for (uint32_t k = MAX_LOCKSTEP; k < MAX_LOCKSTEP + MAX_LOCKSTEP / 2; k++) init[k] = 0;
+    BPG_HIP(hipMemcpy(d_pow_result, init, sizeof(init), hipMemcpyHostToDevice));
+    pow_searches = 0;
+  }
   {
     void* dev = nullptr;
     BPG_HIP(hipHostMalloc(&args_mem, ARG_RING_BYTES, hipHostMallocDefault));
@@ -338,6 +346,7 @@
   sync_event = nullptr;
   pinned = nullptr;
   d_pow_result = nullptr;
+  d_pow_tickets = nullptr;
   stream = nullptr;
 }
 extern "C" int bp_host_wait_mode(int device);
@@ -464,7 +473,7 @@
 int Worker::d2h(uint64_t* host_dst, const uint64_t* dev_src, size_t words) {
   for (size_t off = 0; off < words; off += pinned_words) {
     size_t k = std::min(pinned_words, words - off);
-    BPG_HIP(hipMemcpyAsync(pinned, dev_src + off, k * 8, hipMemcpyDeviceToHost, stream));
+    BPG_HIP(stream_copy(pinned, dev_src + off, k * 8, hipMemcpyDeviceToHost, stream));
     TRY(wait());
     std::memcpy(host_dst + off, pinned, k * 8);
   }
@@ -510,7 +519,7 @@
                          &mirrored, batch, (uint64_t)n_cols * m, dw));
   if (!mirrored) {
     for (uint32_t b = 0; b < batch; b++)
-      BPG_HIP(hipMemcpyAsync(lane.pinned + mailbox_word + b * cw, digests + (b + 1) * dw - cw, cw * 8, hipMemcpyDeviceToHost,
+      BPG_HIP(stream_copy(lane.pinned + mailbox_word + b * cw, digests + (b + 1) * dw - cw, cw * 8, hipMemcpyDeviceToHost,
                              lane.stream));
   }
   *pc = PendingCommit{&lane, mailbox_word, d_in, coeffs, lde, digests, dw, cw, n_cols, batch, log_n, rate_bits, cap_height, from_coeffs};
@@ -594,6 +603,43 @@
   for (uint32_t k = 0; k < arity; k++) fa.wa_inv_pow[k] = gl::pow(wa_inv, k);
   fa.arity_inv = gl::inv(arity);
   return BP_OK;
+}
+
+std::atomic<uint64_t>* stream_packet_counts() {
+  static std::atomic<uint64_t> n[2];
+  return n;
+}
+
+int pow_search(const PowSearch& s, PowArgs* pa, uint32_t B, uint32_t bits, unsigned long long* res) {
+  if (B == 0 || B > MAX_LOCKSTEP || bits == 0 || bits > 40) return fail(BP_ERR_INVALID_INPUT, "proof of work: %u proofs, %u bits", B, bits);
+  constexpr uint64_t LIMIT = (uint64_t)1 << POW_CAND_BITS;
+  constexpr uint32_t MAX_LAUNCH = 1u << 20, KEYS = (1u << (64 - POW_CAND_BITS)) - 1;
+  if (*s.searches >= KEYS) {
+    BPG_HIP(stream_fill(s.d_result, 0xFF, 8 * MAX_LOCKSTEP, s.stream));
+    *s.searches = 0;
+  }
+  const uint64_t key = (uint64_t)(KEYS - 1 - *s.searches) << POW_CAND_BITS;
+  ++*s.searches;
+  const uint32_t batch0 = (uint32_t)std::min<uint64_t>(MAX_LAUNCH, std::max<uint64_t>(1u << 12, (uint64_t)1 << (bits - 1)));
+  uint32_t batch = batch0, n_batches = 0;
+  for (uint64_t base = 0;;) {
+    if (base + 4 * (uint64_t)MAX_LAUNCH > LIMIT) return fail(BP_ERR_DEVICE, "proof of work search exhausted");
+    for (int k = 0; k < 4; k++) {
+      if (++n_batches > 8) batch = std::min<uint32_t>(MAX_LAUNCH, batch * 2);
+      for (uint32_t b = 0; b < B; b++) { pa[b].base = base; pa[b].key = key; }
+      TRY(launch_pow(pa, B, batch, s.d_result, s.d_tickets, s.mailbox_dev, s.stream));
+      base += batch;
+    }
+    if (s.worker) TRY(s.worker->wait());
+    else BPG_HIP(hipStreamSynchronize(s.stream));
+    bool all = true;
+    for (uint32_t b = 0; b < B; b++) {
+      res[b] = reinterpret_cast<const volatile unsigned long long*>(s.mailbox)[b];
+      all = all && res[b] != ~0ULL;
+    }
+    if (all) return BP_OK;
+    if (s.worker && s.worker->aborted()) return fail(BP_ERR_ABORTED, "aborted during proof of work");
+  }
 }
 
 int stark_prove(Worker& w, const StarkCfg& cfg, const Committed* consts, const Committed& trace,
@@ -799,6 +845,8 @@
   ARENA_ALLOC(d_glde, (size_t)B * 6 * M);
   TRY(ntt_br2nat(d_g, N, d_glde, M, N, log_n, 6 * B, R, coset_scale, false, st));
   ARENA_ALLOC(d_v0, (size_t)B * 2 * M);
+  const uint64_t final_ml = (uint64_t)1 << (log_n - L.n_layers * cfg.arity_bits + r);
+  if (2 * final_ml * B > w.pinned_words) return fail(BP_ERR_UNSUPPORTED, "final FRI layer does not fit the mailbox");
   {
     FriInitArgs fi[MAX_LOCKSTEP] = {};
     for (uint32_t b = 0; b < B; b++) {
@@ -817,6 +865,7 @@
       f.alpha_shift[1] = gl::pow(alpha[b], k2);
       f.alpha_shift[2] = gl::ext(1);
       f.out = d_v0 + (size_t)b * 2 * M;
+      f.mirror = L.n_layers ? nullptr : w.pinned_dev + (size_t)b * 2 * final_ml;
     }
     TRY(launch_fri_init(fi, B, st));
   }
@@ -845,7 +894,7 @@
     TRY(merkle_upper_levels(d_dig, log_leaves, h, st, w.pinned_dev, &mirrored, B, dw));
     if (!mirrored)
       for (uint32_t b = 0; b < B; b++)
-        BPG_HIP(hipMemcpyAsync(w.pinned + b * L.cap_words, d_dig + (b + 1) * dw - L.cap_words, L.cap_words * 8,
+        BPG_HIP(stream_copy(w.pinned + b * L.cap_words, d_dig + (b + 1) * dw - L.cap_words, L.cap_words * 8,
                                hipMemcpyDeviceToHost, st));
     TRY(w.wait());
     for (uint32_t b = 0; b < B; b++) {
@@ -853,6 +902,7 @@
       std::memcpy(cap, w.pinned + b * L.cap_words, L.cap_words * 8);
       ch[b].observe(cap, L.cap_words);
       fa[b].beta = ch[b].challenge_ext();
+      fa[b].mirror = l + 1 == L.n_layers ? w.pinned_dev + (size_t)b * 2 * final_ml : nullptr;
     }
     TRY(launch_fri_fold(fa, B, st));
     layer_values[l] = cur; layer_vstride[l] = cur_stride; layer_digests[l] = d_dig; layer_dstride[l] = dw;
@@ -864,10 +914,7 @@
   }
   {
     const uint32_t log_ml = log_nl + r;
-    const uint64_t ml = (uint64_t)1 << log_ml, nl = (uint64_t)1 << log_nl;
-    if (2 * ml * B > w.pinned_words) return fail(BP_ERR_UNSUPPORTED, "final FRI layer does not fit the mailbox");
-    for (uint32_t b = 0; b < B; b++)
-      BPG_HIP(hipMemcpyAsync(w.pinned + b * 2 * ml, cur + b * cur_stride, 2 * ml * 8, hipMemcpyDeviceToHost, st));
+    const uint64_t ml = final_ml, nl = (uint64_t)1 << log_nl;
     TRY(w.wait());
     const uint64_t w_inv = gl::inv(gl::root(log_ml)), s_inv = gl::inv(shift), ml_inv = gl::inv(ml);
     std::vector<uint64_t> wp(ml);
@@ -907,29 +954,7 @@
     }
     unsigned long long res[MAX_LOCKSTEP];
     for (uint32_t b = 0; b < B; b++) res[b] = 0;
-    if (cfg.pow_bits) {
-      const uint32_t batch0 = (uint32_t)std::min<uint64_t>(1u << 20, std::max<uint64_t>(1u << 12, (uint64_t)1 << (cfg.pow_bits ? cfg.pow_bits - 1 : 0)));
-      uint32_t batch = batch0, n_batches = 0;
-      BPG_HIP(hipMemsetAsync(w.d_pow_result, 0xFF, 8 * MAX_LOCKSTEP, st));
-      for (uint64_t base = 0;;) {
-        for (int k = 0; k < 4; k++) {
-          if (++n_batches > 8) batch = std::min<uint32_t>(1u << 20, batch * 2);
-          for (uint32_t b = 0; b < B; b++) pa[b].base = base;
-          TRY(launch_pow(pa, B, batch, w.d_pow_result, st));
-          base += batch;
-        }
-        BPG_HIP(hipMemcpyAsync(w.pinned, w.d_pow_result, 8 * B, hipMemcpyDeviceToHost, st));
-        TRY(w.wait());
-        bool all = true;
-        for (uint32_t b = 0; b < B; b++) {
-          res[b] = reinterpret_cast<const unsigned long long*>(w.pinned)[b];
-          all = all && res[b] != ~0ULL;
-        }
-        if (all) break;
-        if (w.aborted()) return fail(BP_ERR_ABORTED, "aborted during proof of work");
-        if (base > ((uint64_t)1 << 44)) return fail(BP_ERR_DEVICE, "proof of work search exhausted");
-      }
-    }
+    if (cfg.pow_bits) TRY(pow_search(pow_search_of(w), pa, B, cfg.pow_bits, res));
     for (uint32_t b = 0; b < B; b++) {
       const uint64_t nonce = res[b];
       P[b][L.pow] = nonce;
@@ -969,8 +994,7 @@
       }
     }
     qa2->leaf_oracle = K ? 1 : 0;
-    TRY(launch_query_initial(*qa2, B, n_or, st));
-    TRY(launch_query_layers(*ql, B, L.n_layers, st));
+    TRY(launch_queries(*qa2, *ql, B, n_or, L.n_layers, st));
     if (q_direct) {
       TRY(w.wait());
       for (uint32_t b = 0; b < B; b++) std::memcpy(P[b] + L.queries, w.pinned + b * q_words, q_words * 8);
diff --git a/proof_protocol_decoder_amd/csrc/prover.hpp b/proof_protocol_decoder_amd/csrc/prover.hpp
--- a/proof_protocol_decoder_amd/csrc/prover.hpp
+++ b/proof_protocol_decoder_amd/csrc/prover.hpp
@@ -119,6 +119,8 @@
   size_t pinned_words = 0;
   uint64_t *hash_rows = nullptr, *hash_rows_dev = nullptr;
   unsigned long long* d_pow_result = nullptr;
+  uint32_t* d_pow_tickets = nullptr;
+  uint32_t pow_searches = 0;
   ArgRing args;
   void* args_mem = nullptr;
   hipEvent_t sync_event = nullptr;
@@ -159,6 +161,19 @@
                       const Committed* trace, const uint64_t* const* d_trace_values, const Ctl* ctl, Challenger* ch,
                       std::vector<uint64_t>* proofs, uint64_t* first_trace_leaf = nullptr);
 
+struct PowSearch {
+  hipStream_t stream;
+  Worker* worker;
+  unsigned long long* d_result;
+  uint32_t* d_tickets;
+  uint32_t* searches;
+  uint64_t *mailbox, *mailbox_dev;
+};
+inline PowSearch pow_search_of(Worker& w) {
+  return PowSearch{w.stream, &w, w.d_pow_result, w.d_pow_tickets, &w.pow_searches, w.pinned, w.pinned_dev};
+}
+int pow_search(const PowSearch& s, PowArgs* pa, uint32_t batch, uint32_t bits, unsigned long long* res);
+
 constexpr size_t ARG_RING_BYTES = (size_t)1 << 20;
 void arg_ring_register(hipStream_t st, ArgRing* ring);
 void arg_ring_unregister(hipStream_t st);
diff --git a/proof_protocol_decoder_amd/csrc/stark_api.cpp b/proof_protocol_decoder_amd/csrc/stark_api.cpp
--- a/proof_protocol_decoder_amd/csrc/stark_api.cpp
+++ b/proof_protocol_decoder_amd/csrc/stark_api.cpp
@@ -449,30 +449,68 @@
   if (!state || !nonce_out) return fail(BP_ERR_INVALID_INPUT, "bp_pow_grind: null argument");
   if (pos >= 8 || bits == 0 || bits > 40) return fail(BP_ERR_INVALID_INPUT, "bp_pow_grind: pos must be a rate word, bits in 1..40");
   hipStream_t st = as_stream(stream);
-  DeviceBuf res_buf;
-  BPG_HIP(hipMalloc(&res_buf.p, 8));
-  unsigned long long* d_res = res_buf.as<unsigned long long>();
+  DeviceBuf words;
+  BPG_HIP(hipMalloc(&words.p, 12 * MAX_LOCKSTEP));
+  {
+    uint64_t init[MAX_LOCKSTEP + MAX_LOCKSTEP / 2];
+    for (uint32_t k = 0; k < MAX_LOCKSTEP + MAX_LOCKSTEP / 2; k++) init[k] = k < MAX_LOCKSTEP ? ~0ULL : 0;
+    BPG_HIP(hipMemcpy(words.p, init, sizeof(init), hipMemcpyHostToDevice));
+  }
+  struct Mailbox {
+    uint64_t* p = nullptr;
+    ~Mailbox() { if (p) (void)hipHostFree(p); }
+  } mailbox;
+  uint64_t* mailbox_dev = nullptr;
+  BPG_HIP(hipHostMalloc(reinterpret_cast<void**>(&mailbox.p), 8, hipHostMallocDefault));
+  BPG_HIP(hipHostGetDevicePointer(reinterpret_cast<void**>(&mailbox_dev), mailbox.p, 0));
   PowArgs pa{};
   for (int i = 0; i < 12; i++) pa.state[i] = state[i];
   pa.pos = pos; pa.bits = bits;
-  int rc = BP_OK;
+  uint32_t searches = 0;
   unsigned long long res = ~0ULL;
-  if (hipMemsetAsync(d_res, 0xFF, 8, st) != hipSuccess) rc = fail(BP_ERR_DEVICE, "hipMemsetAsync failed");
-  uint32_t batch = (uint32_t)std::min<uint64_t>(1u << 20, std::max<uint64_t>(1u << 12, (uint64_t)2 << bits));
-  for (uint64_t base = 0; rc == BP_OK; base += batch, batch = std::min<uint32_t>(1u << 20, batch * 2)) {
-    pa.base = base;
-    if ((rc = launch_pow(pa, batch, d_res, st))) break;
-    if (hipMemcpyAsync(&res, d_res, 8, hipMemcpyDeviceToHost, st) != hipSuccess || hipStreamSynchronize(st) != hipSuccess) {
-      rc = fail(BP_ERR_DEVICE, "bp_pow_grind: copy back failed");
-      break;
-    }
-    if (res != ~0ULL) break;
-    if (base > ((uint64_t)1 << 44)) rc = fail(BP_ERR_DEVICE, "proof of work search exhausted");
-  }
+  const PowSearch ps{st, nullptr, words.as<unsigned long long>(), reinterpret_cast<uint32_t*>(words.as<unsigned long long>() + MAX_LOCKSTEP),
+                     &searches, mailbox.p, mailbox_dev};
+  const int rc = pow_search(ps, &pa, 1, bits, &res);
+  if (rc != BP_OK) (void)hipStreamSynchronize(st);
   if (rc == BP_OK) *nonce_out = res;
   return rc;
 }
 BPG_ABI_CATCH("bp_pow_grind")
+
+int bp_debug_pow_search(const uint64_t* states, const uint32_t* pos, uint32_t n, uint32_t bits, uint64_t* nonces_out, int device) try {
+  if (!states || !pos || !nonces_out) return fail(BP_ERR_INVALID_INPUT, "bp_debug_pow_search: null argument");
+  if (n == 0 || n > MAX_LOCKSTEP || bits == 0 || bits > 40)
+    return fail(BP_ERR_INVALID_INPUT, "bp_debug_pow_search: 1..%u proofs, bits in 1..40", MAX_LOCKSTEP);
+  PowArgs pa[MAX_LOCKSTEP] = {};
+  for (uint32_t b = 0; b < n; b++) {
+    if (pos[b] >= 8) return fail(BP_ERR_INVALID_INPUT, "bp_debug_pow_search: pos must be a rate word");
+    for (int i = 0; i < 12; i++) pa[b].state[i] = states[12 * b + i];
+    pa[b].pos = pos[b]; pa[b].bits = bits;
+  }
+  WorkerLease lease(device, (size_t)1 << 20);
+  if (lease.rc()) return lease.rc();
+  Worker& w = *lease;
+  unsigned long long res[MAX_LOCKSTEP];
+  int rc = pow_search(pow_search_of(w), pa, n, bits, res);
+  if (rc != BP_OK) {
+    (void)hipStreamSynchronize(w.stream);
+    w.args.rewind();
+    return rc;
+  }
+  for (uint32_t b = 0; b < n; b++) nonces_out[b] = res[b];
+  return BP_OK;
+}
+BPG_ABI_CATCH("bp_debug_pow_search")
+
+int bp_debug_stream_packets(uint64_t out[2], int reset) try {
+  std::atomic<uint64_t>* n = stream_packet_counts();
+  for (int k = 0; k < 2; k++) {
+    const uint64_t v = reset ? n[k].exchange(0) : n[k].load();
+    if (out) out[k] = v;
+  }
+  return BP_OK;
+}
+BPG_ABI_CATCH("bp_debug_stream_packets")
 
 int bp_openings(const uint64_t* d_coeffs, uint64_t stride, uint32_t log_n, uint32_t n_cols, const uint64_t z0[2],
                 const uint64_t z1[2], uint64_t* d_pw_scratch, uint64_t* d_out, void* stream) try {
diff --git a/proof_protocol_decoder_amd/csrc/stark_kernels.hip b/proof_protocol_decoder_amd/csrc/stark_kernels.hip
--- a/proof_protocol_decoder_amd/csrc/stark_kernels.hip
+++ b/proof_protocol_decoder_amd/csrc/stark_kernels.hip
@@ -1136,6 +1136,10 @@
   }
   a.out[2 * pos] = sum.c0;
   a.out[2 * pos + 1] = sum.c1;
+  if (a.mirror) {
+    a.mirror[2 * pos] = sum.c0;
+    a.mirror[2 * pos + 1] = sum.c1;
+  }
 }
 
 __global__ void __launch_bounds__(256) fri_layer_leaf_kernel(bpg::ArgPtr<bpg::FriLayerArgs> args) {
@@ -1297,32 +1301,54 @@
   acc = gl::scale(acc, a.arity_inv);
   a.out[2 * id] = acc.c0;
   a.out[2 * id + 1] = acc.c1;
-}
-
-__global__ void __launch_bounds__(256) pow_grind_kernel(bpg::ArgPtr<bpg::PowArgs> args, unsigned long long* result) {
+  if (a.mirror) {
+    a.mirror[2 * id] = acc.c0;
+    a.mirror[2 * id + 1] = acc.c1;
+  }
+}
+
+__device__ __forceinline__ void pow_done(unsigned long long* result, uint32_t* ticket, uint64_t* mailbox, uint64_t key) {
+  if (threadIdx.x != 0) return;
+  __threadfence();
+  if (atomicAdd(ticket, 1u) != gridDim.x - 1) return;
+  __threadfence();
+  const unsigned long long v = __hip_atomic_load(result, __ATOMIC_RELAXED, __HIP_MEMORY_SCOPE_AGENT);
+  *mailbox = (v >> bpg::POW_CAND_BITS) == (key >> bpg::POW_CAND_BITS) ? v - key : ~0ULL;
+  __hip_atomic_store(ticket, 0u, __ATOMIC_RELAXED, __HIP_MEMORY_SCOPE_AGENT);
+}
+__global__ void __launch_bounds__(256) pow_grind_kernel(bpg::ArgPtr<bpg::PowArgs> args, unsigned long long* result,
+                                                        uint32_t* tickets, uint64_t* mailbox) {
   BPG_ARG_BATCH(bpg::PowArgs, args);
   const bpg::PowArgs& a = batch[blockIdx.z];
   result += blockIdx.z;
-  if (__hip_atomic_load(result, __ATOMIC_RELAXED, __HIP_MEMORY_SCOPE_AGENT) < a.base + blockIdx.x * (uint64_t)blockDim.x) return;
-  const uint64_t cand = a.base + blockIdx.x * (uint64_t)blockDim.x + threadIdx.x;
-  uint64_t s[12];
-#pragma unroll
-  for (int k = 0; k < 12; k++) s[k] = a.state[k];
-  s[a.pos] = cand;
-  poseidon::permute(s);
-  if ((gl::canon(s[7]) >> (64 - a.bits)) == 0) atomicMin(result, (unsigned long long)cand);
+  if (__hip_atomic_load(result, __ATOMIC_RELAXED, __HIP_MEMORY_SCOPE_AGENT) >= a.key + a.base + blockIdx.x * (uint64_t)blockDim.x) {
+    const uint64_t cand = a.base + blockIdx.x * (uint64_t)blockDim.x + threadIdx.x;
+    uint64_t s[12];
+#pragma unroll
+    for (int k = 0; k < 12; k++) s[k] = a.state[k];
+    s[a.pos] = cand;
+    poseidon::permute(s);
+    if ((gl::canon(s[7]) >> (64 - a.bits)) == 0) atomicMin(result, (unsigned long long)(a.key + cand));
+    __threadfence();
+  }
+  __syncthreads();
+  pow_done(result, tickets + blockIdx.z, mailbox + blockIdx.z, a.key);
 }
 template <bool GR>
 __global__ void __launch_bounds__(256) __attribute__((amdgpu_waves_per_eu(3)))
-pow_grind_mx_kernel(bpg::ArgPtr<bpg::PowArgs> args, unsigned long long* result, const uint32_t* __restrict__ gtab) {
+pow_grind_mx_kernel(bpg::ArgPtr<bpg::PowArgs> args, unsigned long long* result, uint32_t* tickets, uint64_t* mailbox,
+                    const uint32_t* __restrict__ gtab) {
   BPG_ARG_BATCH(bpg::PowArgs, args);
   const bpg::PowArgs& a = batch[blockIdx.z];
   result += blockIdx.z;
   __shared__ uint32_t beaten;
   if (threadIdx.x == 0)
-    beaten = __hip_atomic_load(result, __ATOMIC_RELAXED, __HIP_MEMORY_SCOPE_AGENT) < a.base + (uint64_t)blockIdx.x * 256;
+    beaten = __hip_atomic_load(result, __ATOMIC_RELAXED, __HIP_MEMORY_SCOPE_AGENT) < a.key + a.base + (uint64_t)blockIdx.x * 256;
   __syncthreads();
-  if (beaten) return;
+  if (beaten) {
+    pow_done(result, tickets + blockIdx.z, mailbox + blockIdx.z, a.key);
+    return;
+  }
   __shared__ __attribute__((aligned(16))) uint32_t cin[GR ? poseidon::mx::CIN_GROUPED_WORDS : poseidon::mx::CIN_WORDS];
   __shared__ __attribute__((aligned(16))) uint32_t gt[GR ? poseidon::mx::grp::TABLE_WORDS : 4];
   if constexpr (GR) {
@@ -1349,14 +1375,15 @@
   if (c.kb == 3) {
 #pragma unroll
     for (int m = 0; m < 4; m++)
-      if ((gl::canon(e[m][1]) >> (64 - a.bits)) == 0) atomicMin(result, (unsigned long long)(cand0 + 16 * m));
-  }
-}
-
-__global__ void __launch_bounds__(256) query_initial_kernel(bpg::ArgPtr<bpg::QueryArgs> args) {
-  if (gridDim.x * gridDim.y * gridDim.z <= 64) __builtin_amdgcn_s_setprio(3);
-  const bpg::QueryArgs& a = *(const bpg::QueryArgs*)args;
-  const uint32_t b = blockIdx.x / a.n_queries, q = blockIdx.x % a.n_queries, o = blockIdx.y;
+      if ((gl::canon(e[m][1]) >> (64 - a.bits)) == 0) atomicMin(result, (unsigned long long)(a.key + cand0 + 16 * m));
+    __threadfence();
+  }
+  __syncthreads();
+  pow_done(result, tickets + blockIdx.z, mailbox + blockIdx.z, a.key);
+}
+
+__device__ __forceinline__ void query_initial(const bpg::QueryArgs& a, uint32_t o) {
+  const uint32_t b = blockIdx.x / a.n_queries, q = blockIdx.x % a.n_queries;
   const uint64_t x = a.x_index[blockIdx.x];
   const bpg::QueryOracle& orc = a.proof[b].oracle[o];
   const uint32_t log_rows = a.log_n + a.rate_bits;
@@ -1375,10 +1402,8 @@
   }
   if (q == 0 && o == a.leaf_oracle && a.proof[b].first_leaf && threadIdx.x < 4) a.proof[b].first_leaf[threadIdx.x] = orc.digests[x * 4 + threadIdx.x];
 }
-__global__ void __launch_bounds__(64) query_layers_kernel(bpg::ArgPtr<bpg::QueryLayerArgs> args) {
-  if (gridDim.x * gridDim.y * gridDim.z <= 64) __builtin_amdgcn_s_setprio(3);
-  const bpg::QueryLayerArgs& a = *(const bpg::QueryLayerArgs*)args;
-  const uint32_t b = blockIdx.x / a.n_queries, q = blockIdx.x % a.n_queries, l = blockIdx.y;
+__device__ __forceinline__ void query_layer(const bpg::QueryLayerArgs& a, uint32_t l) {
+  const uint32_t b = blockIdx.x / a.n_queries, q = blockIdx.x % a.n_queries;
   const bpg::QueryLayer& L = a.proof[b].layer[l];
   const uint32_t arity = 1u << a.arity_bits;
   const uint64_t leaf = a.x_index[blockIdx.x] >> (a.arity_bits * (l + 1));
@@ -1398,6 +1423,12 @@
     const uint64_t off = ((uint64_t)2 << log_leaves) - ((uint64_t)2 << (log_leaves - lvl));
     w[k] = L.digests[(off + ((leaf >> lvl) ^ 1)) * 4 + (k & 3)];
   }
+}
+__global__ void __launch_bounds__(256) query_kernel(bpg::ArgPtr<bpg::QueryArgs> args, bpg::ArgPtr<bpg::QueryLayerArgs> layers,
+                                                    uint32_t n_oracles) {
+  if (gridDim.x * gridDim.y * gridDim.z <= 64) __builtin_amdgcn_s_setprio(3);
+  if (blockIdx.y < n_oracles) query_initial(*(const bpg::QueryArgs*)args, blockIdx.y);
+  else query_layer(*(const bpg::QueryLayerArgs*)layers, blockIdx.y - n_oracles);
 }
 
 }
@@ -1542,7 +1573,7 @@
   } pole;
   const size_t words = 2 * (size_t)air::prog::MAX_PORTS;
   BPG_HIP(hipMalloc(reinterpret_cast<void**>(&pole.d), batch * words * 8));
-  BPG_HIP(hipMemsetAsync(pole.d, 0xFF, batch * words * 8, st));
+  BPG_HIP(stream_fill(pole.d, 0xFF, batch * words * 8, st));
   for (uint32_t b = 0; b < batch; b++)
     if (int rc = launch_port_terms(a[b], air_id, log_n, trace_stride, pole.d + b * words, st)) return rc;
   {
@@ -1552,7 +1583,7 @@
     BPG_LAUNCH_CHECK();
   }
   uint64_t found[MAX_LOCKSTEP * 2 * air::prog::MAX_PORTS];
-  BPG_HIP(hipMemcpyAsync(found, pole.d, batch * words * 8, hipMemcpyDeviceToHost, st));
+  BPG_HIP(stream_copy(found, pole.d, batch * words * 8, hipMemcpyDeviceToHost, st));
   BPG_HIP(hipStreamSynchronize(st));
   for (uint32_t b = 0; b < batch; b++)
     for (uint32_t k = 0; k < n_aux; k++)
@@ -1646,7 +1677,7 @@
   BPG_HIP(hipMalloc(reinterpret_cast<void**>(&tab.d), quotient_table_words(q) * 8));
   q.apow = tab.d;
   if (int rc = launch_alpha_tables(&q, 1, QuotCoset{}, st)) return rc;
-  BPG_HIP(hipMemcpyAsync(d_out, tab.d + 2 * (size_t)q.n_constraints + 48, air::plonk::HASH_FOLD_WORDS * 8, hipMemcpyDeviceToDevice, st));
+  BPG_HIP(stream_copy(d_out, tab.d + 2 * (size_t)q.n_constraints + 48, air::plonk::HASH_FOLD_WORDS * 8, hipMemcpyDeviceToDevice, st));
   BPG_HIP(hipStreamSynchronize(st));
   return BP_OK;
 }
@@ -1786,40 +1817,35 @@
   BPG_LAUNCH_CHECK();
   return BP_OK;
 }
-int launch_pow(const PowArgs* a, uint32_t batch, uint32_t n_candidates, unsigned long long* d_result, hipStream_t st) {
+int launch_pow(const PowArgs* a, uint32_t batch, uint32_t n_candidates, unsigned long long* d_result, uint32_t* d_tickets,
+               uint64_t* mailbox, hipStream_t st) {
   if (int rc = check_batch(batch)) return rc;
+  if (!n_candidates || n_candidates % 256) return fail(BP_ERR_INVALID_INPUT, "proof of work: a launch takes a multiple of 256 candidates");
   BPG_ARG_BLOCKS(ab, a, batch, st);
   const dim3 grid(n_candidates / 256, 1, batch);
   if (poseidon_mx()) {
     const uint32_t* gtab = group_tables();
-    if (gtab) pow_grind_mx_kernel<true><<<grid, 256, 0, st>>>(ab, d_result, gtab);
-    else pow_grind_mx_kernel<false><<<grid, 256, 0, st>>>(ab, d_result, nullptr);
+    if (gtab) pow_grind_mx_kernel<true><<<grid, 256, 0, st>>>(ab, d_result, d_tickets, mailbox, gtab);
+    else pow_grind_mx_kernel<false><<<grid, 256, 0, st>>>(ab, d_result, d_tickets, mailbox, nullptr);
   } else
-    pow_grind_kernel<<<grid, 256, 0, st>>>(ab, d_result);
-  BPG_LAUNCH_CHECK();
-  return BP_OK;
-}
-int launch_query_initial(const QueryArgs& a, uint32_t batch, uint32_t n_oracles, hipStream_t st) {
+    pow_grind_kernel<<<grid, 256, 0, st>>>(ab, d_result, d_tickets, mailbox);
+  BPG_LAUNCH_CHECK();
+  return BP_OK;
+}
+int launch_queries(const QueryArgs& a, const QueryLayerArgs& la, uint32_t batch, uint32_t n_oracles, uint32_t n_layers, hipStream_t st) {
   if (int rc = check_batch(batch)) return rc;
-  if (!a.n_queries || a.n_queries * batch > MAX_BATCH_QUERIES) return fail(BP_ERR_INVALID_INPUT, "query launch: %u x %u indices, at most %u", a.n_queries, batch, MAX_BATCH_QUERIES);
-  dim3 grid(a.n_queries * batch, n_oracles);
+  if (!a.n_queries || a.n_queries * batch > MAX_BATCH_QUERIES || n_layers > MAX_FRI_LAYERS || (n_layers && la.n_queries != a.n_queries))
+    return fail(BP_ERR_INVALID_INPUT, "query launch: %u x %u indices (at most %u), %u layers", a.n_queries, batch, MAX_BATCH_QUERIES, n_layers);
+  if (!n_oracles || n_oracles > 4) return fail(BP_ERR_INVALID_INPUT, "query launch: %u oracles", n_oracles);
+  dim3 grid(a.n_queries * batch, n_oracles + n_layers);
   const QueryArgs* ab = nullptr;
+  const QueryLayerArgs* lb = nullptr;
   if (int rc = arg_put(st, &a, 1, &ab)) return rc;
-  query_initial_kernel<<<grid, 256, 0, st>>>(arg_ptr(ab));
-  BPG_LAUNCH_CHECK();
-  return BP_OK;
-}
-int launch_query_layers(const QueryLayerArgs& a, uint32_t batch, uint32_t n_layers, hipStream_t st) {
-  if (!n_layers) return BP_OK;
-  if (int rc = check_batch(batch)) return rc;
-  if (!a.n_queries || a.n_queries * batch > MAX_BATCH_QUERIES || n_layers > MAX_FRI_LAYERS)
-    return fail(BP_ERR_INVALID_INPUT, "query launch: %u x %u indices, %u layers", a.n_queries, batch, n_layers);
-  dim3 grid(a.n_queries * batch, n_layers);
-  const QueryLayerArgs* ab = nullptr;
-  if (int rc = arg_put(st, &a, 1, &ab)) return rc;
-  query_layers_kernel<<<grid, 64, 0, st>>>(arg_ptr(ab));
-  BPG_LAUNCH_CHECK();
-  return BP_OK;
-}
-
-}
+  if (n_layers)
+    if (int rc = arg_put(st, &la, 1, &lb)) return rc;
+  query_kernel<<<grid, 256, 0, st>>>(arg_ptr(ab), arg_ptr(lb), n_oracles);
+  BPG_LAUNCH_CHECK();
+  return BP_OK;
+}
+
+}
diff --git a/proof_protocol_decoder_amd/csrc/stark_kernels.hpp b/proof_protocol_decoder_amd/csrc/stark_kernels.hpp
--- a/proof_protocol_decoder_amd/csrc/stark_kernels.hpp
+++ b/proof_protocol_decoder_amd/csrc/stark_kernels.hpp
@@ -1,5 +1,6 @@
 #pragma once
 #include <hip/hip_runtime.h>
+#include <atomic>
 #include <cstdint>
 #include "air.hpp"
 #include "gl.hpp"
@@ -105,6 +106,7 @@
   uint32_t log_n, rate_bits;
   uint64_t g_t[16];
   gl::Ext y[3], z[3], alpha_shift[3];
+  uint64_t* mirror;
 };
 struct FriLayerArgs {
   const uint64_t* values;
@@ -116,11 +118,14 @@
   uint64_t wa_inv_pow[16];
   uint64_t arity_inv;
   gl::Ext beta;
-};
+  uint64_t* mirror;
+};
+constexpr uint32_t POW_CAND_BITS = 44;
 struct PowArgs {
   uint64_t state[12];
   uint64_t base;
   uint32_t pos, bits;
+  uint64_t key;
 };
 struct QueryOracle {
   const uint64_t *lde, *digests;
@@ -212,12 +217,19 @@
 int launch_fri_layer_leaves(const FriLayerArgs* a, uint32_t batch, hipStream_t st);
 int launch_fri_fold(const FriLayerArgs* a, uint32_t batch, hipStream_t st);
 inline int launch_fri_fold(const FriLayerArgs& a, hipStream_t st) { return launch_fri_fold(&a, 1, st); }
-int launch_pow(const PowArgs* a, uint32_t batch, uint32_t n_candidates, unsigned long long* d_result, hipStream_t st);
-inline int launch_pow(const PowArgs& a, uint32_t n_candidates, unsigned long long* d_result, hipStream_t st) {
-  return launch_pow(&a, 1, n_candidates, d_result, st);
-}
-int launch_query_initial(const QueryArgs& a, uint32_t batch, uint32_t n_oracles, hipStream_t st);
-int launch_query_layers(const QueryLayerArgs& a, uint32_t batch, uint32_t n_layers, hipStream_t st);
+int launch_pow(const PowArgs* a, uint32_t batch, uint32_t n_candidates, unsigned long long* d_result, uint32_t* d_tickets,
+               uint64_t* mailbox, hipStream_t st);
+int launch_queries(const QueryArgs& a, const QueryLayerArgs& la, uint32_t batch, uint32_t n_oracles, uint32_t n_layers, hipStream_t st);
+
+std::atomic<uint64_t>* stream_packet_counts();
+inline hipError_t stream_copy(void* dst, const void* src, size_t bytes, hipMemcpyKind kind, hipStream_t st) {
+  stream_packet_counts()[0].fetch_add(1, std::memory_order_relaxed);
+  return hipMemcpyAsync(dst, src, bytes, kind, st);
+}
+inline hipError_t stream_fill(void* dst, int value, size_t bytes, hipStream_t st) {
+  stream_packet_counts()[1].fetch_add(1, std::memory_order_relaxed);
+  return hipMemsetAsync(dst, value, bytes, st);
+}
 
 int init_ntt_kernels();
 int get_table(int kind, uint32_t log_n, uint32_t rate_bits, const uint64_t** out);
diff --git a/proof_protocol_decoder_amd/ops.py b/proof_protocol_decoder_amd/ops.py
--- a/proof_protocol_decoder_amd/ops.py
+++ b/proof_protocol_decoder_amd/ops.py
@@ -364,6 +364,20 @@
     nonce = C.c_uint64()
     check(own().bp_pow_grind((C.c_uint64 * 12)(*[int(x) for x in state]), pos, bits, C.byref(nonce), _stream()))
     return nonce.value
+
+
+def pow_search(states, pos, bits, device=0):
+    n = len(states)
+    flat = (C.c_uint64 * (12 * n))(*[int(x) for s in states for x in s])
+    nonces = (C.c_uint64 * n)()
+    check(own().bp_debug_pow_search(flat, (C.c_uint32 * n)(*[int(p) for p in pos]), n, bits, nonces, device))
+    return list(nonces)
+
+
+def stream_packets(reset=False):
+    out = (C.c_uint64 * 2)()
+    check(own().bp_debug_stream_packets(out, 1 if reset else 0))
+    return out[0], out[1]
 
 
 def merkle_commit(lde, log_n, rate_bits, cap_height):
```

Measured after the change: 35.95. -9.0%, worse.
